# beta-team/beta-recsys

Hardware: AMD Instinct MI355X
Metric: training interactions/sec (BPR triples) (higher is better)
Workload: dtype f32; 1 GPU; BPR-MF, MovieLens-1M-shaped synthetic (BASELINE configs[1]): 6040 users x 3706 items, dim 64, batch 4096 triples/GPU, uniform users, Zipf(1.0) positives, uniform negatives; optimizer=adam, loss=bpr, batch_per_gpu=4096, global_batch=4096, parallelism=single GPU, epoch=245 steps = 1003520 triples (SURVEY 8d C2: ~1M triples / epoch)

## Files before the change

beta-recsys_amd/_lib.py:

```python
import ctypes
import os
from ctypes import POINTER, Structure, c_char_p, c_double, c_float, c_int, c_int32, c_int64
from ctypes import c_size_t, c_uint32, c_void_p

_HERE = os.path.dirname(os.path.abspath(__file__))
LIB_PATH = os.path.join(_HERE, os.environ.get("HIPREC_LIB", "libhiprec.so"))

OPT_SGD, OPT_ADAM, OPT_RMSPROP = 0, 1, 2
OPT_KINDS = {"sgd": OPT_SGD, "adam": OPT_ADAM, "rmsprop": OPT_RMSPROP}
OPT_RMSPROP_MOMENTUM = 3

STATUS_USER_OOB, STATUS_ITEM_OOB, STATUS_ROW_OOB, STATUS_ROUTE_OVERFLOW = 1, 2, 4, 8
STATUS_NEG_EXHAUSTED = 16
STATUS_LAZY_TABLE = 32
STATUS_TABLE_FULL = 64


class MfTables(Structure):

    _fields_ = [
        ("user_emb", c_void_p),
        ("item_emb", c_void_p),
        ("user_bias", c_void_p),
        ("item_bias", c_void_p),
# ... 222 lines not shown
    "hiprec_mf_sgd_rows": (
        c_int,
        [_T, _T, _P, _P, _P, _P, c_int64, c_double, _P, _P, c_int32, _P, _P, _P],
    ),
    "hiprec_ncf_plan_bytes": (c_size_t, []),
    "hiprec_gemm_f32": (
        c_int,
        [c_int, c_int, c_int, c_int, _P, c_int, _P, c_int, _P, c_int, _P, c_int, _P, c_int, _P],
    ),
    "hiprec_ncf_forward": (c_int, [POINTER(NcfPlan), _P, _P, c_int64, _P, _P]),
    "hiprec_ncf_grad": (
        c_int,
        [POINTER(NcfPlan), _P, _P, _P, c_int64, c_float, _P, _P, c_size_t, _P],
    ),
    "hiprec_ncf_step": (
        c_int,
        [POINTER(NcfPlan), _P, _P, _P, c_int64, c_float, c_int, _P, _P, _P, _P, c_int64, c_int64, c_int64, c_double,
         c_double, c_double, c_double, _P, _P, c_size_t, _P],
    ),
    "hiprec_lightgcn_plan_bytes": (c_size_t, []),
    "hiprec_spmm_csr": (c_int, [POINTER(Csr), _P, c_float, _P, _P, _P, c_int32, _P]),
    "hiprec_sliced_width": (c_int32, [c_int64, c_int32]),
    "hiprec_sliced_row_cap": (c_int32, [c_int64, c_int32]),
    "hiprec_to_sliced": (c_int, [_P, c_int64, c_int32, c_int32, _P, _P, _P]),
    "hiprec_from_sliced": (c_int, [_P, c_int64, c_int32, c_int32, _P, c_int32, _P]),
    "hiprec_sliced_drop_values": (c_int, [POINTER(SlicedCsr), _P, _P, _P]),
    "hiprec_spmm_sliced": (c_int, [POINTER(SlicedCsr), _P, c_float, _P, _P, _P, c_int32, c_int32, c_int32, _P]),
    "hiprec_edge_dropout_mask": (c_int, [_P, c_int64, c_float, ctypes.c_uint64, ctypes.c_uint64, _P]),
    "hiprec_lightgcn_step_values": (c_int, [POINTER(LightGcnPlan), _P, c_float, c_int32, ctypes.c_uint64,
                                            ctypes.c_uint64, _P]),
    "hiprec_lightgcn_opt_stage": (c_int, [POINTER(LightGcnPlan), c_int32, _P, _P, _P, c_double, c_double, c_double,
                                          c_double, _P, _P, c_float, ctypes.c_uint64, ctypes.c_uint64, _P]),
    "hiprec_lightgcn_propagate": (c_int, [POINTER(LightGcnPlan), _P, c_float, _P]),
    "hiprec_lightgcn_predict": (c_int, [POINTER(LightGcnPlan), _P, _P, c_int64, _P, _P, _P]),
    "hiprec_lightgcn_grad": (
        c_int,
        [POINTER(LightGcnPlan), _P, c_float, _P, _P, _P, c_int64, c_float, _P, _P, c_size_t, _P],
    ),
    "hiprec_random_permutation": (c_int, [_P, c_int64, ctypes.c_uint64, _P]),
    "hiprec_fused_step_bytes": (c_size_t, []),
    "hiprec_mf_bpr_fused_step": (c_int, [POINTER(FusedStep), _P, _P, _P, c_int64, c_int64, c_float, _P, _P]),
    "hiprec_dp_step_bytes": (c_size_t, []),
    "hiprec_mf_dp_step_begin": (c_int, [POINTER(DpStep), _P, _P, _P, c_int64, c_float, _P]),
    "hiprec_mf_dp_step_end": (c_int, [POINTER(DpStep), _P]),
    "hiprec_sample_negatives": (
        c_int,
        [_P, _P, c_int64, c_int64, _P, c_int64, c_int32, ctypes.c_uint64, _P, _P, _P],
    ),
    "hiprec_pgmf_workspace_bytes": (c_size_t, [c_int32]),
    "hiprec_pgmf_bpr_grad": (
        c_int,
        [POINTER(PgmfTables), POINTER(PgmfTables), _P, _P, _P, c_int64, c_float, c_float, _P, _P, c_size_t,
         _P, c_size_t, _P],
    ),
    "hiprec_pgmf_epoch": (
        c_int,
        [POINTER(PgmfTables), POINTER(PgmfTables), _P, _P, _P, c_int64, c_int64, c_float, c_float, c_int,
         c_double, c_double, c_double, c_double, _P, _P, _P, _P, c_int64, _P, _P, c_size_t, _P, c_size_t,
         _P, c_size_t, _P],
    ),
    "hiprec_cmn_tables_bytes": (c_size_t, []),
    "hiprec_cmn_workspace_bytes": (c_size_t, [c_int32, c_int64]),
    "hiprec_cmn_grad_padded": (
        c_int,
        [POINTER(CmnTables), POINTER(CmnTables), _P, _P, _P, _P, _P, c_int64, _P, _P, c_int64, c_int64, c_float,
         c_float, _P, _P, _P, _P, c_size_t, _P, c_size_t, _P],
    ),
    "hiprec_cmn_grad_csr": (
        c_int,
        [POINTER(CmnTables), POINTER(CmnTables), _P, _P, _P, _P, _P, c_int64, c_float, c_float, _P, _P, _P, _P,
         c_size_t, _P, c_size_t, _P],
    ),
    "hiprec_cmn_epoch": (
        c_int,
        [POINTER(CmnTables), POINTER(CmnTables), _P, _P, _P, _P, _P, c_int64, c_int64, c_float, c_float, c_int,
         c_double, c_double, c_double, c_double, _P, _P, _P, _P, c_int64, _P, _P, c_size_t, _P, c_size_t,
         _P, c_size_t, _P],
    ),
    "hiprec_t2v_epoch": (
        c_int,
        [POINTER(T2vTables), POINTER(T2vTables), _P, _P, _P, _P, _P, _P, c_int64, c_int64, c_int32, c_float,
         c_int, c_double, c_double, c_double, c_double, _P, _P, _P, _P, c_int64, _P, _P, c_size_t, _P],
    ),
    "hiprec_clip_workspace_bytes": (c_size_t, []),
    "hiprec_clip_grad_norm": (c_int, [_P, c_int64, c_float, _P, c_size_t, _P]),
    "hiprec_clip_opt_dense_step": (
        c_int,
        [c_int, _P, _P, _P, _P, c_int64, c_double, c_double, c_double, c_double, _P, _P, c_int64, c_float, _P, c_size_t,
         _P],
    ),
    "hiprec_t2v_grad": (
        c_int,
        [POINTER(T2vTables), POINTER(T2vTables), _P, _P, _P, _P, _P, _P, c_int64, c_int32, c_float, _P, _P,
         c_size_t, _P],
    ),
    "hiprec_t2v_predict": (c_int, [POINTER(T2vTables), _P, _P, c_int64, _P, _P, _P]),
    "hiprec_sumsq_workspace_bytes": (c_size_t, []),
    "hiprec_sumsq": (c_int, [_P, c_int64, _P, c_size_t, _P]),
    "hiprec_opt_dense_step_decay": (
        c_int,
        [c_int, _P, _P, _P, _P, c_int64, c_double, c_double, c_double, c_double, _P, _P, c_float, _P, c_size_t, _P],
    ),
    "hiprec_decay_grad": (c_int, [_P, _P, c_int64, c_float, _P]),
    "hiprec_ultragcn_grad": (
        c_int,
        [POINTER(UltraGcnTables), POINTER(UltraGcnTables), POINTER(UltraGcnParams), _P, _P, _P, c_int64, c_int32, _P,
         _P, _P, c_size_t, _P],
    ),
    "hiprec_ultragcn_predict": (c_int, [POINTER(UltraGcnTables), _P, _P, c_int64, _P, _P, _P]),
    "hiprec_ultragcn_epoch": (
        c_int,
        [POINTER(UltraGcnTables), POINTER(UltraGcnTables), POINTER(UltraGcnParams), _P, _P, _P, c_int64, c_int64,
         c_int32, c_int, c_double, c_double, c_double, c_double, _P, _P, _P, _P, c_int64, _P, c_size_t, _P, _P,
         c_size_t, _P],
    ),
    "hiprec_alias_sample": (c_int, [_P, _P, _P, c_int64, ctypes.c_uint64, _P, c_int64, _P]),
    "hiprec_ngcf_plan_bytes": (c_size_t, []),
    "hiprec_ngcf_forward": (c_int, [POINTER(NgcfPlan), c_int, _P]),
    "hiprec_ngcf_predict": (c_int, [POINTER(NgcfPlan), _P, _P, c_int64, _P, _P, _P]),
    "hiprec_ngcf_grad": (c_int, [POINTER(NgcfPlan), _P, _P, _P, c_int64, c_float, _P, _P, c_size_t, _P]),
    "hiprec_csr_n_slices": (c_int64, [c_int64]),
    "hiprec_csr_slice_rows": (c_int, [POINTER(Csr), _P, c_int64, _P]),
    "hiprec_rank_metrics_workspace_bytes": (c_size_t, [c_int64, c_int32]),
    "hiprec_rank_metrics": (
        c_int,
        [_P, c_int64, _P, _P, POINTER(c_int32), c_int32, _P, c_size_t, _P, _P],
    ),
    "hiprec_topk_workspace_bytes": (c_size_t, [c_int64, c_int64, c_int32, c_int32]),
    "hiprec_topk_recommend": (
        c_int,
        [_P, c_int64, c_int64, _P, c_int64, c_int64, c_int32, c_float, _P, _P, c_int64, _P, _P, c_int32, c_int32, _P,
         c_size_t, _P, _P, _P, _P],
    ),
    "hiprec_topk_metrics": (
        c_int,
        [_P, c_int64, c_int32, _P, _P, POINTER(c_int32), c_int32, _P, c_size_t, _P, _P],
    ),
    "hiprec_stage_epoch": (c_int, [_P, _P, _P, c_int32, _P, c_int64, c_int64, _P, _P, _P, _P]),
    "hiprec_stage_epoch_shuffled": (c_int, [_P, _P, _P, c_int32, ctypes.c_uint64, c_int64, c_int64, _P, _P, _P, _P]),
    "hiprec_mf_bce_epoch": (
        c_int,
        [_T, _T, _P, _P, _P, _P, c_int64, c_int64, c_float, c_int]
        + [c_double, c_double, c_double, c_double]
        + [_P, _P, _P, _P, c_int64, _P, _P, c_int32, _P, _P, c_size_t, _P],
    ),
    "hiprec_mf_bpr_epoch_fused": (
        c_int,
        [c_int, _P, _P, _P, _P, _P, c_int64, c_int64, c_int32, _P, _P, _P, c_int64, c_int64, c_float,
         c_double, c_double, c_double, c_double, _P, POINTER(c_int32), _P],
    ),
    "hiprec_mf_bpr_epoch_fused_range": (
        c_int,
        [c_int, _P, _P, _P, _P, _P, c_int64, c_int64, c_int32, _P, _P, _P, c_int64, c_int64, c_int64, c_int64,
         c_float, c_double, c_double, c_double, c_double, _P, POINTER(c_int32), _P],
    ),
    "hiprec_mf_bpr_dp_epoch_fused_range": (
        c_int,
        [c_int, _P, _P, c_int64, _P, _P, c_int64, c_int64, c_int64, c_int32, _P, _P, _P, c_int64, c_int64, c_int64,
         c_int64, c_int32, c_float, c_double, c_double, c_double, c_double, _P, _P, _P, POINTER(c_int32), _P],
    ),
    "hiprec_mf_bpr_epoch_owned": (
        c_int,
        [_P, c_int64, c_int64, c_int32, _P, _P, _P, _P, _P, _P, _P, c_int64, _P, _P, c_int64, _P, _P, c_int64,
         c_int64, c_int64, c_int64, c_float, c_double, _P, _P],
    ),
    "hiprec_ownership_table_bits": (c_int32, [c_int64]),
    "hiprec_ownership_ws_ints": (c_int64, [c_int64, c_int64, c_int32]),
    "hiprec_batch_row_ownership": (
        c_int, [_P, _P, _P, c_int64, c_int64, c_int64, c_int64, c_int32, _P, _P, _P, _P]),
    "hiprec_stage_grouped_ws_ints": (c_int64, [c_int64, c_int64, c_int64]),
    "hiprec_stage_epoch_grouped": (
        c_int, [_P, _P, _P, _P, c_int32, ctypes.c_uint64, c_int64, c_int64, c_int64, _P, _P, _P, _P, _P]),
    "hiprec_mf_pull_chunk": (c_int32, [c_int32]),
    "hiprec_contrib_row_cap": (c_int64, [c_int64, c_int32]),
    "hiprec_batch_row_contrib": (
        c_int, [_P, _P, _P, c_int64, c_int64, c_int64, c_int64, c_int32, c_int32, c_int32, _P, _P, _P, c_int64, _P, _P]),
    "hiprec_mf_bpr_epoch_pull": (
        c_int,
        [_P, c_int64, c_int64, c_int32, _P, _P, _P, _P, c_int64, _P, c_int64, _P, _P, _P, _P, c_int64, c_int64,
         c_int64, c_int64, c_float, c_double, _P, _P],
    ),
    "hiprec_mf_bpr_owned_remote_step": (
        c_int,
        [_P, c_int64, c_int64, c_int32, _P, _P, c_int64, _P, _P, _P, _P, _P, _P, _P, _P, _P, c_int64, c_float,
         c_float, c_double, _P, _P, _P],
    ),
    "hiprec_mf_bpr_pull_remote_step": (
        c_int,
        [_P, c_int64, c_int64, c_int32, _P, _P, c_int64, _P, _P, _P, _P, _P, _P, _P, c_int64, _P, _P, _P, _P, c_int32,
         c_int64, c_float, c_float, c_double, _P, _P, _P],
    ),
    "hiprec_batch_row_ownership_tables": (
        c_int, [_P, _P, _P, c_int64, c_int64, c_int64, c_int64, c_int32, _P, _P, _P, _P, _P, _P, _P]),
    "hiprec_plan_route_tiles": (c_int64, [c_int64, c_int64]),
    "hiprec_plan_route_triples": (
        c_int, [_P, _P, _P, _P, c_int64, c_int64, c_int32, c_int64, c_int64, _P, _P, _P, _P, _P]),
    "hiprec_plan_place_triples": (c_int, [_P, c_int64, _P, c_int32, c_int64, c_int64, _P, _P, _P, _P, _P]),
    "hiprec_plan_slot_ws_ints": (c_int64, [c_int64, c_int32, c_int32]),
    "hiprec_plan_item_slots": (
        c_int, [_P, c_int64, c_int64, c_int32, c_int64, c_int32] + [_P] * 16 + [_P, _P, c_int64, _P, _P]),
    "hiprec_plan_place_requests": (c_int, [_P, c_int64, _P, c_int32, c_int64, _P, _P, _P, _P, c_int64, _P, _P]),
    "hiprec_shard_payload_zero": (
        c_int, [_P, _P, c_int64, c_int32, _P, c_int64, c_int64, c_int64, _P, _P, _P, c_int64, _P, _P, _P]),
    "hiprec_mf_bpr_grad_remote_step": (
        c_int,
        [_P, _P, c_int64, c_int64, c_int32, _P, _P, c_int64, _P, _P, _P, _P, _P, _P, _P, c_int64, c_float, c_float,
         _P, _P, _P],
    ),
    "hiprec_shard_apply_finish": (
        c_int, [_P, _P, c_int64, c_int32, _P, _P, c_int64, c_int64, c_int64, _P, c_double, _P, c_int32, _P, c_double,
                c_int32, _P, _P, _P]),
    "hiprec_shard_planned_steps": (
        c_int, [POINTER(ShardPlan), POINTER(ShardBufs), c_int64, c_int64, c_int32, c_float, c_double, c_double,
                c_double, c_double, POINTER(NcclFns), _P, _P, _P]),
    "hiprec_shard_planned_steps_ex": (
        c_int, [POINTER(ShardPlan), POINTER(ShardBufs), c_int64, c_int64, c_int32, c_float, c_double, c_double,
                c_double, c_double, POINTER(NcclFns), _P, ctypes.c_uint32, _P, _P]),
    "hiprec_gather_epoch": (c_int, [_P, _P, _P, _P, c_int32, ctypes.c_uint64, _P, c_int64, _P, _P, _P, _P]),
    "hiprec_stage_sort_keys": (c_int, [_P, _P, c_int32, ctypes.c_uint64, c_int64, c_int64, c_int64, c_int32, _P, _P]),
    "hiprec_group_epoch_by_item": (c_int, [_P, _P, _P, c_int64, c_int64, c_int64, c_int32, _P, _P, _P, _P, _P, _P, _P, _P,
                                           _P, _P]),
    "hiprec_lazy_state_bytes": (c_size_t, []),
    "hiprec_lazy_catchup": (c_int, [POINTER(LazyState), POINTER(LazyRows), _P, _P]),
    "hiprec_lazy_update": (c_int, [POINTER(LazyState), POINTER(LazyRows), _P, _P, _P]),
    "hiprec_lazy_flush": (c_int, [POINTER(LazyState), _P, _P]),
    "hiprec_lazy_mark_current": (c_int, [POINTER(LazyState), _P, _P]),
    "hiprec_mf_epoch_lazy": (c_int, [POINTER(LazyState), _T, _T, _P, _P, _P, c_int32, c_int64, c_int64, c_int32, c_float,
                                     _P, _P, c_size_t, _P]),
    "hiprec_mf_bpr_grad_owned": (c_int, [_P, _P, c_int64, c_int64, c_int32, _P, _P, _P, _P, _P, _P, _P, c_int64, c_float,
                                         c_float, _P, _P, _P]),
    "hiprec_mf_epoch_lazy_pull": (c_int, [POINTER(LazyState), _P, _P, _P, _P, c_int64, _P, c_int64, _P, _P, _P, c_int64,
                                          c_int64, c_int32, c_float, _P, _P, _P]),
    "hiprec_mf_epoch_lazy_owned": (c_int, [POINTER(LazyState), _P, _P, _P, _P, _P, _P, _P, c_int64, c_int64, c_int64,
                                           c_int32, c_float, _P, _P, _P]),
    "hiprec_shard_plan_bytes": (c_size_t, []),
    "hiprec_shard_bufs_bytes": (c_size_t, []),
    "hiprec_shard_publish_partials": (c_int, [_P, _P, c_int32, _P, c_int32, _P]),
    "hiprec_shard_apply_rows": (c_int, [_P, _P, c_int64, c_int32, _P, _P, c_int64, c_double, _P, _P]),
    "hiprec_shard_finish_step": (c_int, [_P, c_int32, _P, c_int32, _P, c_double, c_int32, _P, _P]),
    "hiprec_mf_bpr_epoch_sgd_fused": (
        c_int,
        [_P, _P, _P, c_int64, c_int64, c_int32, _P, _P, _P, c_int64, c_int64, c_float, c_double, _P,
         POINTER(c_int32), _P],
    ),
    "hiprec_mf_bpr_epoch": (
        c_int,
        [_T, _T, _P, _P, _P, _P, c_int64, c_int64, c_float, c_int]
        + [c_double, c_double, c_double, c_double]
        + [_P, _P, _P, _P, c_int64, _P, _P, c_int32, _P, _P, c_size_t, _P],
    ),
}

_lib = None


class HiprecError(RuntimeError):
    """A libhiprec call returned a non-zero code."""


def load():
    global _lib
    if _lib is not None:
        return _lib
    if not os.path.exists(LIB_PATH):
        raise RuntimeError(
            f"libhiprec.so not found at {LIB_PATH}: the HIP extension is the only compute path of "
            "this package (there is no CPU fallback). Build it with "
            "`python -c 'import __graft_entry__ as g; g.build()'` (hipcc --offload-arch=gfx950)."
        )
    import torch

    lib = ctypes.CDLL(LIB_PATH)
    for name, (restype, argtypes) in SIGNATURES.items():
        try:
            fn = getattr(lib, name)
        except AttributeError as exc:
            raise RuntimeError(f"libhiprec.so does not export {name}; rebuild it") from exc
        fn.restype = restype
        fn.argtypes = argtypes
    if lib.hiprec_stats_bytes() != ctypes.sizeof(Stats):
        raise RuntimeError("hiprec_stats layout mismatch between _lib.py and libhiprec.so")
    if lib.hiprec_lightgcn_plan_bytes() != ctypes.sizeof(LightGcnPlan):
        raise RuntimeError("hiprec_lightgcn_plan layout mismatch between _lib.py and libhiprec.so")
    if lib.hiprec_fused_step_bytes() != ctypes.sizeof(FusedStep):
        raise RuntimeError("hiprec_fused_step layout mismatch between _lib.py and libhiprec.so")
    if lib.hiprec_dp_step_bytes() != ctypes.sizeof(DpStep):
        raise RuntimeError("hiprec_dp_step layout mismatch between _lib.py and libhiprec.so")
    if lib.hiprec_ngcf_plan_bytes() != ctypes.sizeof(NgcfPlan):
        raise RuntimeError("hiprec_ngcf_plan layout mismatch between _lib.py and libhiprec.so")
    if lib.hiprec_lazy_state_bytes() != ctypes.sizeof(LazyState):
        raise RuntimeError("hiprec_lazy_state layout mismatch between _lib.py and libhiprec.so")
    if lib.hiprec_shard_bufs_bytes() != ctypes.sizeof(ShardBufs):
        raise RuntimeError("hiprec_shard_bufs layout mismatch between _lib.py and libhiprec.so")
    if lib.hiprec_cmn_tables_bytes() != ctypes.sizeof(CmnTables):
        raise RuntimeError("hiprec_cmn_tables layout mismatch between _lib.py and libhiprec.so")
    if lib.hiprec_ncf_plan_bytes() != ctypes.sizeof(NcfPlan):
        raise RuntimeError("hiprec_ncf_plan layout mismatch between _lib.py and libhiprec.so")
    _lib = _DeviceGuardedLib(lib)
    return _lib


class _Stream(c_void_p):

    device_index = None


# ... 77 lines not shown
```

beta-recsys_amd/csrc/common.hpp:

```cpp
#pragma once
#include <hip/hip_runtime.h>

#include <atomic>
#include <initializer_list>

#include <cstdarg>
#include <cstdint>
#include <cstdio>

#include "../../include/hiprec.h"

namespace hiprec {

constexpr int kWave = 64;
constexpr int kBlock = 256;
constexpr int kWavesPerBlock = kBlock / kWave;
constexpr int kMaxBlocks = 2048;
constexpr int kAggWaves = 16;
constexpr int kAggBlock = kAggWaves * kWave;
constexpr int kAggMaxBlocks = 512;
constexpr size_t kScratchBytes = 16 + sizeof(float) * 4 * kMaxBlocks;

struct Scratch {
  uint32_t n_partials;
  uint32_t _pad[3];
  float4 partials[kMaxBlocks];
};
static_assert(sizeof(Scratch) == kScratchBytes, "scratch layout");

void set_error(const char* fmt, ...);
int hip_fail(hipError_t e, const char* what);

int allow_dynamic_lds(std::initializer_list<const void*> kernels, size_t bytes, std::atomic<uint64_t>& done,
                      const char* what);

int opt_dense_step_impl(int kind, float* w, float* g, float* m, float* v, int64_t n, double lr, double beta1,
                        double beta2, double eps, hiprec_stats* stats, const void* scratch, int64_t scalar_index,
                        double* clip_ws, int n_clip, float max_norm, void* stream);

#define HIPREC_TRY(expr)                                   \
  do {                                                     \
    hipError_t _e = (expr);                                \
    if (_e != hipSuccess) return hiprec::hip_fail(_e, #expr); \
  } while (0)

#define HIPREC_REQUIRE(cond, ...)        \
  do {                                   \
    if (!(cond)) {                       \
      hiprec::set_error(__VA_ARGS__);    \
      return HIPREC_E_BADARG;            \
    }                                    \
  } while (0)

inline int grid_for_waves(int64_t n_waves) {
  int64_t blocks = (n_waves + kWavesPerBlock - 1) / kWavesPerBlock;
  if (blocks < 1) blocks = 1;
  if (blocks > kMaxBlocks) blocks = kMaxBlocks;
  return static_cast<int>(blocks);
}

inline int grid_for_threads(int64_t n_threads) {
  int64_t blocks = (n_threads + kBlock - 1) / kBlock;
  if (blocks < 1) blocks = 1;
  if (blocks > kMaxBlocks) blocks = kMaxBlocks;
  return static_cast<int>(blocks);
}

__host__ __device__ inline int feistel_half_bits(uint64_t n) {
  int bits = 2;
  while (bits < 62 && (1ull << bits) < n) ++bits;
  return (bits + 1) / 2;
}

#if defined(__HIPCC__)

__device__ __forceinline__ uint64_t splitmix64(uint64_t x) {
  x += 0x9E3779B97F4A7C15ull;
  x = (x ^ (x >> 30)) * 0xBF58476D1CE4E5B9ull;
  x = (x ^ (x >> 27)) * 0x94D049BB133111EBull;
  return x ^ (x >> 31);
}

__device__ __forceinline__ bool keep_draw(uint64_t seed, uint64_t step, int64_t e, float keep_prob) {
  uint64_t z = seed + 0x9E3779B97F4A7C15ull * (static_cast<uint64_t>(e) + 1) + 0xD1B54A32D192ED03ull * (step + 1);
  z = (z ^ (z >> 30)) * 0xBF58476D1CE4E5B9ull;
  z = (z ^ (z >> 27)) * 0x94D049BB133111EBull;
  z ^= z >> 31;
  return static_cast<float>(z >> 40) * (1.0f / 16777216.0f) < keep_prob;
}

__device__ __forceinline__ uint32_t feistel_round(uint32_t x, uint32_t key) {
  x = (x ^ key) * 0x9E3779B1u;
  x ^= x >> 15;
  x *= 0x85EBCA77u;
  x ^= x >> 13;
  return x;
}

__device__ __forceinline__ uint64_t feistel_permute(uint64_t i, uint64_t n, int half_bits, uint64_t seed) {
  const uint64_t mask = (1ull << half_bits) - 1ull;
  uint64_t x = i;
  do {
    uint32_t l = static_cast<uint32_t>(x >> half_bits), r = static_cast<uint32_t>(x & mask);
#pragma unroll
    for (int round = 0; round < 6; ++round) {
      const uint32_t k = static_cast<uint32_t>(seed >> (8 * (round & 3))) + 0x632BE5ABu * (round + 1) +
                         static_cast<uint32_t>(seed >> 32);
      const uint32_t f = feistel_round(r, k) & static_cast<uint32_t>(mask);
      const uint32_t nl = r;
      r = l ^ f;
      l = nl;
    }
    x = (static_cast<uint64_t>(l) << half_bits) | r;
  } while (x >= n);
  return x;
}

template <int CTRL>
__device__ __forceinline__ float dpp_add(float v) {
  int moved = __builtin_amdgcn_update_dpp(0, __builtin_bit_cast(int, v), CTRL, 0xF, 0xF, false);
  return v + __builtin_bit_cast(float, moved);
}

__device__ __forceinline__ float wave_sum(float v) {
  v = dpp_add<0xB1>(v);
  v = dpp_add<0x4E>(v);
  v = dpp_add<0x141>(v);
  v = dpp_add<0x140>(v);
  int iv = __builtin_bit_cast(int, v);
  float r0 = __builtin_bit_cast(float, __builtin_amdgcn_readlane(iv, 0));
  float r1 = __builtin_bit_cast(float, __builtin_amdgcn_readlane(iv, 16));
  float r2 = __builtin_bit_cast(float, __builtin_amdgcn_readlane(iv, 32));
  float r3 = __builtin_bit_cast(float, __builtin_amdgcn_readlane(iv, 48));
  return (r0 + r1) + (r2 + r3);
}

__device__ __forceinline__ int wave_in_block() {
  return __builtin_amdgcn_readfirstlane(static_cast<int>(threadIdx.x) >> 6);
}

__device__ __forceinline__ int lane_id() { return static_cast<int>(threadIdx.x) & 63; }

__device__ __forceinline__ void lds_barrier() {
  asm volatile("s_waitcnt lgkmcnt(0)" ::: "memory");
  __builtin_amdgcn_s_barrier();
  asm volatile("" ::: "memory");
}

__device__ __forceinline__ void lds_add_f32(float* p, float v) {
  __hip_atomic_fetch_add(p, v, __ATOMIC_RELAXED, __HIP_MEMORY_SCOPE_WORKGROUP);
}

__device__ __forceinline__ void atomic_add_f32(float* p, float v) {
  __hip_atomic_fetch_add(p, v, __ATOMIC_RELAXED, __HIP_MEMORY_SCOPE_AGENT);
}

__device__ __forceinline__ int run_head(const long long* s_item, int wv, long long item) {
  int head = wv;
  while (head > 0 && s_item[head - 1] == item) --head;
  return head;
}

__device__ __forceinline__ int run_end(const long long* s_item, int wv, long long item, int n_waves) {
  int end = wv + 1;
  while (end < n_waves && s_item[end] == item) ++end;
  return end;
}

__device__ __forceinline__ float sigmoid_f32(float s) { return 1.0f / (1.0f + expf(-s)); }

__device__ __forceinline__ float neg_logsigmoid(float x, float* sig_neg_x) {
  float z = expf(-fabsf(x));
  float frac = z / (1.0f + z);
  *sig_neg_x = x < 0.0f ? 1.0f - frac : frac;
  return log1pf(z) - fminf(x, 0.0f);
}

template <int NW>
__device__ __forceinline__ void publish_partials(float loss_w, float reg_lane, float gb_w,
                                                 float inv_batch, Scratch* scratch) {
  __shared__ float s_loss[NW];
  __shared__ float s_reg[NW];
  __shared__ float s_gb[NW];
  float reg_w = wave_sum(reg_lane);
  const int w = wave_in_block();
  if (lane_id() == 0) {
    s_loss[w] = loss_w;
    s_reg[w] = reg_w;
    s_gb[w] = gb_w;
  }
  lds_barrier();
  if (threadIdx.x == 0) {
    float l = 0.f, r = 0.f, b = 0.f;
#pragma unroll
    for (int i = 0; i < NW; ++i) {
      l += s_loss[i];
      r += s_reg[i];
      b += s_gb[i];
    }
    scratch->partials[blockIdx.x] = make_float4(l * inv_batch, r * inv_batch, b, 0.f);
    if (blockIdx.x == 0) scratch->n_partials = gridDim.x;
  }
}

template <int NT = kBlock>
__device__ __forceinline__ float finalize_partials(hiprec_stats* stats, const Scratch* scratch) {
  __shared__ double s_l[NT];
  __shared__ double s_r[NT];
  __shared__ double s_b[NT];
  const uint32_t n = scratch->n_partials;
  double l = 0.0, r = 0.0, b = 0.0;
  for (uint32_t i = threadIdx.x; i < n; i += NT) {
    float4 p = scratch->partials[i];
    l += p.x;
    r += p.y;
    b += p.z;
  }
  s_l[threadIdx.x] = l;
  s_r[threadIdx.x] = r;
  s_b[threadIdx.x] = b;
  __syncthreads();
  for (int s = NT / 2; s > 0; s >>= 1) {
    if (static_cast<int>(threadIdx.x) < s) {
      s_l[threadIdx.x] += s_l[threadIdx.x + s];
// ... 108 lines not shown
```

beta-recsys_amd/csrc/mf.hip:

```cpp
#include <algorithm>
#include <type_traits>

#include "common.hpp"

namespace hiprec {



struct TripleIdx {
  int64_t u, p, n;
  bool valid;
};

__device__ __forceinline__ TripleIdx load_triple(const hiprec_mf_tables& w,
                                                 const int64_t* __restrict__ users,
                                                 const int64_t* __restrict__ pos,
                                                 const int64_t* __restrict__ neg,
                                                 const int64_t* __restrict__ perm, int64_t t,
                                                 int64_t batch, hiprec_stats* stats, int lane) {
  TripleIdx r{0, 0, 0, t < batch};
  if (r.valid) {
    const int64_t j = perm ? perm[t] : t;
    r.u = users[j];
    r.p = pos[j];
// ... 324 lines not shown
      const bool i_ok = static_cast<uint64_t>(p) < static_cast<uint64_t>(f.n_items) &&
                        static_cast<uint64_t>(n) < static_cast<uint64_t>(f.n_items);
      if (!(u_ok && i_ok)) {
        if (lane == 0)
          atomicOr(&stats->status,
                   (u_ok ? 0u : HIPREC_STATUS_USER_OOB) | (i_ok ? 0u : HIPREC_STATUS_ITEM_OOB));
        valid = false;
      }
    }
    if (lane == 0) s_item[wv] = valid ? static_cast<long long>(p) : -static_cast<long long>(wv + 1);
    lds_barrier();
    const int head = valid ? run_head(s_item, wv, p) : wv;
    const bool is_head = head == wv;
    const int tail = (valid && is_head) ? run_end(s_item, wv, p, kAggWaves) : wv + 1;

    float uu[NPL], pp[NPL];
    float dpos = 0.f, bp = 0.f;
    if (valid) {
      const int64_t ou = u * D, op = o_ie + p * D, on = o_ie + n * D;
      float nn[NPL];
      float dp = 0.f, dn = 0.f;
      const float wbu = wf[o_ub + u], gbu = f.g_prev[o_ub + u];
      const float wbn = wf[o_ib + n], gbn = f.g_prev[o_ib + n];
      const float wbp = wf[o_ib + p], gbp_ = f.g_prev[o_ib + p];
      float mbu = 0.f, mbn = 0.f, mbp = 0.f, vbu = 0.f, vbn = 0.f, vbp = 0.f;
      if constexpr (kHasM) {
        mbu = f.m_read[o_ub + u];
        mbn = f.m_read[o_ib + n];
        mbp = f.m_read[o_ib + p];
      }
      if constexpr (kHasV) {
        vbu = f.v_read[o_ub + u];
        vbn = f.v_read[o_ib + n];
        vbp = f.v_read[o_ib + p];
      }
      float wu[NPL], gu[NPL], wp[NPL], gpv[NPL], wn[NPL], gn[NPL];
      float mu[NPL], mpv[NPL], mn[NPL], vu[NPL], vpv[NPL], vn[NPL];
#pragma unroll
      for (int k = 0; k < NPL; ++k) {
        const int c = lane + kWave * k;
        const int cc = c < D ? c : D - 1;
        wu[k] = wf[ou + cc];
        gu[k] = f.g_prev[ou + cc];
        wp[k] = wf[op + cc];
        gpv[k] = f.g_prev[op + cc];
        wn[k] = wf[on + cc];
        gn[k] = f.g_prev[on + cc];
        mu[k] = mpv[k] = mn[k] = vu[k] = vpv[k] = vn[k] = 0.f;
        if constexpr (kHasM) {
          mu[k] = f.m_read[ou + cc];
          mpv[k] = f.m_read[op + cc];
          mn[k] = f.m_read[on + cc];
        }
        if constexpr (kHasV) {
          vu[k] = f.v_read[ou + cc];
          vpv[k] = f.v_read[op + cc];
          vn[k] = f.v_read[on + cc];
        }
      }
#pragma unroll
      for (int k = 0; k < NPL; ++k) {
        const bool in = lane + kWave * k < D;
        if (apply) {
          wu[k] = fused_eff<KIND>(wu[k], gu[k], mu[k], vu[k], f.s, step_size, bc2_sqrt);
          wp[k] = fused_eff<KIND>(wp[k], gpv[k], mpv[k], vpv[k], f.s, step_size, bc2_sqrt);
          wn[k] = fused_eff<KIND>(wn[k], gn[k], mn[k], vn[k], f.s, step_size, bc2_sqrt);
        }
        uu[k] = in ? wu[k] : 0.f;
        pp[k] = in ? wp[k] : 0.f;
        nn[k] = in ? wn[k] : 0.f;
      }
#pragma unroll
      for (int k = 0; k < NPL; ++k) {
        dp += uu[k] * pp[k];
        dn += uu[k] * nn[k];
        reg_acc += 2.f * uu[k] * uu[k] + pp[k] * pp[k] + nn[k] * nn[k];
      }
      dp = wave_sum(dp);
      dn = wave_sum(dn);
      if (!gb_ready) {
        float gbp = 0.f;
#pragma unroll
        for (int j = 0; j < kFusedSlots; ++j) {
          asm volatile("" : "+v"(gbz[j]));
          gbp += lane + kWave * j < f.n_prev_partials ? gbz[j] : 0.f;
        }
        gb = apply ? fused_eff<KIND>(gb_w, gb_g + wave_sum(gbp), gb_m, gb_v, f.s, step_size, bc2_sqrt)
                   : gb_w;
        gb_ready = true;
      }
      float bu = wbu, bn = wbn;
      bp = wbp;
      if (apply) {
        bu = fused_eff<KIND>(wbu, gbu, mbu, vbu, f.s, step_size, bc2_sqrt);
        bn = fused_eff<KIND>(wbn, gbn, mbn, vbn, f.s, step_size, bc2_sqrt);
        bp = fused_eff<KIND>(wbp, gbp_, mbp, vbp, f.s, step_size, bc2_sqrt);
      }
      const float yp = sigmoid_f32(((dp + bu) + bp) + gb);
      const float yn = sigmoid_f32(((dn + bu) + bn) + gb);
      float sig_neg_x;
      const float nls = neg_logsigmoid(yp - yn, &sig_neg_x);
      const float delta = -sig_neg_x * inv_batch;
      dpos = delta * ((1.f - yp) * yp);
      const float dneg = -delta * ((1.f - yn) * yn);
      float* gur = gf + ou;
      float* gnr = gf + on;
      float* slot = s_acc + wv * ld;
#pragma unroll
      for (int k = 0; k < NPL; ++k) {
        const int c = lane + kWave * k;
        if (c < D) {
          atomic_add_f32(gur + c, (dpos * pp[k] + dneg * nn[k]) + ru * uu[k]);
          atomic_add_f32(gnr + c, dneg * uu[k] + ri * nn[k]);
          slot[c] = dpos * uu[k] + ri * pp[k];
        }
      }
      if (lane == 0) {
        atomic_add_f32(gf + o_ub + u, (dpos + dneg) + ru * bu);
        atomic_add_f32(gf + o_ib + n, dneg + ri * bn);
        slot[D] = dpos + ri * bp;
        reg_acc += 2.f * bu * bu + bp * bp + bn * bn;
      }
      loss_acc += nls;
      gb_acc += dpos + dneg;
    }
    lds_barrier();
    if (valid && is_head) {
      float* gpr = gf + o_ie + p * D;
      for (int c = lane; c <= D; c += kWave) {
        float t = s_acc[wv * ld + c];
        for (int j = wv + 1; j < tail; ++j) t += s_acc[j * ld + c];
        atomic_add_f32(c < D ? gpr + c : gf + o_ib + p, t);
      }
    }
  }
  __shared__ float s_loss[kAggWaves], s_reg[kAggWaves], s_gbv[kAggWaves];
  const float reg_w = wave_sum(reg_acc);
  if (lane == 0) {
    s_loss[wv] = loss_acc;
    s_reg[wv] = reg_w;
    s_gbv[wv] = gb_acc;
  }
  lds_barrier();
  if (threadIdx.x == 0) {
    float l = 0.f, r = 0.f, b = 0.f;
#pragma unroll
    for (int i = 0; i < kAggWaves; ++i) {
      l += s_loss[i];
      r += s_reg[i];
      b += s_gbv[i];
    }
    scratch->partials[blockIdx.x] = make_float4(l * inv_batch, r * inv_batch, b, 0.f);
    if (blockIdx.x == 0) scratch->n_partials = static_cast<uint32_t>(f.n_gather_blocks);
  }
}

template <int NPL>
__global__ __launch_bounds__(kAggBlock) void mf_bce_grad_kernel(
    hiprec_mf_tables w, hiprec_mf_tables g, const int64_t* __restrict__ users,
    const int64_t* __restrict__ items, const float* __restrict__ ratings,
    const int64_t* __restrict__ perm, int64_t batch, float inv_batch, float reg_coef,
    hiprec_stats* stats, Scratch* scratch) {
  extern __shared__ __attribute__((aligned(16))) float s_acc[];
  __shared__ long long s_item[kAggWaves];
  const int lane = lane_id();
  const int wv = wave_in_block();
  const int D = w.dim;
  const int ld = D + 1;
  const float gb = load_scalar_param(w.global_bias);
  const float rr = 2.f * reg_coef * inv_batch;

  float loss_acc = 0.f, reg_acc = 0.f, gb_acc = 0.f;
  const bool stepper = blockIdx.x == 0 && threadIdx.x == 0;
  StepState step_state{};
  if (stepper) step_state = step_load(stats);

  for (int64_t base = static_cast<int64_t>(blockIdx.x) * kAggWaves; base < batch;
       base += static_cast<int64_t>(gridDim.x) * kAggWaves) {
    const int64_t t = base + wv;
    bool valid = t < batch;
    int64_t u = 0, i = 0;
    float r = 0.f;
    if (valid) {
      const int64_t j = perm ? perm[t] : t;
      u = users[j];
      i = items[j];
      r = ratings[j];
      const bool u_ok = static_cast<uint64_t>(u) < static_cast<uint64_t>(w.n_users);
      const bool i_ok = static_cast<uint64_t>(i) < static_cast<uint64_t>(w.n_items);
      if (!(u_ok && i_ok)) {
        if (lane == 0)
          atomicOr(&stats->status,
                   (u_ok ? 0u : HIPREC_STATUS_USER_OOB) | (i_ok ? 0u : HIPREC_STATUS_ITEM_OOB));
        valid = false;
      }
    }
    if (lane == 0) s_item[wv] = valid ? static_cast<long long>(i) : -static_cast<long long>(wv + 1);
    lds_barrier();
    const int head = valid ? run_head(s_item, wv, i) : wv;
    const bool is_head = head == wv;
    const int tail = (valid && is_head) ? run_end(s_item, wv, i, kAggWaves) : wv + 1;

    const float* ur = w.user_emb + u * D;
    const float* ir = w.item_emb + i * D;
    float uu[NPL > 0 ? NPL : 1], ii[NPL > 0 ? NPL : 1];
    float ds = 0.f, bi = 0.f;
    if (valid) {
      float* gur = g.user_emb + u * D;
      float dot = 0.f;
      if constexpr (NPL > 0) {
#pragma unroll
        for (int k = 0; k < NPL; ++k) {
          const int c = lane + kWave * k;
          const bool in = c < D;
          uu[k] = in ? ur[c] : 0.f;
          ii[k] = in ? ir[c] : 0.f;
          dot += uu[k] * ii[k];
          reg_acc += uu[k] * uu[k] + ii[k] * ii[k];
        }
      } else {
        for (int c = lane; c < D; c += kWave) {
          const float a = ur[c], b = ir[c];
          dot += a * b;
          reg_acc += a * a + b * b;
        }
      }
      dot = wave_sum(dot);
      const float bu = w.user_bias[u];
      bi = w.item_bias[i];
      const float y = sigmoid_f32(((dot + bu) + bi) + gb);
      const float ly = fmaxf(logf(y), -100.f);
      const float l1y = fmaxf(log1pf(-y), -100.f);
      const float loss_k = -(r * ly + (1.f - r) * l1y);
      const float gy = (y - r) / fmaxf((1.f - y) * y, 1e-12f) * inv_batch;
      ds = gy * ((1.f - y) * y);

      float* slot = s_acc + wv * ld;
      if constexpr (NPL > 0) {
#pragma unroll
        for (int k = 0; k < NPL; ++k) {
          const int c = lane + kWave * k;
          if (c < D) {
            atomic_add_f32(gur + c, ds * ii[k] + rr * uu[k]);
            slot[c] = ds * uu[k] + rr * ii[k];
          }
        }
      } else {
        for (int c = lane; c < D; c += kWave) {
          const float a = ur[c], b = ir[c];
          atomic_add_f32(gur + c, ds * b + rr * a);
          slot[c] = ds * a + rr * b;
        }
      }
      if (lane == 0) {
        atomic_add_f32(g.user_bias + u, ds + rr * bu);
        slot[D] = ds + rr * bi;
        reg_acc += bu * bu + bi * bi;
      }
      loss_acc += loss_k;
      gb_acc += ds;
    }
    lds_barrier();
    if (valid && is_head) {
      float* gir = g.item_emb + i * D;
      for (int c = lane; c <= D; c += kWave) {
        float t = s_acc[wv * ld + c];
        for (int j = wv + 1; j < tail; ++j) t += s_acc[j * ld + c];
        atomic_add_f32(c < D ? gir + c : g.item_bias + i, t);
      }
    }
  }
  publish_partials<kAggWaves>(loss_acc, reg_acc, gb_acc, inv_batch, scratch);
  if (stepper) step_store_advanced(stats, step_state);
}

__global__ __launch_bounds__(kBlock) void mf_predict_kernel(hiprec_mf_tables w,
                                                            const int64_t* __restrict__ users,
                                                            const int64_t* __restrict__ items,
                                                            int64_t n, float* __restrict__ scores,
                                                            float* __restrict__ sq, hiprec_stats* stats) {
  const int lane = lane_id();
  const int D = w.dim;
  const int64_t wave0 = static_cast<int64_t>(blockIdx.x) * kWavesPerBlock + wave_in_block();
  const int64_t n_waves = static_cast<int64_t>(gridDim.x) * kWavesPerBlock;
  const float gb = load_scalar_param(w.global_bias);
  for (int64_t t = wave0; t < n; t += n_waves) {
    const int64_t u = users[t], i = items[t];
    const bool u_ok = static_cast<uint64_t>(u) < static_cast<uint64_t>(w.n_users);
    const bool i_ok = static_cast<uint64_t>(i) < static_cast<uint64_t>(w.n_items);
    if (!(u_ok && i_ok)) {
      if (lane == 0) {
        atomicOr(&stats->status,
                 (u_ok ? 0u : HIPREC_STATUS_USER_OOB) | (i_ok ? 0u : HIPREC_STATUS_ITEM_OOB));
        scores[t] = __builtin_nanf("");
        if (sq) sq[t] = 0.f;
      }
      continue;
    }
    const float* ur = w.user_emb + u * D;
    const float* ir = w.item_emb + i * D;
    float dot = 0.f, ss = 0.f;
    for (int c = lane; c < D; c += kWave) {
      const float a = ur[c], b = ir[c];
      dot += a * b;
      ss += a * a + b * b;
    }
// ... 247 lines not shown
  return dispatch_npl(w->dim, [&](auto npl) {
    mf_sgd_rows_kernel<decltype(npl)::value><<<grid, kBlock, 0, st>>>(
        *w, *g, users, items_a, items_b, perm, batch, static_cast<float>(lr), user_stamp, item_stamp, stamp,
        stats, static_cast<const Scratch*>(scratch));
  });
}

template <int KIND>
static int launch_fused(int dim, int grid, size_t lds, hipStream_t st, const FusedOpt& f, const int64_t* uu,
                        const int64_t* pp, const int64_t* nn, int64_t b, float inv_b, float reg_coef,
                        hiprec_stats* stats, Scratch* sc) {
  if (b == 0)
    mf_bpr_fused_kernel<1, KIND, true><<<grid, kAggBlock, lds, st>>>(f, uu, pp, nn, b, inv_b, reg_coef, stats, sc);
  else if (dim <= 64)
    mf_bpr_fused_kernel<1, KIND, false><<<grid, kAggBlock, lds, st>>>(f, uu, pp, nn, b, inv_b, reg_coef, stats, sc);
  else if (dim <= 128)
    mf_bpr_fused_kernel<2, KIND, false><<<grid, kAggBlock, lds, st>>>(f, uu, pp, nn, b, inv_b, reg_coef, stats, sc);
  else
    mf_bpr_fused_kernel<4, KIND, false><<<grid, kAggBlock, lds, st>>>(f, uu, pp, nn, b, inv_b, reg_coef, stats, sc);
  HIPREC_TRY(hipGetLastError());
  return 0;
}

extern "C" int hiprec_mf_bpr_fused_step(const hiprec_fused_step* c, const int64_t* users,
                                        const int64_t* pos, const int64_t* neg, int64_t batch,
                                        int64_t prev_batch, float inv_batch, hiprec_stats* stats,
                                        void* stream) {
  HIPREC_REQUIRE(c && stats, "NULL step / stats");
  const int kind = c->kind;
  HIPREC_REQUIRE(kind == HIPREC_OPT_SGD || kind == HIPREC_OPT_ADAM || kind == HIPREC_OPT_RMSPROP,
                 "unknown optimizer kind %d", kind);
  const bool has_m = kind == HIPREC_OPT_ADAM, has_v = kind != HIPREC_OPT_SGD;
  HIPREC_REQUIRE(c->w_read && c->w_write && c->g_prev && c->g_cur && c->g_zero && c->scratch_prev &&
                     c->scratch_cur, "NULL buffer");
  HIPREC_REQUIRE(!has_m || (c->m_read && c->m_write), "Adam needs m_read / m_write");
  HIPREC_REQUIRE(!has_v || (c->v_read && c->v_write), "Adam/RMSprop need v_read / v_write");
  HIPREC_REQUIRE(c->n_users > 0 && c->n_items > 0 && c->dim > 0 && c->dim <= 256, "fused step needs dim <= 256");
  HIPREC_REQUIRE(batch >= 0 && prev_batch >= 0, "negative batch");
  HIPREC_REQUIRE(batch == 0 || (users && pos && neg), "NULL index arrays");
  hipStream_t st = static_cast<hipStream_t>(stream);
  const int64_t n_users = c->n_users, n_items = c->n_items;
  const int dim = c->dim;
  const int64_t n_flat = (n_users + n_items) * (static_cast<int64_t>(dim) + 1) + 1;
  FusedOpt f;
  f.n_users = n_users;
  f.n_items = n_items;
  f.dim = dim;
  f._pad0 = 0;
  f.g_cur = c->g_cur;
  f.w_read = c->w_read;
  f.g_prev = c->g_prev;
  f.m_read = has_m ? c->m_read : nullptr;
  f.v_read = has_v ? c->v_read : nullptr;
  f.w_write = c->w_write;
  f.m_write = has_m ? c->m_write : nullptr;
  f.v_write = has_v ? c->v_write : nullptr;
  f.g_zero = c->g_zero;
  f.g_zero2 = batch == 0 ? const_cast<float*>(c->g_prev) : nullptr;
  f.n_flat = n_flat;
  f.s = OptScalars{c->lr,
                   static_cast<float>(c->lr),
                   static_cast<float>(c->beta2),
                   static_cast<float>(1.0 - c->beta1),
                   static_cast<float>(1.0 - c->beta2),
                   static_cast<float>(c->eps)};
  f.n_gather_blocks = batch > 0 ? std::min(agg_grid(batch), kFusedMaxGather) : 0;
  f.n_prev_partials = prev_batch > 0 ? std::min(agg_grid(prev_batch), kFusedMaxGather) : 0;
  f.apply_prev = prev_batch > 0 ? 1 : 0;
  f.scratch_prev = static_cast<const Scratch*>(c->scratch_prev);
  Scratch* sc = static_cast<Scratch*>(c->scratch_cur);
  const size_t lds = agg_lds_bytes(dim);
  const int n_sweep = static_cast<int>(std::min<int64_t>(256, (n_flat / 4 + kAggBlock - 1) / kAggBlock));
  const int grid = f.n_gather_blocks + n_sweep;
  int rc;
  if (kind == HIPREC_OPT_SGD)
    rc = launch_fused<HIPREC_OPT_SGD>(dim, grid, lds, st, f, users, pos, neg, batch, inv_batch, c->reg_coef, stats, sc);
  else if (kind == HIPREC_OPT_ADAM)
    rc = launch_fused<HIPREC_OPT_ADAM>(dim, grid, lds, st, f, users, pos, neg, batch, inv_batch, c->reg_coef, stats, sc);
  else
    rc = launch_fused<HIPREC_OPT_RMSPROP>(dim, grid, lds, st, f, users, pos, neg, batch, inv_batch, c->reg_coef, stats, sc);
  return rc;
}

extern "C" size_t hiprec_fused_step_bytes(void) { return sizeof(hiprec_fused_step); }

extern "C" int hiprec_mf_bpr_epoch_fused_range(int kind, float* const* w_flat, float* const* g_flat,
                                               float* const* m_flat, float* const* v_flat,
                                               void* const* scratch2, int64_t n_users, int64_t n_items,
                                               int32_t dim, const int64_t* users, const int64_t* pos,
                                               const int64_t* neg, int64_t n_triples, int64_t batch,
                                               int64_t step_begin, int64_t step_end,
                                               float reg_coef, double lr, double beta1, double beta2,
                                               double eps, hiprec_stats* stats, int32_t* final_index,
                                               void* stream) {
  HIPREC_REQUIRE(w_flat && g_flat && scratch2 && final_index && stats, "NULL pointer");
  HIPREC_REQUIRE(w_flat[0] && w_flat[1] && g_flat[0] && g_flat[1] && g_flat[2] && scratch2[0] &&
                     scratch2[1], "NULL buffer");
  const bool has_m = kind == HIPREC_OPT_ADAM, has_v = kind != HIPREC_OPT_SGD;
  HIPREC_REQUIRE(!has_m || (m_flat && m_flat[0] && m_flat[1]), "Adam needs m_flat[2]");
  HIPREC_REQUIRE(!has_v || (v_flat && v_flat[0] && v_flat[1]), "Adam/RMSprop need v_flat[2]");
  HIPREC_REQUIRE(n_triples >= 0 && batch > 0, "bad n_triples/batch");
  HIPREC_REQUIRE(n_triples == 0 || (users && pos && neg), "NULL index arrays");
  const int64_t n_steps = (n_triples + batch - 1) / batch;
  HIPREC_REQUIRE(0 <= step_begin && step_begin <= step_end && step_end <= n_steps,
                 "bad step range [%lld, %lld) of %lld", (long long)step_begin, (long long)step_end, (long long)n_steps);
  const int64_t k_end = step_end == n_steps ? n_steps + 1 : step_end;
  hiprec_fused_step c{};
  c.kind = kind;
  c.dim = dim;
  c.n_users = n_users;
  c.n_items = n_items;
  c.lr = lr;
  c.beta1 = beta1;
  c.beta2 = beta2;
  c.eps = eps;
  c.reg_coef = reg_coef;
  for (int64_t k = step_begin; k < k_end; ++k) {
    const int64_t off = k * batch;
    const int64_t b = k < n_steps ? std::min<int64_t>(batch, n_triples - off) : 0;
    const int64_t prev_b = k > 0 ? std::min<int64_t>(batch, n_triples - (k - 1) * batch) : 0;
    const int out = k == n_steps ? 0 : static_cast<int>((k + 1) & 1);
    c.w_read = w_flat[k & 1];
    c.w_write = w_flat[out];
    c.m_read = has_m ? m_flat[k & 1] : nullptr;
    c.m_write = has_m ? m_flat[out] : nullptr;
    c.v_read = has_v ? v_flat[k & 1] : nullptr;
    c.v_write = has_v ? v_flat[out] : nullptr;
    c.g_prev = g_flat[(k + 2) % 3];
    c.g_cur = g_flat[k % 3];
    c.g_zero = g_flat[(k + 1) % 3];
    c.scratch_prev = scratch2[(k + 1) & 1];
    c.scratch_cur = scratch2[k & 1];
    const float inv_b = b > 0 ? 1.0f / static_cast<float>(b) : 0.f;
    if (int rc = hiprec_mf_bpr_fused_step(&c, users ? users + off : nullptr, pos ? pos + off : nullptr,
                                          neg ? neg + off : nullptr, b, prev_b, inv_b, stats, stream))
      return rc;
  }
  *final_index = step_end == n_steps ? 0 : -1;
  return 0;
}

extern "C" int hiprec_mf_bpr_epoch_fused(int kind, float* const* w_flat, float* const* g_flat,
                                         float* const* m_flat, float* const* v_flat,
                                         void* const* scratch2, int64_t n_users, int64_t n_items,
                                         int32_t dim, const int64_t* users, const int64_t* pos,
                                         const int64_t* neg, int64_t n_triples, int64_t batch,
                                         float reg_coef, double lr, double beta1, double beta2,
                                         double eps, hiprec_stats* stats, int32_t* final_index,
                                         void* stream) {
  const int64_t n_steps = batch > 0 && n_triples >= 0 ? (n_triples + batch - 1) / batch : 0;
  return hiprec_mf_bpr_epoch_fused_range(kind, w_flat, g_flat, m_flat, v_flat, scratch2, n_users, n_items, dim,
                                         users, pos, neg, n_triples, batch, 0, n_steps, reg_coef, lr, beta1,
                                         beta2, eps, stats, final_index, stream);
}

using nccl_all_reduce_fn = int (*)(const void*, void*, size_t, int, int, void*, hipStream_t);
constexpr int kNcclFloat32 = 7, kNcclSum = 0;

extern "C" int hiprec_mf_bpr_dp_epoch_fused_range(int kind, float* const* w_flat, float* const* bufs,
                                                  int64_t scratch_floats, float* const* m_flat,
                                                  float* const* v_flat, int64_t n_flat, int64_t n_users,
                                                  int64_t n_items, int32_t dim, const int64_t* users,
                                                  const int64_t* pos, const int64_t* neg, int64_t n_triples,
                                                  int64_t batch, int64_t step_begin, int64_t step_end,
                                                  int32_t world, float reg_coef, double lr, double beta1,
                                                  double beta2, double eps, hiprec_stats* stats,
                                                  void* all_reduce_fn, void* comm, int32_t* final_index,
                                                  void* stream) {
  HIPREC_REQUIRE(w_flat && bufs && final_index && stats && all_reduce_fn && comm, "NULL pointer");
  HIPREC_REQUIRE(w_flat[0] && w_flat[1] && bufs[0] && bufs[1] && bufs[2], "NULL buffer");
  const bool has_m = kind == HIPREC_OPT_ADAM, has_v = kind != HIPREC_OPT_SGD;
  HIPREC_REQUIRE(!has_m || (m_flat && m_flat[0] && m_flat[1]), "Adam needs m_flat[2]");
  HIPREC_REQUIRE(!has_v || (v_flat && v_flat[0] && v_flat[1]), "Adam/RMSprop need v_flat[2]");
  HIPREC_REQUIRE(n_triples >= 0 && batch > 0 && world >= 1 && scratch_floats >= 4 && n_flat > 0, "bad sizes");
  HIPREC_REQUIRE(n_triples == 0 || (users && pos && neg), "NULL index arrays");
  const int64_t n_steps = (n_triples + batch - 1) / batch;
  HIPREC_REQUIRE(0 <= step_begin && step_begin <= step_end && step_end <= n_steps,
                 "bad step range [%lld, %lld) of %lld", (long long)step_begin, (long long)step_end, (long long)n_steps);
  const auto all_reduce = reinterpret_cast<nccl_all_reduce_fn>(all_reduce_fn);
  const int64_t k_end = step_end == n_steps ? n_steps + 1 : step_end;
  hiprec_fused_step c{};
  c.kind = kind;
  c.dim = dim;
  c.n_users = n_users;
  c.n_items = n_items;
  c.lr = lr;
  c.beta1 = beta1;
  c.beta2 = beta2;
  c.eps = eps;
  c.reg_coef = reg_coef;
  for (int64_t k = step_begin; k < k_end; ++k) {
    const int64_t off = k * batch;
    const int64_t b = k < n_steps ? std::min<int64_t>(batch, n_triples - off) : 0;
    const int64_t prev_b = k > 0 ? std::min<int64_t>(batch, n_triples - (k - 1) * batch) : 0;
    const int out = k == n_steps ? 0 : static_cast<int>((k + 1) & 1);
    float* prev = bufs[(k + 2) % 3];
    float* cur = bufs[k % 3];
    float* nxt = bufs[(k + 1) % 3];
    c.w_read = w_flat[k & 1];
    c.w_write = w_flat[out];
    c.m_read = has_m ? m_flat[k & 1] : nullptr;
    c.m_write = has_m ? m_flat[out] : nullptr;
    c.v_read = has_v ? v_flat[k & 1] : nullptr;
    c.v_write = has_v ? v_flat[out] : nullptr;
    c.scratch_prev = prev;
    c.g_prev = prev + scratch_floats;
    c.scratch_cur = cur;
    c.g_cur = cur + scratch_floats;
    c.g_zero = nxt + scratch_floats;
    const float inv_b = b > 0 ? 1.0f / (static_cast<float>(b) * static_cast<float>(world)) : 0.f;
    if (int rc = hiprec_mf_bpr_fused_step(&c, b ? users + off : nullptr, b ? pos + off : nullptr,
                                          b ? neg + off : nullptr, b, prev_b, inv_b, stats, stream))
      return rc;
    if (k < n_steps) {
      const int rc = all_reduce(cur + 4, cur + 4, static_cast<size_t>(scratch_floats - 4 + n_flat), kNcclFloat32,
                                kNcclSum, comm, static_cast<hipStream_t>(stream));
      if (rc != 0) {
        set_error("the caller's all-reduce returned %d at step %lld", rc, (long long)k);
        return HIPREC_E_UNSUPPORTED;
      }
    }
  }
  *final_index = step_end == n_steps ? 0 : -1;
  return 0;
}

extern "C" int hiprec_mf_bpr_epoch_sgd_fused(float* const* w_flat, float* const* g_flat,
                                             void* const* scratch2, int64_t n_users,
                                             int64_t n_items, int32_t dim, const int64_t* users,
                                             const int64_t* pos, const int64_t* neg,
                                             int64_t n_triples, int64_t batch, float reg_coef,
                                             double lr, hiprec_stats* stats, int32_t* final_index,
                                             void* stream) {
  return hiprec_mf_bpr_epoch_fused(HIPREC_OPT_SGD, w_flat, g_flat, nullptr, nullptr, scratch2, n_users,
                                   n_items, dim, users, pos, neg, n_triples, batch, reg_coef, lr, 0.0,
                                   0.0, 0.0, stats, final_index, stream);
}
```

beta-recsys_amd/csrc/util.hip:

```cpp
#include <cstring>

#include <cmath>

#include "common.hpp"

namespace hiprec {

static thread_local char g_err[512] = "";

void set_error(const char* fmt, ...) {
  va_list ap;
  va_start(ap, fmt);
  vsnprintf(g_err, sizeof(g_err), fmt, ap);
  va_end(ap);
}

int hip_fail(hipError_t e, const char* what) {
  set_error("HIP error %d (%s) in %s", static_cast<int>(e), hipGetErrorString(e), what);
  return static_cast<int>(e);
}

int allow_dynamic_lds(std::initializer_list<const void*> kernels, size_t bytes, std::atomic<uint64_t>& done,
                      const char* what) {
  int dev = 0, lds_max = 0;
// ... 116 lines not shown
__global__ __launch_bounds__(kBlock) void scatter_add_rows_kernel(float* __restrict__ table,
                                                                  int64_t n_rows, int dim,
                                                                  const int64_t* __restrict__ idx,
                                                                  const float* __restrict__ src,
                                                                  int64_t src_stride, int64_t n,
                                                                  hiprec_stats* stats) {
  const int lane = lane_id();
  const int64_t wave0 = static_cast<int64_t>(blockIdx.x) * kWavesPerBlock + wave_in_block();
  const int64_t n_waves = static_cast<int64_t>(gridDim.x) * kWavesPerBlock;
  for (int64_t k = wave0; k < n; k += n_waves) {
    const int64_t r = idx[k];
    if (r == -1) continue;
    if (static_cast<uint64_t>(r) >= static_cast<uint64_t>(n_rows)) {
      if (lane == 0) atomicOr(&stats->status, HIPREC_STATUS_ROW_OOB);
      continue;
    }
    const float* s = src + k * src_stride;
    float* d = table + r * dim;
    for (int c = lane; c < dim; c += kWave) atomic_add_f32(d + c, s[c]);
  }
}

__global__ __launch_bounds__(kBlock) void random_permutation_kernel(int64_t* __restrict__ out,
                                                                    int64_t n, int half_bits,
                                                                    uint64_t seed) {
  const int64_t stride = static_cast<int64_t>(gridDim.x) * kBlock;
  for (int64_t i = static_cast<int64_t>(blockIdx.x) * kBlock + threadIdx.x; i < n; i += stride) {
    const uint64_t x = feistel_permute(static_cast<uint64_t>(i), static_cast<uint64_t>(n), half_bits, seed);
    out[i] = static_cast<int64_t>(x);
  }
}

template <typename K, int NPAD, int NT>
__device__ __forceinline__ void bitonic_sort_lds(K* s_kv, bool dirty) {
  constexpr int kWaves = NT / kWave;
  constexpr int C = NPAD / kWaves;
  static_assert(C >= kWave && (C & (C - 1)) == 0, "chunk must be a power of two >= the wave size");
  const int lane = lane_id();
  const int chunk0 = wave_in_block() * C;
  for (int k = 2; k <= NPAD; k <<= 1) {
    for (int j = k >> 1; j > 0; j >>= 1) {
      if (j >= C) {
        __syncthreads();
        for (int p = threadIdx.x; p < NPAD / 2; p += NT) {
          const int i = ((p & ~(j - 1)) << 1) | (p & (j - 1)), l = i | j;
          const K a = s_kv[i], b = s_kv[l];
          if ((a > b) == ((i & k) == 0)) {
            s_kv[i] = b;
            s_kv[l] = a;
          }
        }
        dirty = true;
      } else {
        if (dirty) {
          __syncthreads();
          dirty = false;
        }
#pragma unroll
        for (int p = lane; p < C / 2; p += kWave) {
          const int i = chunk0 + (((p & ~(j - 1)) << 1) | (p & (j - 1))), l = i | j;
          const K a = s_kv[i], b = s_kv[l];
          if ((a > b) == ((i & k) == 0)) {
            s_kv[i] = b;
            s_kv[l] = a;
          }
        }
        __builtin_amdgcn_fence(__ATOMIC_ACQ_REL, "wavefront");
        __builtin_amdgcn_wave_barrier();
      }
    }
  }
  __syncthreads();
}

constexpr int kStagePosBits = 13;

template <int NPAD, int NT>
__global__ __launch_bounds__(NT) void stage_epoch_kernel(const int64_t* __restrict__ users,
                                                         const int64_t* __restrict__ items,
                                                         const void* __restrict__ third,
                                                         int third_bytes,
                                                         const int64_t* __restrict__ perm,
                                                         uint64_t seed, int half_bits,
                                                         int64_t n, int64_t batch,
                                                         int64_t* __restrict__ out_u,
                                                         int64_t* __restrict__ out_i,
                                                         void* __restrict__ out_third) {
  static_assert(NPAD <= (1 << kStagePosBits), "position bits");
  __shared__ unsigned long long s_kv[NPAD];
  uint32_t* s_k32 = reinterpret_cast<uint32_t*>(s_kv);
  const int64_t off = static_cast<int64_t>(blockIdx.x) * batch;
  const int cnt = static_cast<int>(min<int64_t>(batch, n - off));
  auto source = [&](int i) -> int64_t {
    const int64_t j = off + i;
    if (perm) return perm[j];
    if (half_bits)
      return static_cast<int64_t>(feistel_permute(static_cast<uint64_t>(j), static_cast<uint64_t>(n), half_bits, seed));
    return j;
  };
  constexpr int kPer = (NPAD + NT - 1) / NT;
  uint32_t mine[kPer];
  bool fits = true;
#pragma unroll
  for (int t = 0; t < kPer; ++t) {
    const int i = threadIdx.x + t * NT;
    mine[t] = 0xFFFFFFFFu;
    if (i < cnt) {
      mine[t] = static_cast<uint32_t>(items[source(i)]);
      fits = fits && (mine[t] >> (32 - kStagePosBits)) == 0;
    }
  }
  const bool small = __syncthreads_and(fits) != 0;
  int src_of[kPer];
  if (small) {
#pragma unroll
    for (int t = 0; t < kPer; ++t) {
      const int i = threadIdx.x + t * NT;
      if (i < NPAD) s_k32[i] = i < cnt ? (mine[t] << kStagePosBits) | static_cast<uint32_t>(i) : 0xFFFFFFFFu;
    }
    bitonic_sort_lds<uint32_t, NPAD, NT>(s_k32, true);
#pragma unroll
    for (int t = 0; t < kPer; ++t) {
      const int i = threadIdx.x + t * NT;
      src_of[t] = i < cnt ? static_cast<int>(s_k32[i] & ((1u << kStagePosBits) - 1u)) : 0;
    }
  } else {
#pragma unroll
    for (int t = 0; t < kPer; ++t) {
      const int i = threadIdx.x + t * NT;
      if (i < NPAD)
        s_kv[i] = i < cnt ? (static_cast<unsigned long long>(mine[t]) << 32) | static_cast<uint32_t>(i) : ~0ull;
    }
    bitonic_sort_lds<unsigned long long, NPAD, NT>(s_kv, true);
#pragma unroll
    for (int t = 0; t < kPer; ++t) {
      const int i = threadIdx.x + t * NT;
      src_of[t] = i < cnt ? static_cast<int>(s_kv[i] & 0xFFFFFFFFull) : 0;
    }
  }
#pragma unroll
  for (int t = 0; t < kPer; ++t) {
    const int i = threadIdx.x + t * NT;
    if (i >= cnt) continue;
    const int64_t j = source(src_of[t]);
    out_u[off + i] = users[j];
    out_i[off + i] = items[j];
    if (third_bytes == 8)
      static_cast<int64_t*>(out_third)[off + i] = static_cast<const int64_t*>(third)[j];
    else
      static_cast<float*>(out_third)[off + i] = static_cast<const float*>(third)[j];
  }
}

}

using namespace hiprec;

extern "C" int hiprec_random_permutation(int64_t* out, int64_t n, uint64_t seed, void* stream) {
  HIPREC_REQUIRE(n >= 0 && n < (1ll << 62) && (n == 0 || out), "bad permutation request");
  if (n == 0) return 0;
  const int half_bits = feistel_half_bits(static_cast<uint64_t>(n));
  HIPREC_REQUIRE(half_bits <= 31, "n too large for the 32-bit Feistel halves");
  random_permutation_kernel<<<grid_for_threads(n), kBlock, 0, static_cast<hipStream_t>(stream)>>>(
      out, n, half_bits, seed);
  HIPREC_TRY(hipGetLastError());
  return 0;
}

static int stage_epoch_impl(const int64_t* users, const int64_t* items, const void* third, int32_t third_bytes,
                            const int64_t* perm, uint64_t seed, bool shuffle, int64_t n, int64_t batch,
                            int64_t* out_users, int64_t* out_items, void* out_third, void* stream) {
  HIPREC_REQUIRE(n >= 0 && batch > 0, "bad n / batch");
  HIPREC_REQUIRE(third_bytes == 4 || third_bytes == 8, "third array must be fp32 or int64");
  if (n == 0) return 0;
  HIPREC_REQUIRE(users && items && third && out_users && out_items && out_third, "NULL pointer");
  if (batch > 8192) {
    set_error("hiprec_stage_epoch sorts a batch in LDS: batch %lld > 8192 is not supported",
              (long long)batch);
    return HIPREC_E_UNSUPPORTED;
  }
  const int64_t n_batches = (n + batch - 1) / batch;
  HIPREC_REQUIRE(n_batches < (1ll << 31), "too many batches");
  int half_bits = 0;
  if (shuffle) {
    half_bits = feistel_half_bits(static_cast<uint64_t>(n));
    HIPREC_REQUIRE(half_bits <= 31, "n too large for the 32-bit Feistel halves");
  }
  hipStream_t st = static_cast<hipStream_t>(stream);
  const int grid = static_cast<int>(n_batches);
#define HIPREC_STAGE(NP, T)                                                                              \
  stage_epoch_kernel<NP, T><<<grid, T, 0, st>>>(users, items, third, third_bytes, perm, seed, half_bits, \
                                                n, batch, out_users, out_items, out_third)
  if (batch <= 64) HIPREC_STAGE(64, 64);
  else if (batch <= 256) HIPREC_STAGE(256, 256);
  else if (batch <= 1024) HIPREC_STAGE(1024, 512);
  else if (batch <= 2048) HIPREC_STAGE(2048, 1024);
  else if (batch <= 4096) HIPREC_STAGE(4096, 1024);
  else HIPREC_STAGE(8192, 1024);
#undef HIPREC_STAGE
  HIPREC_TRY(hipGetLastError());
  return 0;
}

extern "C" int hiprec_stage_epoch(const int64_t* users, const int64_t* items, const void* third,
                                  int32_t third_bytes, const int64_t* perm, int64_t n, int64_t batch,
                                  int64_t* out_users, int64_t* out_items, void* out_third,
                                  void* stream) {
  return stage_epoch_impl(users, items, third, third_bytes, perm, 0, false, n, batch, out_users, out_items,
                          out_third, stream);
}

extern "C" int hiprec_stage_epoch_shuffled(const int64_t* users, const int64_t* items, const void* third,
                                           int32_t third_bytes, uint64_t seed, int64_t n, int64_t batch,
                                           int64_t* out_users, int64_t* out_items, void* out_third,
                                           void* stream) {
  return stage_epoch_impl(users, items, third, third_bytes, nullptr, seed, true, n, batch, out_users,
                          out_items, out_third, stream);
}

extern "C" int hiprec_scatter_add_rows(float* table, int64_t n_rows, int32_t dim,
                                       const int64_t* idx, const float* src, int64_t src_stride,
                                       int64_t n, hiprec_stats* stats, void* stream) {
  HIPREC_REQUIRE(n >= 0 && n_rows > 0 && dim > 0 && src_stride >= dim, "bad sizes");
  if (n == 0) return 0;
  HIPREC_REQUIRE(table && idx && src && stats, "NULL pointer");
  scatter_add_rows_kernel<<<grid_for_waves(n), kBlock, 0, static_cast<hipStream_t>(stream)>>>(
      table, n_rows, dim, idx, src, src_stride, n, stats);
  HIPREC_TRY(hipGetLastError());
  return 0;
}

extern "C" int hiprec_version(void) { return HIPREC_VERSION; }

#ifndef HIPREC_SOURCE_HASH
#define HIPREC_SOURCE_HASH "unknown"
#endif
extern "C" const char* hiprec_source_hash(void) { return HIPREC_SOURCE_HASH; }
extern "C" const char* hiprec_last_error(void) { return g_err; }
extern "C" size_t hiprec_stats_bytes(void) { return sizeof(hiprec_stats); }
extern "C" size_t hiprec_scratch_bytes(int64_t) { return kScratchBytes; }

extern "C" int hiprec_stats_reset(hiprec_stats* stats, double beta1, double beta2, void* stream) {
  HIPREC_REQUIRE(stats, "NULL stats");
  stats_reset_kernel<<<1, 1, 0, static_cast<hipStream_t>(stream)>>>(stats, beta1, beta2);
  HIPREC_TRY(hipGetLastError());
  return 0;
}

extern "C" int hiprec_stats_set_step(hiprec_stats* stats, int64_t step, double beta1, double beta2, void* stream) {
  HIPREC_REQUIRE(stats && step >= 0, "NULL stats / negative step");
  stats_set_step_kernel<<<1, 1, 0, static_cast<hipStream_t>(stream)>>>(
      stats, static_cast<long long>(step), beta1, beta2, pow(beta1, static_cast<double>(step)),
      pow(beta2, static_cast<double>(step)));
  HIPREC_TRY(hipGetLastError());
  return 0;
}

extern "C" int hiprec_stats_begin_epoch(hiprec_stats* stats, void* stream) {
  HIPREC_REQUIRE(stats, "NULL stats");
  stats_begin_epoch_kernel<<<1, 1, 0, static_cast<hipStream_t>(stream)>>>(stats);
  HIPREC_TRY(hipGetLastError());
  return 0;
}

extern "C" int hiprec_stats_advance_step(hiprec_stats* stats, void* stream) {
  HIPREC_REQUIRE(stats, "NULL stats");
  stats_advance_kernel<<<1, 1, 0, static_cast<hipStream_t>(stream)>>>(stats);
  HIPREC_TRY(hipGetLastError());
  return 0;
}

extern "C" int hiprec_finalize_stats(hiprec_stats* stats, const void* scratch, float* g_scalar,
                                     float* loss_reg_out, void* stream) {
  HIPREC_REQUIRE(stats && scratch, "NULL stats/scratch");
  finalize_kernel<<<1, kBlock, 0, static_cast<hipStream_t>(stream)>>>(
      stats, static_cast<const Scratch*>(scratch), g_scalar, loss_reg_out);
  HIPREC_TRY(hipGetLastError());
  return 0;
}

extern "C" int hiprec_gather_rows(const float* table, int64_t n_rows, int32_t dim,
                                  const int64_t* idx, int64_t n, float* out, hiprec_stats* stats,
                                  void* stream) {
  HIPREC_REQUIRE(n >= 0 && n_rows > 0 && dim > 0, "bad sizes");
  if (n == 0) return 0;
  HIPREC_REQUIRE(table && idx && out && stats, "NULL pointer");
  hipStream_t st = static_cast<hipStream_t>(stream);
  const bool vec4 = (dim % 4 == 0) && ((reinterpret_cast<uintptr_t>(table) & 15) == 0) &&
                    ((reinterpret_cast<uintptr_t>(out) & 15) == 0);
  if (vec4) {
    gather_rows_kernel<4><<<grid_for_threads(n * (dim / 4)), kBlock, 0, st>>>(table, n_rows, dim,
                                                                             idx, n, out, stats);
  } else {
    gather_rows_kernel<1><<<grid_for_threads(n * dim), kBlock, 0, st>>>(table, n_rows, dim, idx,
                                                                       n, out, stats);
  }
  HIPREC_TRY(hipGetLastError());
  return 0;
}

extern "C" int hiprec_route_bucket(const int64_t* keys, int64_t n, int32_t n_dest, int64_t cap,
                                   int32_t* counts, int64_t* slot_out, hiprec_stats* stats,
                                   void* stream) {
  HIPREC_REQUIRE(n >= 0 && n_dest > 0 && n_dest <= 64 && cap > 0, "bad routing sizes");
  HIPREC_REQUIRE(counts && stats && (n == 0 || (keys && slot_out)), "NULL pointer");
  hipStream_t st = static_cast<hipStream_t>(stream);
  HIPREC_TRY(hipMemsetAsync(counts, 0, sizeof(int32_t) * n_dest, st));
  if (n == 0) return 0;
  route_bucket_kernel<<<grid_for_threads(n), kBlock, 0, st>>>(keys, n, n_dest, cap, counts, slot_out,
                                                              stats);
  HIPREC_TRY(hipGetLastError());
  return 0;
}

extern "C" int hiprec_mf_bpr_epoch(const hiprec_mf_tables* w, const hiprec_mf_tables* g,
                                   const int64_t* users, const int64_t* pos, const int64_t* neg,
                                   const int64_t* perm, int64_t n_triples, int64_t batch,
                                   float reg_coef, int kind,
                                   double lr, double beta1, double beta2, double eps,
                                   float* flat_w, float* flat_g, float* flat_m, float* flat_v,
                                   int64_t n_flat, int32_t* user_stamp, int32_t* item_stamp,
                                   int32_t first_stamp, hiprec_stats* stats, void* scratch,
                                   size_t scratch_bytes, void* stream) {
  HIPREC_REQUIRE(n_triples >= 0 && batch > 0, "bad n_triples/batch");
  const bool rows_sgd = (kind == HIPREC_OPT_SGD) && user_stamp && item_stamp;
  if (!rows_sgd) HIPREC_REQUIRE(flat_w && flat_g && n_flat > 0, "dense optimizer needs flat buffers");
  if (int rc = hiprec_stats_begin_epoch(stats, stream)) return rc;
  int32_t stamp = first_stamp;
  for (int64_t off = 0; off < n_triples; off += batch, ++stamp) {
    const int64_t b = (n_triples - off < batch) ? (n_triples - off) : batch;
    const float inv_b = 1.0f / static_cast<float>(b);
    const int64_t* pm = perm ? perm + off : nullptr;
    const int64_t* uu = perm ? users : users + off;
    const int64_t* pp = perm ? pos : pos + off;
    const int64_t* nn = perm ? neg : neg + off;
    if (int rc = hiprec_mf_bpr_grad(w, g, uu, pp, nn, pm, b, inv_b, reg_coef, stats, scratch,
                                    scratch_bytes, stream))
      return rc;
    int rc;
    if (rows_sgd)
      rc = hiprec_mf_sgd_rows(w, g, uu, pp, nn, pm, b, lr, user_stamp, item_stamp, stamp, stats,
                              scratch, stream);
    else
      rc = hiprec_opt_dense_step(kind, flat_w, flat_g, flat_m, flat_v, n_flat, lr, beta1, beta2,
                                 eps, stats, scratch, w->global_bias - flat_w, stream);
    if (rc) return rc;
  }
  return 0;
}

extern "C" int hiprec_mf_bce_epoch(const hiprec_mf_tables* w, const hiprec_mf_tables* g,
                                   const int64_t* users, const int64_t* items, const float* ratings,
                                   const int64_t* perm, int64_t n_samples, int64_t batch,
                                   float reg_coef, int kind, double lr, double beta1, double beta2,
                                   double eps, float* flat_w, float* flat_g, float* flat_m,
                                   float* flat_v, int64_t n_flat, int32_t* user_stamp,
                                   int32_t* item_stamp, int32_t first_stamp, hiprec_stats* stats,
                                   void* scratch, size_t scratch_bytes, void* stream) {
  HIPREC_REQUIRE(n_samples >= 0 && batch > 0, "bad n_samples/batch");
  const bool rows_sgd = (kind == HIPREC_OPT_SGD) && user_stamp && item_stamp;
  if (!rows_sgd) HIPREC_REQUIRE(flat_w && flat_g && n_flat > 0, "dense optimizer needs flat buffers");
  if (int rc = hiprec_stats_begin_epoch(stats, stream)) return rc;
  int32_t stamp = first_stamp;
  for (int64_t off = 0; off < n_samples; off += batch, ++stamp) {
    const int64_t b = (n_samples - off < batch) ? (n_samples - off) : batch;
    const float inv_b = 1.0f / static_cast<float>(b);
    const int64_t* pm = perm ? perm + off : nullptr;
    const int64_t* uu = perm ? users : users + off;
    const int64_t* ii = perm ? items : items + off;
    const float* rr = perm ? ratings : ratings + off;
// ... 38 lines not shown
```

beta-recsys_amd/mf.py:

```python
import ctypes
import time
from functools import wraps

import numpy as np
import torch
import torch.nn as nn
from torch.nn import Parameter

from . import _lib
from .torch_engine import ModelEngine


def timeit(method):

    @wraps(method)
    def wrapper(*args, **kw):
        ts = time.time()
        result = method(*args, **kw)
        te = time.time()
        if "log_time" in kw:
            name = kw.get("log_name", method.__name__.upper())
            kw["log_time"][name] = int((te - ts) * 1000)
        else:
            print("Execute [{}] method costing {:2.2f} ms".format(method.__name__, (te - ts) * 1000))
# ... 95 lines not shown
    return out.reshape(*idx.shape, table.shape[1])


class MF(nn.Module):

    def __init__(self, config):
        super().__init__()
        self.config = config
        self.device = self.config["device_str"]
        self.stddev = self.config["stddev"] if "stddev" in self.config else 0.1
        self.n_users = int(self.config["n_users"])
        self.n_items = int(self.config["n_items"])
        self.emb_dim = int(self.config["emb_dim"])
        U, I, D = self.n_users, self.n_items, self.emb_dim
        self._sizes = (U * D, I * D, U, I, 1)
        flat = torch.empty(sum(self._sizes), dtype=torch.float32)
        ue, ie, ub, ib, gb = self._views(flat)
        ue.normal_(0, 1)
        ie.normal_(0, 1)
        ub.normal_(0, 1)
        ib.normal_(0, 1)
        ub.fill_(0.0)
        ib.fill_(0.0)
        gb.fill_(0.0)
        ue.normal_(0, self.stddev)
        ie.normal_(0, self.stddev)
        self._flat = flat
        self._table_cache = {}
        self.user_emb = _Table(ue)
        self.item_emb = _Table(ie)
        self.user_bias = _Table(ub)
        self.item_bias = _Table(ib)
        self.global_bias = Parameter(gb, requires_grad=False)
        self._stats = None

    def _views(self, flat):
        U, I, D = self.n_users, self.n_items, self.emb_dim
        o = np.cumsum((0,) + self._sizes)
        return (
            flat[o[0]:o[1]].view(U, D),
            flat[o[1]:o[2]].view(I, D),
            flat[o[2]:o[3]].view(U, 1),
            flat[o[3]:o[4]].view(I, 1),
            flat[o[4]:o[5]],
        )

    def _rebind(self, flat):
        ue, ie, ub, ib, gb = self._views(flat)
        self._flat = flat
        self.user_emb.weight.data = ue
        self.item_emb.weight.data = ie
        self.user_bias.weight.data = ub
        self.item_bias.weight.data = ib
        self.global_bias.data = gb

    def _apply(self, fn, recurse=True):
        new_flat = fn(self._flat)
        if new_flat.dtype != torch.float32:
            raise TypeError("hiprec MF keeps fp32 parameters (the reference trains in fp32)")
        if new_flat is not self._flat:
            self._rebind(new_flat.contiguous())
            self._stats = None
        return self

    @property
    def flat(self):
        return self._flat

    def tables(self, flat=None):
        flat = self._flat if flat is None else flat
        base = flat.data_ptr()
        cached = self._table_cache.get(base)
        if cached is None:
            o = np.cumsum((0,) + self._sizes) * 4
            cached = _lib.MfTables(
                base + int(o[0]), base + int(o[1]), base + int(o[2]), base + int(o[3]),
                base + int(o[4]), self.n_users, self.n_items, self.emb_dim, 0)
            if len(self._table_cache) > 8:
                self._table_cache.clear()
            self._table_cache[base] = cached
        return cached

    def _require_hip(self):
        if self._flat.device.type != "cuda":
            raise RuntimeError(
                "hiprec MF computes on an MI355X through libhiprec.so only; parameters are on "
                f"{self._flat.device} and there is deliberately no CPU fallback"
            )
        if self._stats is None:
            self._stats = _new_stats(self._flat.device)
        return _lib.load()

    def forward(self, batch_data):
        users, items = batch_data
        dev = self._flat.device
        users = torch.as_tensor(users, dtype=torch.int64, device=dev).contiguous()
        items = torch.as_tensor(items, dtype=torch.int64, device=dev).contiguous()
        lib, n = self._require_hip(), users.numel()
        if items.numel() != n:
            raise ValueError("users and items must have the same length")
        scores, sq = torch.empty(n, dtype=torch.float32, device=dev), torch.empty(n, dtype=torch.float32, device=dev)
        tabs = self.tables()
        _lib.check(lib.hiprec_mf_forward(ctypes.byref(tabs), _lib.ptr(users), _lib.ptr(items), n, _lib.ptr(scores),
                                         _lib.ptr(sq), _lib.ptr(self._stats), _lib.stream_ptr(dev)))
        st = read_stats(self._stats)
        if st.status:
            clear_status(self._stats)
            raise_on_status(st.status)
        return scores, sq.sum() / max(n, 1)

    def _scores(self, users, items):
        lib = self._require_hip()
        dev = self._flat.device
        n = users.numel()
        if items.numel() != n:
            raise ValueError("users and items must have the same length")
        scores = torch.empty(n, dtype=torch.float32, device=dev)
        tabs = self.tables()
        _lib.check(
            lib.hiprec_mf_predict(
                ctypes.byref(tabs), _lib.ptr(users), _lib.ptr(items), n, _lib.ptr(scores),
                _lib.ptr(self._stats), _lib.stream_ptr(dev),
            )
        )
        return scores

    def ranking_factors(self):
        self._require_hip()
        return self.user_emb.weight.data, self.item_emb.weight.data, 1.0, self.item_bias.weight.data.reshape(-1)

    def predict(self, users, items):
        dev = self._flat.device
        users_t = torch.as_tensor(np.asarray(users), dtype=torch.int64).to(dev).contiguous()
        items_t = torch.as_tensor(np.asarray(items), dtype=torch.int64).to(dev).contiguous()
        scores = self._scores(users_t.reshape(-1), items_t.reshape(-1))
        st = read_stats(self._stats)
        if st.status:
            _lib.check(_lib.load().hiprec_stats_reset(_lib.ptr(self._stats), 0.9, 0.999,
                                                      _lib.stream_ptr(dev)))
            raise_on_status(st.status)
        return scores


def sort_within_batches(perm, items, batch_size, n_items):
    n = items.numel()
    idx = torch.arange(n, device=items.device) if perm is None else perm
    key = torch.div(torch.arange(n, device=items.device), batch_size, rounding_mode="floor")
    key = key * int(n_items) + items[idx]
    if (n + batch_size - 1) // batch_size * int(n_items) < 2**31:
        key = key.to(torch.int32)
    return idx[torch.argsort(key)].contiguous()


class PreparedEpoch(tuple):

    own = None


def batch_row_ownership(users, pos, neg, batch_size, n_users, n_items):
    if users.device.type != "cuda" or n_users + n_items >= 2**31:
        return batch_row_ownership_torch(users, pos, neg, batch_size, n_users, n_items)
    lib = _lib.load()
    n, dev = users.numel(), users.device
    n_batches = max((n + batch_size - 1) // batch_size, 1)
    bits = lib.hiprec_ownership_table_bits(batch_size)
    stride = 1 << bits
    keys = torch.empty(max(lib.hiprec_ownership_ws_ints(n, batch_size, bits), 1), dtype=torch.int32, device=dev)
    total = torch.empty((n_batches, stride), dtype=torch.int32, device=dev)
    own = torch.empty((3, n), dtype=torch.int32, device=dev)
    _lib.check(lib.hiprec_batch_row_ownership(
        _lib.ptr(users), _lib.ptr(pos), _lib.ptr(neg), n, batch_size, n_users, n_items, bits, _lib.ptr(keys),
        _lib.ptr(total), _lib.ptr(own), _lib.stream_ptr(dev)))
    return own, total, stride


class RowContributions(tuple):
    """(cidx int32 [3, n], rows int32 [n_batches, row_cap, 4], counts int32 [n_batches, 4], row_cap) of a staged
    epoch: hiprec_batch_row_contrib's arrays for the owner-pulls step (hiprec_mf_bpr_epoch_pull)."""


def batch_row_contributions(users, pos, neg, batch_size, n_users, n_items, dim, every_row=False):
    lib = _lib.load()
    n, dev = users.numel(), users.device
    n_batches = max((n + batch_size - 1) // batch_size, 1)
    bits = lib.hiprec_ownership_table_bits(batch_size)
    min_contrib = 1 if every_row else 2
    row_cap = lib.hiprec_contrib_row_cap(batch_size, min_contrib)
    i32 = dict(dtype=torch.int32, device=dev)
    ws = torch.empty(max(lib.hiprec_ownership_ws_ints(n, batch_size, bits), 1), **i32)
    cidx = torch.empty((3, n), **i32)
    rows = torch.empty((n_batches, row_cap, 4), **i32)
    counts = torch.empty((n_batches, 4), **i32)
    _lib.check(lib.hiprec_batch_row_contrib(
        _lib.ptr(users), _lib.ptr(pos), _lib.ptr(neg), n, batch_size, n_users, n_items, bits,
        lib.hiprec_mf_pull_chunk(dim), min_contrib, _lib.ptr(ws), _lib.ptr(cidx), _lib.ptr(rows), row_cap, _lib.ptr(counts),
        _lib.stream_ptr(dev)))
    return RowContributions((cidx, rows, counts, row_cap))


def group_epoch_by_item(users, pos, neg, batch_size, n_users, n_items):
    lib = _lib.load()
    n, dev = users.numel(), users.device
    n_batches = max((n + batch_size - 1) // batch_size, 1)
    bits = lib.hiprec_ownership_table_bits(batch_size)
    stride = 1 << bits
    i32 = dict(dtype=torch.int32, device=dev)
    keys, occ = torch.empty(max(lib.hiprec_ownership_ws_ints(n, batch_size, bits), 1), **i32), torch.empty(3 * n, **i32)
    own, own2 = torch.empty((3, n), **i32), torch.empty((3, n), **i32)
    total, tab_keys, pos_cnt = (torch.empty((n_batches, stride), **i32) for _ in range(3))
    invalid = torch.empty(n_batches, **i32)
    st = _lib.stream_ptr(dev)
    _lib.check(lib.hiprec_batch_row_ownership_tables(
        _lib.ptr(users), _lib.ptr(pos), _lib.ptr(neg), n, batch_size, n_users, n_items, bits, _lib.ptr(keys),
        _lib.ptr(total), _lib.ptr(own), _lib.ptr(tab_keys), _lib.ptr(pos_cnt), _lib.ptr(occ), st))
    ou, op, on = torch.empty_like(users), torch.empty_like(pos), torch.empty_like(neg)
    _lib.check(lib.hiprec_group_epoch_by_item(
        _lib.ptr(users), _lib.ptr(pos), _lib.ptr(neg), n, batch_size, n_users, bits, _lib.ptr(own), _lib.ptr(occ),
        _lib.ptr(tab_keys), _lib.ptr(pos_cnt), _lib.ptr(invalid), _lib.ptr(ou), _lib.ptr(op), _lib.ptr(on),
        _lib.ptr(own2), st))
    return ou, op, on, (own2, total, stride)


def batch_row_ownership_torch(users, pos, neg, batch_size, n_users, n_items):
    n, dev = users.numel(), users.device
    n_batches = (n + batch_size - 1) // batch_size
    stride = batch_size + batch_size // 2
    total = torch.zeros(n_batches * stride + 1, dtype=torch.int32, device=dev)
    if n == 0:
        return torch.zeros((3, 0), dtype=torch.int32, device=dev), total[:-1].view(n_batches, stride), stride
    idx = torch.arange(n, device=dev)
    bid = torch.div(idx, batch_size, rounding_mode="floor")
    ok = ((users >= 0) & (users < n_users) & (pos >= 0) & (pos < n_items) & (neg >= 0) & (neg < n_items))

    def slots(keys, n_rows, first_slot):
        skeys, order = torch.sort(keys)
        new_run = torch.ones_like(skeys, dtype=torch.bool)
        new_run[1:] = skeys[1:] != skeys[:-1]
        run = torch.cumsum(new_run, 0) - 1
        cnt = torch.zeros_like(skeys).index_add_(0, run, torch.ones_like(skeys))[run]
        shared = (cnt > 1) & (skeys >= 0)
        head = (shared & new_run).to(torch.int64)
        sb = torch.div(skeys, n_rows, rounding_mode="floor").clamp_(min=0)
        n_shared = torch.zeros(n_batches, dtype=torch.int64, device=dev).index_add_(0, sb, head)
        batch_start = torch.cumsum(n_shared, 0) - n_shared
        slot = torch.cumsum(head, 0) - 1 - batch_start[sb] + first_slot[sb]
        dump = torch.full_like(slot, n_batches * stride)
        total.index_put_((torch.where(head.bool(), sb * stride + slot, dump),), cnt.to(torch.int32))
        out = torch.empty_like(slot)
        out[order] = torch.where(shared, slot, torch.full_like(slot, -1))
        return out, n_shared

    ku = torch.where(ok, bid * n_users + users, -1 - idx)
    su, n_su = slots(ku, n_users, torch.zeros(n_batches, dtype=torch.int64, device=dev))
    ki = torch.cat([torch.where(ok, bid * n_items + pos, -1 - idx), torch.where(ok, bid * n_items + neg, -1 - n - idx)])
    si, _ = slots(ki, n_items, n_su)
    own = torch.stack([su, si[:n], si[n:]]).to(torch.int32).contiguous()
    return own, total[:-1].view(n_batches, stride), stride


class DeviceTripleBatcher:

    def __init__(self, users, pos_items, neg_items, batch_size, shuffle=True, generator=None):
        self.user_tensor = torch.as_tensor(users, dtype=torch.int64).contiguous()
        dev = self.user_tensor.device
        self.pos_item_tensor = torch.as_tensor(pos_items, dtype=torch.int64, device=dev).contiguous()
        self.neg_item_tensor = torch.as_tensor(neg_items, dtype=torch.int64, device=dev).contiguous()
        if not (len(self.user_tensor) == len(self.pos_item_tensor) == len(self.neg_item_tensor)):
            raise ValueError("users / pos_items / neg_items differ in length")
        self.batch_size = int(batch_size)
        self.shuffle = shuffle
        self.generator = generator

    def __len__(self):
        n = len(self.user_tensor)
        return (n + self.batch_size - 1) // self.batch_size

    def draw_seed(self):
        return int(torch.randint(0, 2**62, (1,)).item())

    def native_shuffle(self):
        return self.shuffle and self.generator is None and self.user_tensor.device.type == "cuda"

    def permutation(self):
        if not self.shuffle:
            return None
        n = len(self.user_tensor)
        dev = self.user_tensor.device
        if self.generator is not None:
            return torch.randperm(n, generator=self.generator).to(dev)
        if dev.type != "cuda":
            return torch.randperm(n)
        seed = self.draw_seed()
        perm = torch.empty(n, dtype=torch.int64, device=dev)
        _lib.check(_lib.load().hiprec_random_permutation(_lib.ptr(perm), n, seed, _lib.stream_ptr(dev)))
        return perm

    def __iter__(self):
        perm = self.permutation()
        n = len(self.user_tensor)
        for off in range(0, n, self.batch_size):
            if perm is None:
                sl = slice(off, min(off + self.batch_size, n))
                yield self.user_tensor[sl], self.pos_item_tensor[sl], self.neg_item_tensor[sl]
            else:
                idx = perm[off:off + self.batch_size]
                yield self.user_tensor[idx], self.pos_item_tensor[idx], self.neg_item_tensor[idx]


def _print_config_table(config, tag):
    print("-" * 80)
    print(tag)
    for k, v in config.items():
        print(f"  {k:<16} {v}")
    print("-" * 80)


class MFEngine(ModelEngine):

    ROWS_SGD_MIN_BYTES = 64 << 20
    SORT_MIN_BATCH = 256
    presorted = False
    fused_step = True

    def __init__(self, config):
        self.config = config
        _print_config_table(config["model"], tag="MF model config")
        self.model = MF(config["model"])
        self.reg = config["model"]["reg"] if "reg" in config else 0.0
        self.batch_size = config["model"]["batch_size"]
        super(MFEngine, self).__init__(config)
        self.model.to(self.device)
        self.loss = self.config["model"]["loss"] if "loss" in self.config["model"] else "bpr"
        print(f"using {self.loss} loss...")
        self._buffers_ready = False
        self._stamp = 1

    def _setup(self):
        lib = self.require_hip()
        if self._buffers_ready and self._g_flat.device == self.model.flat.device:
            return lib
        flat = self.model.flat
        dev = flat.device
        self._g_flat = torch.zeros_like(flat)
        self.optimizer.allocate_state(flat)
        self._scratch = torch.zeros(lib.hiprec_scratch_bytes(0), dtype=torch.uint8, device=dev)
        self._stats = _new_stats(dev, self.optimizer.beta1 or 0.9, self.optimizer.beta2 or 0.999)
        rows, self._owned_sgd = self._sgd_modes()
        self._rows_sgd = rows
        if rows:
            self._user_stamp = torch.zeros(self.model.n_users, dtype=torch.int32, device=dev)
            self._item_stamp = torch.zeros(self.model.n_items, dtype=torch.int32, device=dev)
        else:
            self._user_stamp = self._item_stamp = None
        mode = self.config["model"].get("dense_opt", "auto")
        if mode not in ("sweep", "lazy", "auto"):
            raise ValueError(f"dense_opt must be 'sweep', 'lazy' or 'auto', not {mode!r}")
        self._lazy = None
        if (self.optimizer.name != "sgd" and self.model.emb_dim <= 256 and self._lazy_capable
                and (mode == "lazy" or (mode == "auto" and flat.numel() * 4 >= self.ROWS_SGD_MIN_BYTES
                                        and _lib.lazy_betas_converge(self.optimizer)))):
            opt, m = self.optimizer, self.model
            lz = {"stamp_u": torch.full((m.n_users,), -1, dtype=torch.int32, device=dev),
                  "stamp_i": torch.full((m.n_items,), -1, dtype=torch.int32, device=dev),
                  "scalars": _lib.lazy_scalars_table(opt, dev), "dirty": False}
            lz["c"] = _lib.LazyState(
                flat.data_ptr(), self._g_flat.data_ptr(), opt.exp_avg.data_ptr() if opt.exp_avg is not None else None,
                opt.exp_avg_sq.data_ptr(), m.n_users, m.n_items, m.emb_dim, opt.kind, lz["stamp_u"].data_ptr(),
                lz["stamp_i"].data_ptr(), lz["scalars"].data_ptr(), _lib.LAZY_SCALARS_CAP, 0, opt.lr, opt.beta1,
                opt.beta2, opt.eps)
            self._lazy = lz
        self._buffers_ready = True
        return lib

    _lazy_capable = True

    def _epoch_flush(self):
        return bool(self.config["model"].get("lazy_epoch_flush", True))

    def flush_lazy(self):
        lz = getattr(self, "_lazy", None)
        if lz is not None and lz["dirty"]:
            _lib.check(_lib.load().hiprec_lazy_flush(ctypes.byref(lz["c"]), _lib.ptr(self._stats),
                                                     _lib.stream_ptr(self.model.flat.device)))
            lz["dirty"] = False

    def _lazy_mark_current(self):
        lz = getattr(self, "_lazy", None)
        if lz is not None:
            _lib.check(_lib.load().hiprec_lazy_mark_current(ctypes.byref(lz["c"]), _lib.ptr(self._stats),
                                                            _lib.stream_ptr(self.model.flat.device)))

    def _take_stamps(self, n):
        if self._stamp + n >= 2**31 - 1:
            self._user_stamp.zero_()
            self._item_stamp.zero_()
            self._stamp = 1
        first = self._stamp
        self._stamp += n
        return first

    def _as_index(self, t):
        return torch.as_tensor(t, device=self.device).to(torch.int64).contiguous()

    def _prepare_batch(self, batch_data):
        if self.loss == "bpr":
            users, a_items, third = (self._as_index(x) for x in batch_data)
        elif self.loss == "bce":
            users, a_items = (self._as_index(x) for x in batch_data[:2])
            third = torch.as_tensor(batch_data[2], device=self.device).to(torch.float32).contiguous()
        else:
            raise RuntimeError(
                f"Unsupported loss type {self.loss}, try other options: 'bpr' or 'bce'"
            )
        B = users.numel()
        if (B >= self.SORT_MIN_BATCH and not self.presorted and a_items.numel() == B
                and third.numel() == B):
            order = torch.argsort(a_items)
            users, a_items, third = users[order], a_items[order], third[order]
        if not (a_items.numel() == B and third.numel() == B):
            raise ValueError("batch tensors differ in length")
        if B == 0:
            raise ValueError("empty batch")
        if B == 1:
            raise IndexError("Dimension out of range (expected to be in range of [-1, 0], but got 1)")
        return users, a_items, third

    def _enqueue_grad(self, lib, users, a_items, third):
        m = self.model
        st = _lib.stream_ptr(m.flat.device)
        w, g = m.tables(), m.tables(self._g_flat)
        B = users.numel()
        fn = lib.hiprec_mf_bpr_grad if self.loss == "bpr" else lib.hiprec_mf_bce_grad
        _lib.check(fn(
            ctypes.byref(w), ctypes.byref(g), _lib.ptr(users), _lib.ptr(a_items), _lib.ptr(third),
            None, B, 1.0 / B, float(self.reg), _lib.ptr(self._stats), _lib.ptr(self._scratch),
            self._scratch.numel(), st))

    def _enqueue_step(self, batch_data):
        users, a_items, third = self._prepare_batch(batch_data)
        lib = self._setup()
        m = self.model
        st = _lib.stream_ptr(m.flat.device)
        self._enqueue_grad(lib, users, a_items, third)
        opt = self.optimizer
        if self._rows_sgd:
            w, g = m.tables(), m.tables(self._g_flat)
            b_items = third if self.loss == "bpr" else None
            _lib.check(lib.hiprec_mf_sgd_rows(
                ctypes.byref(w), ctypes.byref(g), _lib.ptr(users), _lib.ptr(a_items),
                _lib.ptr(b_items), None, users.numel(), opt.lr, _lib.ptr(self._user_stamp),
                _lib.ptr(self._item_stamp), self._take_stamps(1), _lib.ptr(self._stats),
                _lib.ptr(self._scratch), st))
        else:
            self.flush_lazy()
            _lib.check(lib.hiprec_opt_dense_step(
                opt.kind, _lib.ptr(m.flat), _lib.ptr(self._g_flat), _lib.ptr(opt.exp_avg),
                _lib.ptr(opt.exp_avg_sq), m.flat.numel(), opt.lr, opt.beta1, opt.beta2, opt.eps,
                _lib.ptr(self._stats), _lib.ptr(self._scratch), m.flat.numel() - 1, st))
            self._lazy_mark_current()

    def backward_only(self, batch_data):
        users, a_items, third = self._prepare_batch(batch_data)
        lib = self._setup()
        self._enqueue_grad(lib, users, a_items, third)
        g_global = self.model._views(self._g_flat)[4]
        _lib.check(lib.hiprec_finalize_stats(
            _lib.ptr(self._stats), _lib.ptr(self._scratch), _lib.ptr(g_global), None,
            _lib.stream_ptr(self.model.flat.device)))
        st = self._sync_stats()
        ue, ie, ub, ib, gb = (v.clone() for v in self.model._views(self._g_flat))
        self._g_flat.zero_()
        grads = {"global_bias": gb, "user_emb.weight": ue, "item_emb.weight": ie,
                 "user_bias.weight": ub, "item_bias.weight": ib}
        return st.loss, st.reg, grads

    def load_optimizer_state(self, step, exp_avg=None, exp_avg_sq=None):
        lib = self._setup()
        opt, m = self.optimizer, self.model
        dev = m.flat.device
        _lib.check(lib.hiprec_stats_reset(
            _lib.ptr(self._stats), opt.beta1 or 0.9, opt.beta2 or 0.999, _lib.stream_ptr(dev)))
        _lib.check(lib.hiprec_stats_set_step(_lib.ptr(self._stats), int(step), opt.beta1 or 0.9,
                                             opt.beta2 or 0.999, _lib.stream_ptr(dev)))
        for buf, src in ((opt.exp_avg, exp_avg), (opt.exp_avg_sq, exp_avg_sq)):
            if buf is None:
                continue
            if src is None:
                buf.zero_()
                continue
            ue, ie, ub, ib, gb = m._views(buf)
            for view, key in ((gb, "global_bias"), (ue, "user_emb.weight"), (ie, "item_emb.weight"),
                              (ub, "user_bias.weight"), (ib, "item_bias.weight")):
                view.copy_(torch.as_tensor(src[key], dtype=torch.float32).reshape(view.shape))
        if getattr(self, "_lazy", None) is not None:
            self._lazy["dirty"] = False
            self._lazy_mark_current()

    def optimizer_state(self):
        self._setup()
        self.flush_lazy()
        st = read_stats(self._stats)
        out = []
        for buf in (self.optimizer.exp_avg, self.optimizer.exp_avg_sq):
            if buf is None:
                out.append(None)
                continue
            ue, ie, ub, ib, gb = self.model._views(buf)
            out.append({"global_bias": gb.clone(), "user_emb.weight": ue.clone(),
                        "item_emb.weight": ie.clone(), "user_bias.weight": ub.clone(),
                        "item_bias.weight": ib.clone()})
        return st.step, out[0], out[1]

    def _sync_stats(self):
        st = read_stats(self._stats)
        if st.status:
            clear_status(self._stats)
            ob = getattr(self, "_owned_bufs", None)
            if ob is not None:
                ob["arrived"].zero_()
                ob["acc"].zero_()
            raise_on_status(st.status)
        return st

    def train_single_batch(self, batch_data):
        assert hasattr(self, "model"), "Please specify the exact model !"
        self._enqueue_step(batch_data)
        st = self._sync_stats()
        return st.loss, st.reg

    def _resident_triples(self, train_loader):
        seed = None
        if isinstance(train_loader, DeviceTripleBatcher):
            if (train_loader.native_shuffle() and train_loader.user_tensor.device == self.model.flat.device
                    and (train_loader.batch_size <= 8192 or self.loss == "bpr")):
                ds, perm, seed = train_loader, None, train_loader.draw_seed()
            else:
                ds, perm = train_loader, train_loader.permutation()
        elif (self.loss == "bce" and len(getattr(train_loader, "tensors", ())) == 3
              and train_loader.tensors[2].is_floating_point() and hasattr(train_loader, "permutation")):
            class _Rating:
                user_tensor, item_tensor, target_tensor = train_loader.tensors

            ds, perm = _Rating, train_loader.permutation()
        else:
            ds = getattr(train_loader, "dataset", None)
            names = (("user_tensor", "pos_item_tensor", "neg_item_tensor") if self.loss == "bpr"
                     else ("user_tensor", "item_tensor", "target_tensor"))
            if ds is None or not all(hasattr(ds, a) for a in names):
                return None
            if getattr(train_loader, "drop_last", False) or train_loader.batch_sampler is None:
                return None
            torch.empty((), dtype=torch.int64).random_()
            order = list(iter(train_loader.sampler))
            perm = torch.as_tensor(order, dtype=torch.int64)
        dev = self.device
        users = ds.user_tensor.to(dev, torch.int64).contiguous()
        if self.loss == "bpr":
            pos = ds.pos_item_tensor.to(dev, torch.int64).contiguous()
            neg = ds.neg_item_tensor.to(dev, torch.int64).contiguous()
        else:
            pos = ds.item_tensor.to(dev, torch.int64).contiguous()
            neg = ds.target_tensor.to(dev, torch.float32).contiguous()
        perm = None if perm is None else perm.to(dev).contiguous()
        bs = int(train_loader.batch_size)
        if bs <= 8192 and dev.type == "cuda":
            ou, op, on = torch.empty_like(users), torch.empty_like(pos), torch.empty_like(neg)
            self._stage_into(users, pos, neg, perm, seed, bs, ou, op, on)
            return ou, op, on, None, bs
        if dev.type == "cuda" and self.loss == "bpr" and users.numel() > 0 and bs >= self.SORT_MIN_BATCH:
            lib, n = _lib.load(), users.numel()
            n_batches = (n + bs - 1) // bs
            shuffle = 1 if seed is not None else 0
            ws_ints = lib.hiprec_stage_grouped_ws_ints(n, bs, self.model.n_items)
            if ws_ints > 0 and self.config["model"].get("stage_big_batches", "grouped") == "grouped":
                ws = self._stage_ws = _lib.grow(getattr(self, "_stage_ws", None), ws_ints, torch.int32, dev)
                ou, op, on = torch.empty_like(users), torch.empty_like(pos), torch.empty_like(neg)
                _lib.check(lib.hiprec_stage_epoch_grouped(
                    _lib.ptr(users), _lib.ptr(pos), _lib.ptr(neg), _lib.ptr(perm), shuffle, seed or 0, n, bs,
                    self.model.n_items, _lib.ptr(ws), _lib.ptr(ou), _lib.ptr(op), _lib.ptr(on), _lib.stream_ptr(dev)))
                return ou, op, on, None, bs
            small = n_batches * self.model.n_items < 2**31
            keys = torch.empty(n, dtype=torch.int32 if small else torch.int64, device=dev)
            _lib.check(lib.hiprec_stage_sort_keys(_lib.ptr(pos), _lib.ptr(perm), shuffle, seed or 0, n, bs,
                                                  self.model.n_items, 4 if small else 8, _lib.ptr(keys),
                                                  _lib.stream_ptr(dev)))
            order = torch.sort(keys, stable=False).indices
            ou, op, on = torch.empty_like(users), torch.empty_like(pos), torch.empty_like(neg)
            _lib.check(lib.hiprec_gather_epoch(
                _lib.ptr(users), _lib.ptr(pos), _lib.ptr(neg), _lib.ptr(perm), shuffle, seed or 0, _lib.ptr(order), n,
                _lib.ptr(ou), _lib.ptr(op), _lib.ptr(on), _lib.stream_ptr(dev)))
            return ou, op, on, None, bs
        if seed is not None and perm is None:
            perm = torch.empty(users.numel(), dtype=torch.int64, device=dev)
            _lib.check(_lib.load().hiprec_random_permutation(_lib.ptr(perm), perm.numel(), seed, _lib.stream_ptr(dev)))
        if bs >= self.SORT_MIN_BATCH:
            perm = sort_within_batches(perm, pos, bs, self.model.n_items)
        if perm is not None:
            users, pos, neg, perm = users[perm], pos[perm], neg[perm], None
        return users, pos, neg, perm, bs

    def _stage_into(self, users, pos, neg, perm, seed, bs, ou, op, on):
        lib, dev = _lib.load(), users.device
        if seed is not None:
            _lib.check(lib.hiprec_stage_epoch_shuffled(
                _lib.ptr(users), _lib.ptr(pos), _lib.ptr(neg), neg.element_size(), seed, users.numel(), bs,
                _lib.ptr(ou), _lib.ptr(op), _lib.ptr(on), _lib.stream_ptr(dev)))
        else:
            _lib.check(lib.hiprec_stage_epoch(
                _lib.ptr(users), _lib.ptr(pos), _lib.ptr(neg), neg.element_size(), _lib.ptr(perm),
                users.numel(), bs, _lib.ptr(ou), _lib.ptr(op), _lib.ptr(on), _lib.stream_ptr(dev)))

    def _can_prefetch(self, train_loader):
        return (isinstance(train_loader, DeviceTripleBatcher) and self.loss == "bpr"
                and train_loader.native_shuffle()
                and train_loader.user_tensor.device == self.model.flat.device
                and len(train_loader.user_tensor) > 0)

    def prefetch_epoch(self, train_loader):
        if not self._can_prefetch(train_loader):
            return False
        self._drop_prefetch()
        dev = self.model.flat.device
        main = torch.cuda.current_stream(dev)
        pf = getattr(self, "_pf", None)
        if pf is None or pf["dev"] != dev:
            pf = self._pf = {"dev": dev, "side": torch.cuda.Stream(dev), "slots": [None, None], "next": 0}
        begin = getattr(self, "_ev_epoch_begin", None)
        if begin is not None:
            pf["side"].wait_event(begin)
        else:
            pf["side"].wait_stream(main)
        bs = train_loader.batch_size
        if bs <= 8192:
            users, pos, neg = train_loader.user_tensor, train_loader.pos_item_tensor, train_loader.neg_item_tensor
            k = pf["next"]
            pf["next"] = 1 - k
            slot = pf["slots"][k]
            if slot is None or slot[0].numel() != users.numel():
                with torch.cuda.stream(pf["side"]):
                    slot = pf["slots"][k] = tuple(torch.empty_like(t) for t in (users, pos, neg))
            seed = train_loader.draw_seed()
            with torch.cuda.stream(pf["side"]):
                self._stage_into(users, pos, neg, None, seed, bs, *slot)
                prepared = self._finish_staging(slot + (None, bs))
        else:
            with torch.cuda.stream(pf["side"]):
                prepared = self._finish_staging(self._resident_triples(train_loader))
            for t in prepared[:3]:
                t.record_stream(main)
        with torch.cuda.stream(pf["side"]):
            done = torch.cuda.Event()
            done.record(pf["side"])
        if prepared.own is not None:
            for t in prepared.own:
                if torch.is_tensor(t):
                    t.record_stream(main)
        self._prefetched = (train_loader, done, prepared, self._loader_fingerprint(train_loader))
        return True

    @staticmethod
    def _loader_fingerprint(train_loader):
        ts = (train_loader.user_tensor, train_loader.pos_item_tensor, train_loader.neg_item_tensor)
        return tuple((t.data_ptr(), t.numel(), t._version) for t in ts) + (int(train_loader.batch_size),)

    def _drop_prefetch(self):
        pending = getattr(self, "_prefetched", None)
        if pending is not None:
            torch.cuda.current_stream(self.model.flat.device).wait_event(pending[1])
            self._prefetched = None

    def prepare_epoch(self, train_loader):
        pending = getattr(self, "_prefetched", None)
        if pending is not None:
            self._prefetched = None
            torch.cuda.current_stream(self.model.flat.device).wait_event(pending[1])
            if pending[0] is train_loader and pending[3] == self._loader_fingerprint(train_loader):
                return pending[2]
        if self.loss not in ("bpr", "bce") or isinstance(train_loader, (list, tuple)):
            return None
        if self.loss == "bce" and isinstance(train_loader, DeviceTripleBatcher):
            return None
        return self._finish_staging(self._resident_triples(train_loader))

    def _sgd_modes(self):
        mode = self.config["model"].get("sgd_mode", "auto")
        big = self.model.flat.numel() * 4 >= self.ROWS_SGD_MIN_BYTES
        rows = self.optimizer.name == "sgd" and (mode in ("rows", "owned", "owned_atomic") or (mode == "auto" and big))
        return rows, rows and mode in ("owned", "owned_atomic", "auto") and self.model.emb_dim <= 256

    def _finish_staging(self, staged):
        if staged is None:
            return None
        owned = (self._sgd_modes()[1] or self._lazy_owned()) and self.loss == "bpr"
        if getattr(staged, "own", None) is not None:
            if not owned:
                staged.own = None
            return staged
        prepared = PreparedEpoch(staged)
        users, pos, neg, perm, bs = prepared
        if owned and perm is None and users.device.type == "cuda":
            small_keys = self.model.n_users + self.model.n_items < 2**31
            if self._sgd_modes()[1] and self._owned_form() == "pull" and small_keys:
                prepared.own = batch_row_contributions(users, pos, neg, bs, self.model.n_users, self.model.n_items,
                                                       self.model.emb_dim)
            elif self._lazy_owned() == "pull" and small_keys:
                prepared.own = batch_row_contributions(users, pos, neg, bs, self.model.n_users, self.model.n_items,
                                                       self.model.emb_dim, every_row=True)
            else:
                prepared.own = batch_row_ownership(users, pos, neg, bs, self.model.n_users, self.model.n_items)
        return prepared

    def _owned_form(self):
        return "atomic" if self.config["model"].get("sgd_mode", "auto") == "owned_atomic" else "pull"

    def _lazy_owned(self):
        if self.model.flat.device.type != "cuda" or self.optimizer.name == "sgd":
            return False
        self._setup()
        mode = self.config["model"].get("lazy_grad", "pull")
        if mode not in ("pull", "owned", "atomic"):
            raise ValueError(f"lazy_grad must be 'pull', 'owned' or 'atomic', not {mode!r}")
        if self._lazy is None or mode == "atomic" or self.loss != "bpr":
            return False
        if mode == "pull" and self.model.emb_dim % 4 == 0:
            return "pull"
        return "owned"

    def _fused_ok(self, perm):
        return (self.fused_step and not self._rows_sgd and self.loss == "bpr" and perm is None
                and self.model.emb_dim <= 256)

    def _run_fused_epoch(self, lib, users, pos, neg, n_run, bs, steps=None):
        m, opt = self.model, self.optimizer
        dev = m.flat.device
        if getattr(self, "_fused_bufs", None) is None or self._fused_bufs["dev"] != dev:
            self._fused_bufs = {
                "dev": dev, "w_alt": torch.empty_like(m.flat),
                "m_alt": torch.empty_like(m.flat) if opt.exp_avg is not None else None,
                "v_alt": torch.empty_like(m.flat) if opt.exp_avg_sq is not None else None,
                "g": [self._g_flat, torch.zeros_like(m.flat), torch.zeros_like(m.flat)],
                "scratch": [torch.zeros_like(self._scratch), torch.zeros_like(self._scratch)],
            }
        fb = self._fused_bufs
        fb["g"][0] = self._g_flat

        def pair(primary, alt):
            return None if primary is None else (ctypes.c_void_p * 2)(primary.data_ptr(), alt.data_ptr())

        w_arr = pair(m.flat, fb["w_alt"])
        m_arr = pair(opt.exp_avg, fb["m_alt"])
        v_arr = pair(opt.exp_avg_sq, fb["v_alt"])
        g_arr = (ctypes.c_void_p * 3)(*(t.data_ptr() for t in fb["g"]))
        s_arr = (ctypes.c_void_p * 2)(*(t.data_ptr() for t in fb["scratch"]))
        final = ctypes.c_int32(-1)
        n_steps = (n_run + bs - 1) // bs
        a, b = (0, n_steps) if steps is None else steps
        _lib.check(lib.hiprec_mf_bpr_epoch_fused_range(
            opt.kind, w_arr, g_arr, m_arr, v_arr, s_arr, m.n_users, m.n_items, m.emb_dim,
            _lib.ptr(users), _lib.ptr(pos), _lib.ptr(neg), n_run, bs, a, b, float(self.reg), opt.lr,
            opt.beta1, opt.beta2, opt.eps, _lib.ptr(self._stats), ctypes.byref(final),
            _lib.stream_ptr(dev)))
        if final.value == 1:
            m.flat.copy_(fb["w_alt"])
            if opt.exp_avg is not None:
                opt.exp_avg.copy_(fb["m_alt"])
            if opt.exp_avg_sq is not None:
                opt.exp_avg_sq.copy_(fb["v_alt"])

    def run_prepared_epoch(self, prepared, sync=True, prefetch=None, steps=None):
        lib = self._setup()
        users, pos, neg, perm, bs = prepared
        n = users.numel()
        n_run = n - 1 if n % bs == 1 else n
        if steps is not None:
            n_steps = (n_run + bs - 1) // bs
            if not (0 <= steps[0] <= steps[1] <= n_steps):
                raise ValueError(f"steps {steps} outside the epoch's {n_steps} steps")
            if sync:
                raise ValueError("a partial epoch cannot be read back: pass sync=False")
        if steps is None or steps[0] == 0:
            self._begin_epoch_marker(prepared, prefetch)
        if self._owned_sgd and self.loss == "bpr" and getattr(prepared, "own", None) is not None:
            self._run_owned_epoch(lib, prepared, n_run, steps)
            if not sync:
                return None
            st = self._sync_stats()
            if n_run != n:
                raise IndexError(
                    "Dimension out of range (expected to be in range of [-1, 0], but got 1)")
            return st
        if self._lazy is not None and perm is None and self.loss in ("bpr", "bce"):
            self._run_lazy_epoch(lib, users, pos, neg, n_run, bs, steps, getattr(prepared, "own", None))
            if not sync:
                return None
            st = self._sync_stats()
            if n_run != n:
                raise IndexError(
                    "Dimension out of range (expected to be in range of [-1, 0], but got 1)")
            return st
        if self._fused_ok(perm):
            self._run_fused_epoch(lib, users, pos, neg, n_run, bs, steps)
            if not sync:
                return None
            st = self._sync_stats()
            if n_run != n:
                raise IndexError(
                    "Dimension out of range (expected to be in range of [-1, 0], but got 1)")
            return st
        if steps is not None:
            a, b = steps[0] * bs, min(steps[1] * bs, n_run)
            users, pos, neg, n_run = users[a:b], pos[a:b], neg[a:b], b - a
            perm = None if perm is None else perm[a:b]
        return self._run_unfused_epoch(lib, users, pos, neg, perm, bs, n, n_run, sync)

    def _run_lazy_epoch(self, lib, users, items_a, third, n_run, bs, steps, own=None):
        m, lz = self.model, self._lazy
        n_steps = (n_run + bs - 1) // bs
        a, b = (0, n_steps) if steps is None else steps
        lo, hi = a * bs, min(b * bs, n_run)
        w, g = m.tables(), m.tables(self._g_flat)
        el = third.element_size()
        lz["dirty"] = True
        if isinstance(own, RowContributions) and self.loss == "bpr" and self._lazy_owned() == "pull":
            cidx, rows, counts, row_cap = own
            n_all = cidx.shape[1]
            cap = 3 * min(bs, max(n_all, 1))
            pb = getattr(self, "_pull_bufs", None)
            if pb is None or pb["dev"] != m.flat.device or pb["cap"] < cap:
                pb = self._pull_bufs = {
                    "dev": m.flat.device, "cap": cap,
                    "cbuf": torch.empty(cap * m.emb_dim, dtype=torch.float32, device=m.flat.device),
                    "cbias": torch.empty(cap, dtype=torch.float32, device=m.flat.device),
                    "scratch": torch.zeros_like(self._scratch)}
            _lib.check(lib.hiprec_mf_epoch_lazy_pull(
                ctypes.byref(lz["c"]), ctypes.c_void_p(users.data_ptr() + 8 * lo),
                ctypes.c_void_p(items_a.data_ptr() + 8 * lo), ctypes.c_void_p(third.data_ptr() + 8 * lo),
                ctypes.c_void_p(cidx.data_ptr() + 4 * lo), n_all, ctypes.c_void_p(rows.data_ptr() + 16 * a * row_cap),
                row_cap, ctypes.c_void_p(counts.data_ptr() + 16 * a), _lib.ptr(pb["cbuf"]), _lib.ptr(pb["cbias"]),
                hi - lo, bs, 1 if a == 0 else 0, float(self.reg), _lib.ptr(self._stats), _lib.ptr(self._scratch),
                _lib.stream_ptr(m.flat.device)))
            if b == n_steps and self._epoch_flush():
                self.flush_lazy()
            return
        if own is not None and not isinstance(own, RowContributions) and self.loss == "bpr" and self._lazy_owned():
            o, total, stride = own
            _lib.check(lib.hiprec_mf_epoch_lazy_owned(
                ctypes.byref(lz["c"]), ctypes.c_void_p(users.data_ptr() + 8 * lo),
                ctypes.c_void_p(items_a.data_ptr() + 8 * lo), ctypes.c_void_p(third.data_ptr() + 8 * lo),
                ctypes.c_void_p(o[0].data_ptr() + 4 * lo), ctypes.c_void_p(o[1].data_ptr() + 4 * lo),
                ctypes.c_void_p(o[2].data_ptr() + 4 * lo), ctypes.c_void_p(total.data_ptr() + 4 * a * stride), stride,
                hi - lo, bs, 1 if a == 0 else 0, float(self.reg), _lib.ptr(self._stats), _lib.ptr(self._scratch),
                _lib.stream_ptr(m.flat.device)))
            if b == n_steps and self._epoch_flush():
                self.flush_lazy()
            return
        _lib.check(lib.hiprec_mf_epoch_lazy(
            ctypes.byref(lz["c"]), ctypes.byref(w), ctypes.byref(g), ctypes.c_void_p(users.data_ptr() + 8 * lo),
            ctypes.c_void_p(items_a.data_ptr() + 8 * lo), ctypes.c_void_p(third.data_ptr() + el * lo),
            0 if self.loss == "bpr" else 1, hi - lo, bs, 1 if a == 0 else 0, float(self.reg), _lib.ptr(self._stats),
            _lib.ptr(self._scratch), self._scratch.numel(), _lib.stream_ptr(m.flat.device)))
        if b == n_steps and self._epoch_flush():
            self.flush_lazy()

    def _run_owned_epoch(self, lib, prepared, n_run, steps):
        users, pos, neg, _, bs = prepared
        if isinstance(prepared.own, RowContributions):
            return self._run_pull_epoch(lib, prepared, n_run, steps)
        own, total, stride = prepared.own
        m = self.model
        dev = m.flat.device
        ob = getattr(self, "_owned_bufs", None)
        if ob is None or ob["dev"] != dev or ob["stride"] < stride:
            ob = self._owned_bufs = {
                "dev": dev, "stride": stride,
                "arrived": torch.zeros(stride, dtype=torch.int32, device=dev),
                "acc": torch.zeros(stride * (m.emb_dim + 1), dtype=torch.float32, device=dev),
                "gb": torch.zeros(2, dtype=torch.float32, device=dev),
                "scratch": [torch.zeros_like(self._scratch), torch.zeros_like(self._scratch)]}
        s_arr = (ctypes.c_void_p * 2)(*(t.data_ptr() for t in ob["scratch"]))
        n_steps = (n_run + bs - 1) // bs
        a, b = (0, n_steps) if steps is None else steps
        _lib.check(lib.hiprec_mf_bpr_epoch_owned(
            _lib.ptr(m.flat), m.n_users, m.n_items, m.emb_dim, _lib.ptr(users), _lib.ptr(pos), _lib.ptr(neg),
            _lib.ptr(own[0]), _lib.ptr(own[1]), _lib.ptr(own[2]), _lib.ptr(total), stride,
            _lib.ptr(ob["arrived"]), _lib.ptr(ob["acc"]), ob["stride"], _lib.ptr(ob["gb"]), s_arr, n_run, bs,
            a, b, float(self.reg), self.optimizer.lr, _lib.ptr(self._stats), _lib.stream_ptr(dev)))

    def _run_pull_epoch(self, lib, prepared, n_run, steps):
        users, pos, neg, _, bs = prepared
        cidx, rows, counts, row_cap = prepared.own
        m = self.model
        dev = m.flat.device
        n = users.numel()
        cap = 3 * min(bs, max(n, 1))
        pb = getattr(self, "_pull_bufs", None)
        if pb is None or pb["dev"] != dev or pb["cap"] < cap:
            pb = self._pull_bufs = {
                "dev": dev, "cap": cap,
                "cbuf": torch.empty(cap * m.emb_dim, dtype=torch.float32, device=dev),
                "cbias": torch.empty(cap, dtype=torch.float32, device=dev),
                "scratch": torch.zeros_like(self._scratch)}
        n_steps = (n_run + bs - 1) // bs
        a, b = (0, n_steps) if steps is None else steps
        _lib.check(lib.hiprec_mf_bpr_epoch_pull(
            _lib.ptr(m.flat), m.n_users, m.n_items, m.emb_dim, _lib.ptr(users), _lib.ptr(pos), _lib.ptr(neg),
            _lib.ptr(cidx), n, _lib.ptr(rows), row_cap, _lib.ptr(counts), _lib.ptr(pb["cbuf"]), _lib.ptr(pb["cbias"]),
            _lib.ptr(pb["scratch"]), n_run, bs, a, b, float(self.reg), self.optimizer.lr, _lib.ptr(self._stats),
            _lib.stream_ptr(dev)))

    def _begin_epoch_marker(self, prepared, prefetch):
        self._ev_epoch_begin = torch.cuda.Event()
        self._ev_epoch_begin.record(torch.cuda.current_stream(self.model.flat.device))
        self._epoch_inputs = prepared
        if prefetch is not None:
            self.prefetch_epoch(prefetch)

    def _run_unfused_epoch(self, lib, users, pos, neg, perm, bs, n, n_run, sync):
        m, opt = self.model, self.optimizer
        w, g = m.tables(), m.tables(self._g_flat)
        n_batches = (n_run + bs - 1) // bs
        first = self._take_stamps(n_batches) if self._rows_sgd else 0
        epoch_fn = lib.hiprec_mf_bpr_epoch if self.loss == "bpr" else lib.hiprec_mf_bce_epoch
        _lib.check(epoch_fn(
            ctypes.byref(w), ctypes.byref(g), _lib.ptr(users), _lib.ptr(pos), _lib.ptr(neg),
            _lib.ptr(perm), n_run, bs, float(self.reg), opt.kind, opt.lr, opt.beta1, opt.beta2,
            opt.eps, _lib.ptr(m.flat), _lib.ptr(self._g_flat), _lib.ptr(opt.exp_avg),
            _lib.ptr(opt.exp_avg_sq), m.flat.numel(), _lib.ptr(self._user_stamp),
            _lib.ptr(self._item_stamp), first, _lib.ptr(self._stats),
            _lib.ptr(self._scratch), self._scratch.numel(), _lib.stream_ptr(m.flat.device)))
        if not sync:
            return None
        st = self._sync_stats()
        if n_run != n:
            raise IndexError(
                "Dimension out of range (expected to be in range of [-1, 0], but got 1)")
        return st

    def epoch_stats(self):
        return self._sync_stats()

    @timeit
    def train_an_epoch(self, train_loader, epoch_id):
        assert hasattr(self, "model"), "Please specify the exact model !"
        self.model.train()
        lib = self._setup()
        prepared = self.prepare_epoch(train_loader)
        if prepared is not None:
            ahead = train_loader if self.config["model"].get("prefetch_epoch", True) else None
            self.run_prepared_epoch(prepared, sync=False, prefetch=ahead)
            n, bs = prepared[0].numel(), prepared[4]
            st = self._sync_stats()
            if n % bs == 1:
                raise IndexError("Dimension out of range (expected to be in range of [-1, 0], but got 1)")
        else:
            _lib.check(lib.hiprec_stats_begin_epoch(
                _lib.ptr(self._stats), _lib.stream_ptr(self.model.flat.device)))
            for batch_data in train_loader:
                self._enqueue_step(batch_data)
            st = self._sync_stats()
        loss, total_loss, regularizer = st.loss, st.loss_sum, st.reg_sum
        print(f"[Training Epoch {epoch_id}], Loss {loss}, Regularizer {regularizer}")
        self.writer.add_scalar("model/loss", total_loss, epoch_id)
        self.writer.add_scalar("model/regularizer", regularizer, epoch_id)
```

include/hiprec.h:

```cpp
#ifndef HIPREC_H
#define HIPREC_H

#include <stddef.h>
#include <stdint.h>

#ifdef __cplusplus
extern "C" {
#endif

#define HIPREC_VERSION 100

#define HIPREC_E_BADARG (-1)
#define HIPREC_E_SCRATCH (-2)
#define HIPREC_E_UNSUPPORTED (-3)

#define HIPREC_STATUS_USER_OOB 1u
#define HIPREC_STATUS_ITEM_OOB 2u
#define HIPREC_STATUS_ROW_OOB 4u
#define HIPREC_STATUS_ROUTE_OVERFLOW 8u
#define HIPREC_STATUS_NEG_EXHAUSTED 16u
#define HIPREC_STATUS_LAZY_TABLE 32u
#define HIPREC_STATUS_TABLE_FULL 64u

#define HIPREC_OPT_SGD 0
#define HIPREC_OPT_ADAM 1
#define HIPREC_OPT_RMSPROP 2
#define HIPREC_OPT_RMSPROP_MOMENTUM 3

typedef struct hiprec_mf_tables {
  float* user_emb;
  float* item_emb;
  float* user_bias;
  float* item_bias;
  float* global_bias;
  int64_t n_users;
  int64_t n_items;
  int32_t dim;
  int32_t _pad;
} hiprec_mf_tables;

typedef struct hiprec_stats {
  float loss;
  float reg;
  double loss_sum;
  double reg_sum;
  int64_t step;
  double beta1;
  double beta2;
  double beta1_pow;
  double beta2_pow;
  uint32_t status;
  uint32_t _pad;
} hiprec_stats;

int hiprec_version(void);
const char* hiprec_source_hash(void);
const char* hiprec_last_error(void);
size_t hiprec_stats_bytes(void);
size_t hiprec_scratch_bytes(int64_t batch);
int hiprec_stats_reset(hiprec_stats* stats, double beta1, double beta2, void* stream);
int hiprec_stats_advance_step(hiprec_stats* stats, void* stream);
int hiprec_stats_set_step(hiprec_stats* stats, int64_t step, double beta1, double beta2, void* stream);
int hiprec_stats_begin_epoch(hiprec_stats* stats, void* stream);

int hiprec_gather_rows(const float* table, int64_t n_rows, int32_t dim, const int64_t* idx,
                       int64_t n, float* out, hiprec_stats* stats, void* stream);

int hiprec_route_bucket(const int64_t* keys, int64_t n, int32_t n_dest, int64_t cap, int32_t* counts,
                        int64_t* slot_out, hiprec_stats* stats, void* stream);

int hiprec_shard_route_triples(const int64_t* users, const int64_t* pos, const int64_t* neg, int64_t n,
                               int32_t n_dest, int64_t cap, int32_t* counts, int64_t* send,
                               hiprec_stats* stats, void* stream);
int hiprec_shard_route_items(const int64_t* recv, int64_t n_slots, int32_t n_dest, int64_t cap,
                             int32_t* counts, int64_t* req, int64_t* slot_pos, int64_t* slot_neg,
                             int64_t* u_loc, hiprec_stats* stats, void* stream);
int hiprec_shard_gather_payload(const float* item_emb, const float* item_bias, int64_t n_rows,
                                int32_t dim, const int64_t* incoming, int64_t n, int32_t n_dest,
                                float* payload, int64_t* local_idx, hiprec_stats* stats, void* stream);
int hiprec_shard_split_rows(const float* src, int64_t n, int32_t dim, float* emb, float* bias,
                            void* stream);
int hiprec_shard_join_rows(const float* emb, const float* bias, int64_t n, int32_t dim, float* dst,
                           void* stream);

int hiprec_scatter_add_rows(float* table, int64_t n_rows, int32_t dim, const int64_t* idx,
                            const float* src, int64_t src_stride, int64_t n, hiprec_stats* stats,
                            void* stream);

int hiprec_mf_predict(const hiprec_mf_tables* w, const int64_t* users, const int64_t* items,
                      int64_t n, float* scores, hiprec_stats* stats, void* stream);
int hiprec_mf_forward(const hiprec_mf_tables* w, const int64_t* users, const int64_t* items, int64_t n, float* scores,
                      float* sq, hiprec_stats* stats, void* stream);

int hiprec_mf_bpr_grad(const hiprec_mf_tables* w, const hiprec_mf_tables* g, const int64_t* users,
                       const int64_t* pos, const int64_t* neg, const int64_t* perm, int64_t batch,
                       float inv_batch, float reg_coef, hiprec_stats* stats, void* scratch,
                       size_t scratch_bytes, void* stream);

int hiprec_mf_bce_grad(const hiprec_mf_tables* w, const hiprec_mf_tables* g, const int64_t* users,
                       const int64_t* items, const float* ratings, const int64_t* perm,
                       int64_t batch, float inv_batch, float reg_coef, hiprec_stats* stats,
                       void* scratch, size_t scratch_bytes, void* stream);

int hiprec_finalize_stats(hiprec_stats* stats, const void* scratch, float* g_scalar,
                          float* loss_reg_out, void* stream);

int hiprec_opt_dense_step(int kind, float* w, float* g, float* m, float* v, int64_t n, double lr,
                          double beta1, double beta2, double eps, hiprec_stats* stats,
                          const void* scratch, int64_t scalar_index, void* stream);

int hiprec_mf_sgd_rows(const hiprec_mf_tables* w, const hiprec_mf_tables* g, const int64_t* users,
                       const int64_t* items_a, const int64_t* items_b, const int64_t* perm,
                       int64_t batch, double lr, int32_t* user_stamp, int32_t* item_stamp,
                       int32_t stamp, hiprec_stats* stats, const void* scratch, void* stream);

int hiprec_random_permutation(int64_t* out, int64_t n, uint64_t seed, void* stream);

int hiprec_stage_epoch(const int64_t* users, const int64_t* items, const void* third,
                       int32_t third_bytes, const int64_t* perm, int64_t n, int64_t batch,
                       int64_t* out_users, int64_t* out_items, void* out_third, void* stream);
int hiprec_stage_epoch_shuffled(const int64_t* users, const int64_t* items, const void* third,
                                int32_t third_bytes, uint64_t seed, int64_t n, int64_t batch,
                                int64_t* out_users, int64_t* out_items, void* out_third, void* stream);

int hiprec_mf_bpr_epoch(const hiprec_mf_tables* w, const hiprec_mf_tables* g, const int64_t* users,
                        const int64_t* pos, const int64_t* neg, const int64_t* perm,
                        int64_t n_triples, int64_t batch, float reg_coef, int kind, double lr,
                        double beta1,
                        double beta2, double eps, float* flat_w, float* flat_g, float* flat_m,
                        float* flat_v, int64_t n_flat, int32_t* user_stamp, int32_t* item_stamp,
                        int32_t first_stamp, hiprec_stats* stats, void* scratch,
                        size_t scratch_bytes, void* stream);

int hiprec_mf_bce_epoch(const hiprec_mf_tables* w, const hiprec_mf_tables* g, const int64_t* users,
                        const int64_t* items, const float* ratings, const int64_t* perm,
                        int64_t n_samples, int64_t batch, float reg_coef, int kind, double lr,
                        double beta1, double beta2, double eps, float* flat_w, float* flat_g,
                        float* flat_m, float* flat_v, int64_t n_flat, int32_t* user_stamp,
                        int32_t* item_stamp, int32_t first_stamp, hiprec_stats* stats,
                        void* scratch, size_t scratch_bytes, void* stream);

int hiprec_mf_bpr_epoch_fused(int kind, float* const* w_flat, float* const* g_flat,
                              float* const* m_flat, float* const* v_flat, void* const* scratch2,
                              int64_t n_users, int64_t n_items, int32_t dim, const int64_t* users,
                              const int64_t* pos, const int64_t* neg, int64_t n_triples,
                              int64_t batch, float reg_coef, double lr, double beta1, double beta2,
                              double eps, hiprec_stats* stats, int32_t* final_index, void* stream);
int hiprec_mf_bpr_epoch_fused_range(int kind, float* const* w_flat, float* const* g_flat,
                                    float* const* m_flat, float* const* v_flat, void* const* scratch2,
                                    int64_t n_users, int64_t n_items, int32_t dim, const int64_t* users,
                                    const int64_t* pos, const int64_t* neg, int64_t n_triples,
                                    int64_t batch, int64_t step_begin, int64_t step_end, float reg_coef,
                                    double lr, double beta1, double beta2, double eps, hiprec_stats* stats,
                                    int32_t* final_index, void* stream);
int hiprec_mf_bpr_dp_epoch_fused_range(int kind, float* const* w_flat, float* const* bufs, int64_t scratch_floats,
                                       float* const* m_flat, float* const* v_flat, int64_t n_flat, int64_t n_users,
                                       int64_t n_items, int32_t dim, const int64_t* users, const int64_t* pos,
                                       const int64_t* neg, int64_t n_triples, int64_t batch, int64_t step_begin,
                                       int64_t step_end, int32_t world, float reg_coef, double lr, double beta1,
                                       double beta2, double eps, hiprec_stats* stats, void* all_reduce_fn,
                                       void* comm, int32_t* final_index, void* stream);

int hiprec_mf_bpr_epoch_owned(float* w_flat, int64_t n_users, int64_t n_items, int32_t dim,
                              const int64_t* users, const int64_t* pos, const int64_t* neg,
                              const int32_t* own_u, const int32_t* own_p, const int32_t* own_n,
                              const int32_t* total, int64_t total_stride,
                              int32_t* arrived, float* acc, int64_t n_slots, float* gb_pingpong,
                              void* const* scratch2, int64_t n_triples, int64_t batch,
                              int64_t step_begin, int64_t step_end, float reg_coef, double lr,
                              hiprec_stats* stats, void* stream);

int32_t hiprec_ownership_table_bits(int64_t batch);
int64_t hiprec_ownership_ws_ints(int64_t n, int64_t batch, int32_t table_bits);
int hiprec_batch_row_ownership(const int64_t* users, const int64_t* pos, const int64_t* neg, int64_t n,
                               int64_t batch, int64_t n_users, int64_t n_items, int32_t table_bits,
                               int32_t* ws, int32_t* total, int32_t* own, void* stream);

int64_t hiprec_stage_grouped_ws_ints(int64_t n, int64_t batch, int64_t n_items);
int hiprec_stage_epoch_grouped(const int64_t* users, const int64_t* pos, const int64_t* neg, const int64_t* perm,
                               int32_t shuffle, uint64_t seed, int64_t n, int64_t batch, int64_t n_items, int32_t* ws,
                               int64_t* users_out, int64_t* pos_out, int64_t* neg_out, void* stream);

int32_t hiprec_mf_pull_chunk(int32_t dim);
int64_t hiprec_contrib_row_cap(int64_t batch, int32_t min_contrib);
int hiprec_batch_row_contrib(const int64_t* users, const int64_t* pos, const int64_t* neg, int64_t n, int64_t batch,
                             int64_t n_users, int64_t n_items, int32_t table_bits, int32_t chunk, int32_t min_contrib,
                             int32_t* ws, int32_t* cidx, int32_t* rows, int64_t row_cap, int32_t* counts, void* stream);
int hiprec_mf_bpr_epoch_pull(float* w_flat, int64_t n_users, int64_t n_items, int32_t dim, const int64_t* users,
                             const int64_t* pos, const int64_t* neg, const int32_t* cidx, int64_t cidx_stride,
                             const int32_t* rows, int64_t row_cap, const int32_t* counts, float* cbuf, float* cbias,
                             void* scratch,
                             int64_t n_triples, int64_t batch, int64_t step_begin, int64_t step_end, float reg_coef,
                             double lr, hiprec_stats* stats, void* stream);

int hiprec_mf_bpr_owned_remote_step(float* w_flat, int64_t n_users, int64_t n_items_local, int32_t dim,
                                    const float* fetched, float* g_send, int64_t n_slots, const int64_t* users,
                                    const int64_t* pos_slot, const int64_t* neg_slot, const int32_t* own_u,
                                    const int32_t* own_p, const int32_t* own_n, const int32_t* total,
                                    int32_t* arrived, float* acc, int64_t batch, float inv_batch, float reg_coef,
                                    double lr, hiprec_stats* stats, void* scratch, void* stream);
int hiprec_shard_publish_partials(const void* scratch, float* g_send, int32_t dim, const int64_t* extra_rows,
                                  int32_t n_dest, void* stream);
int hiprec_shard_apply_rows(float* item_emb, float* item_bias, int64_t n_rows, int32_t dim, const int64_t* idx,
                            const float* g_recv, int64_t n, double lr, hiprec_stats* stats, void* stream);
int hiprec_shard_finish_step(const float* g_recv, int32_t dim, const int64_t* extra_rows, int32_t n_src,
                             float* global_bias, double lr, int32_t first_of_epoch, hiprec_stats* stats,
                             void* stream);

int hiprec_batch_row_ownership_tables(const int64_t* users, const int64_t* pos, const int64_t* neg, int64_t n,
                                      int64_t batch, int64_t n_users, int64_t n_items, int32_t table_bits,
                                      int32_t* ws, int32_t* total, int32_t* own, int32_t* tab_keys, int32_t* pos_cnt,
                                      int32_t* occ, void* stream);
int hiprec_stage_sort_keys(const int64_t* items, const int64_t* perm, int32_t shuffle, uint64_t seed, int64_t n,
                           int64_t batch, int64_t n_items, int32_t key_bytes, void* keys, void* stream);
int hiprec_gather_epoch(const int64_t* users, const int64_t* pos, const int64_t* neg, const int64_t* perm,
                        int32_t shuffle, uint64_t seed, const int64_t* order, int64_t n, int64_t* users_out,
                        int64_t* pos_out, int64_t* neg_out, void* stream);
int hiprec_group_epoch_by_item(const int64_t* users, const int64_t* pos, const int64_t* neg, int64_t n, int64_t batch,
                               int64_t n_users, int32_t table_bits, const int32_t* own, const int32_t* occ,
                               const int32_t* tab_keys, int32_t* pos_cnt, int32_t* invalid_cnt, int64_t* users_out,
                               int64_t* pos_out, int64_t* neg_out, int32_t* own_out, void* stream);
int64_t hiprec_plan_route_tiles(int64_t n, int64_t batch);
int hiprec_plan_route_triples(const int64_t* users, const int64_t* pos, const int64_t* neg, const int64_t* perm,
                              int64_t n, int64_t batch, int32_t world, int64_t n_users, int64_t n_items,
                              int32_t* tile_ws, int32_t* cnt_ds, int32_t* send, hiprec_stats* stats, void* stream);
int hiprec_plan_place_triples(const int32_t* recv, int64_t n_recv, const int32_t* recv_cnt, int32_t world,
                              int64_t n_steps, int64_t cap, int32_t* group_ws, int64_t* users, int64_t* pos,
                              int64_t* neg, void* stream);
int64_t hiprec_plan_slot_ws_ints(int64_t n_steps, int32_t table_bits, int32_t world);
int hiprec_plan_item_slots(const int64_t* users, int64_t n_steps, int64_t cap, int32_t world, int64_t n_users_local,
                           int32_t table_bits, const int32_t* own, const int32_t* occ, const int32_t* tab_keys,
                           int32_t* pos_cnt, int32_t* ws, int32_t* slot_of, int32_t* req_cnt, int32_t* req_ds,
                           int32_t* ex_req, int32_t* n_slots, int32_t* send_base, int32_t* req_send,
                           int64_t* users_out, int64_t* pos_slot, int64_t* neg_slot, int32_t* own_out,
                           const int32_t* total, uint8_t* slot_shared, int64_t slot_stride, const int32_t* step_fill,
                           void* stream);
int hiprec_plan_place_requests(const int32_t* incoming, int64_t n_in, const int32_t* in_cnt, int32_t world,
                               int64_t n_steps, int32_t* group_ws, int32_t* in_idx, int32_t* step_off,
                               int32_t* extra_pos, int64_t n_rows_local, uint32_t* dup_ws, void* stream);

int hiprec_mf_bpr_pull_remote_step(float* w_flat, int64_t n_users, int64_t n_items_local, int32_t dim,
                                   const float* fetched, float* g_send, int64_t n_slots, const int64_t* users,
                                   const int64_t* pos_slot, const int64_t* neg_slot, const int32_t* cidx_u,
                                   const int32_t* cidx_p, const int32_t* cidx_n, const int32_t* rows, int64_t row_cap,
                                   const int32_t* counts, float* cbuf, float* cbias, const int32_t* extra_rows,
                                   int32_t n_dest, int64_t batch, float inv_batch, float reg_coef, double lr,
                                   hiprec_stats* stats, void* scratch, void* stream);
int hiprec_shard_payload_zero(const float* item_emb, const float* item_bias, int64_t n_rows, int32_t dim,
                              const int32_t* idx, int64_t n, int64_t self_lo, int64_t self_hi, float* payload,
                              float* self_dst, float* zero, int64_t zero_floats, const uint8_t* shared,
                              hiprec_stats* stats, void* stream);
int hiprec_mf_bpr_grad_remote_step(const float* w_flat, float* g_flat, int64_t n_users, int64_t n_items_local,
                                   int32_t dim, const float* fetched, float* g_send, int64_t n_slots,
                                   const int64_t* users, const int64_t* pos_slot, const int64_t* neg_slot,
                                   const int32_t* own_u, const int32_t* own_p, const int32_t* own_n,
                                   const int32_t* total, int64_t batch, float inv_batch, float reg_coef,
                                   hiprec_stats* stats, void* scratch, void* stream);
int hiprec_shard_apply_finish(float* t_emb, float* t_bias, int64_t n_rows, int32_t dim, const int32_t* idx,
                              const float* g_recv, int64_t n, int64_t self_lo, int64_t self_hi, const float* g_self,
                              double coef, const int32_t* extra_pos, int32_t n_src, float* scalar_target,
                              double scalar_coef, int32_t first_of_epoch, const uint32_t* dup_bits, hiprec_stats* stats,
                              void* stream);

typedef struct hiprec_shard_plan {
  int32_t world, rank;
  int64_t n_steps, cap;
  int64_t local_batch, n_local;
  const int64_t* users;
  const int64_t* pos_slot;
  const int64_t* neg_slot;
  const int32_t* own;
  const int32_t* total;
  int64_t total_stride;
  const int32_t* in_idx;
  const int32_t* ex_req;
  const int32_t* ex_in;
  const int64_t* in_off_host;
  const int64_t* n_slots_host;
  const int64_t* req_cnt_host;
  const int64_t* in_cnt_host;
  const uint8_t* slot_shared;
  int64_t slot_stride;
  const uint32_t* dup_bits;
  int64_t dup_words;
  const int32_t* cidx;
  const int32_t* rows;
  int64_t row_cap;
  const int32_t* counts;
} hiprec_shard_plan;

typedef struct hiprec_shard_bufs {
  float* w_flat;
  int64_t n_users_local, n_items_local;
  int32_t dim, _pad;
  float* payload;
  float* g_recv;
  float* fetched;
  float* g_send;
  int32_t* arrived;
  float* acc;
  void* scratch;
  float* g_flat;
  float* m_flat;
  float* v_flat;
  int32_t* stamp_u;
  int32_t* stamp_i;
  float* lazy_scalars;
// ... 484 lines not shown
```

Before: 373.2 million triples/s.

## Add row-owner BPR step with per-row staged interaction records

Adds a staging pass that groups each batch's triples by embedding row (user/item) into per-row records with inline entries, hot-row headers, and tail lists. A new rows kernel then has one wave own each row, recompute that row's triple scores, accumulate its gradient locally and apply the optimizer in place. This removes scatter/atomic gradient accumulation and the separate dense optimizer pass. In exchange it needs a large per-epoch staging buffer, recomputes dot products from both sides, and adds dispatch logic for an 'auto' mode.

Result: no change. 374.2 million triples/s (median of 3 runs) (+0.3%).

```diff
diff --git a/beta-recsys_amd/_lib.py b/beta-recsys_amd/_lib.py
--- a/beta-recsys_amd/_lib.py
+++ b/beta-recsys_amd/_lib.py
@@ -398,6 +398,13 @@
     "hiprec_mf_bpr_epoch_fused_range": (
         c_int,
         [c_int, _P, _P, _P, _P, _P, c_int64, c_int64, c_int32, _P, _P, _P, c_int64, c_int64, c_int64, c_int64,
+         c_float, c_double, c_double, c_double, c_double, _P, POINTER(c_int32), _P],
+    ),
+    "hiprec_mf_rows_layout": (c_int, [c_int64, c_int64, c_int64, c_int64, POINTER(c_int64)]),
+    "hiprec_stage_rows": (c_int, [_P, _P, _P, c_int64, c_int64, c_int64, c_int64, _P, c_int64, _P]),
+    "hiprec_mf_bpr_epoch_rows_range": (
+        c_int,
+        [c_int, _P, _P, _P, _P, c_int64, c_int64, c_int32, _P, c_int64, c_int64, c_int64, c_int64, c_int64, c_int64,
          c_float, c_double, c_double, c_double, c_double, _P, POINTER(c_int32), _P],
     ),
     "hiprec_mf_bpr_dp_epoch_fused_range": (
diff --git a/beta-recsys_amd/csrc/common.hpp b/beta-recsys_amd/csrc/common.hpp
--- a/beta-recsys_amd/csrc/common.hpp
+++ b/beta-recsys_amd/csrc/common.hpp
@@ -70,6 +70,31 @@
   int bits = 2;
   while (bits < 62 && (1ull << bits) < n) ++bits;
   return (bits + 1) / 2;
+}
+
+constexpr int kRowRecInts = 32;
+constexpr int kRowInline = 15;
+constexpr int kRowHdrInts = 8;
+constexpr int kRowHotInts = 8;
+constexpr int kRowKeyPosBits = 13;
+constexpr int64_t kRowMaxTable = (1ll << 19) - 1;
+
+struct RowRecLayout {
+  int64_t n_batches, rows, max_hot, hdr_stride, tail_stride, rec_off, hdr_off, tail_off, total;
+};
+
+inline RowRecLayout row_rec_layout(int64_t n_users, int64_t n_items, int64_t n_triples, int64_t batch) {
+  RowRecLayout l{};
+  l.n_batches = batch > 0 ? (n_triples + batch - 1) / batch : 0;
+  l.rows = n_users + n_items;
+  l.max_hot = 3 * batch / (kRowInline + 1) + 1;
+  l.hdr_stride = (kRowHdrInts + kRowHotInts * l.max_hot + 31) / 32 * 32;
+  l.tail_stride = 3 * batch * 2;
+  l.rec_off = 0;
+  l.hdr_off = l.rec_off + l.n_batches * l.rows * kRowRecInts;
+  l.tail_off = l.hdr_off + l.n_batches * l.hdr_stride;
+  l.total = l.tail_off + l.n_batches * l.tail_stride;
+  return l;
 }
 
 #if defined(__HIPCC__)
diff --git a/beta-recsys_amd/csrc/mf.hip b/beta-recsys_amd/csrc/mf.hip
--- a/beta-recsys_amd/csrc/mf.hip
+++ b/beta-recsys_amd/csrc/mf.hip
@@ -500,6 +500,376 @@
     }
     scratch->partials[blockIdx.x] = make_float4(l * inv_batch, r * inv_batch, b, 0.f);
     if (blockIdx.x == 0) scratch->n_partials = static_cast<uint32_t>(f.n_gather_blocks);
+  }
+}
+
+constexpr int kRowsHotBlocks = 32;
+constexpr int kRowsSlots = 7;
+constexpr int kRowsMaxUserBlocks = kRowsSlots * kWave - kRowsHotBlocks;
+constexpr int kRowsMaxItemBlocks = 4096;
+constexpr int kRowsHotTrip = 4;
+constexpr int kRowsState = kMaxBlocks - 2;
+
+struct RowsOpt {
+  int64_t n_users, n_items;
+  int32_t dim, max_hot;
+  int64_t batch_cap;
+  const float* w_read;
+  float* w_write;
+  float* m;
+  float* v;
+  const int32_t* rec;
+  const int32_t* hdr;
+  const int32_t* tail;
+  OptScalars s;
+  int n_user_blocks, n_item_blocks;
+  int n_prev_partials;
+  int apply_prev;
+  const Scratch* scratch_prev;
+};
+
+__device__ __forceinline__ float4 load_f4_vector(const float4* p) {
+  int vzero = 0;
+  asm volatile("" : "+v"(vzero));
+  return p[vzero];
+}
+
+__device__ __forceinline__ float readlane_f32(float v, int l) {
+  return __builtin_bit_cast(float, __builtin_amdgcn_readlane(__builtin_bit_cast(int, v), l));
+}
+
+template <int KIND>
+__device__ __forceinline__ void next_step_scalars(const OptScalars& s, const hiprec_stats* stats, float* step_size,
+                                                  float* bc2_sqrt) {
+  *step_size = s.lr;
+  *bc2_sqrt = 1.f;
+  if constexpr (KIND == HIPREC_OPT_ADAM) {
+    const double bc1 = 1.0 - stats->beta1_pow * stats->beta1;
+    const double bc2 = 1.0 - stats->beta2_pow * stats->beta2;
+    *step_size = static_cast<float>(s.lr_d / bc1);
+    *bc2_sqrt = static_cast<float>(sqrt(bc2));
+  }
+}
+
+struct RowsAcc {
+  float g, gbias;
+  float loss, reg, gb;
+};
+
+template <int T, bool USER>
+__device__ __forceinline__ void rows_chunk(const float* __restrict__ wf, int D, int lane, int n_users, int n_items,
+                                           uint32_t o_ie, uint32_t o_ub, uint32_t o_ib, int ea, int eb,
+                                           int n, int n0, float own, float b_own, float gb, float inv_batch, float ru,
+                                           float ri, RowsAcc& acc) {
+  const int cc = lane < D ? lane : D - 1;
+  const bool in = lane < D;
+  const int a_max = (USER ? n_items : n_users) - 1, b_max = n_items - 1;
+  ea = min(max(ea, 0), a_max);
+  eb = min(max(eb, 0), b_max);
+  const bool act = lane < n;
+  const bool first = lane < n0;
+  float bx = 0.f, by = 0.f;
+  if (act) {
+    bx = wf[(USER ? o_ib : o_ub) + ea];
+    by = wf[o_ib + eb];
+  }
+  for (int base = 0; base < n; base += T) {
+    float X[T], Y[T];
+#pragma unroll
+    for (int j = 0; j < T; ++j) {
+      const int e = base + j;
+      X[j] = Y[j] = 0.f;
+      if (e < n) {
+        const uint32_t ra = __builtin_amdgcn_readlane(ea, e), rb = __builtin_amdgcn_readlane(eb, e);
+        X[j] = wf[(USER ? o_ie : 0u) + ra * D + cc];
+        Y[j] = wf[o_ie + rb * D + cc];
+      }
+    }
+    float vdp = 0.f, vdn = 0.f;
+#pragma unroll
+    for (int j = 0; j < T; ++j) {
+      const int e = base + j;
+      if (e < n) {
+        const float x = in ? X[j] : 0.f, y = in ? Y[j] : 0.f;
+        X[j] = x;
+        Y[j] = y;
+        float dp, dn;
+        if (USER) {
+          dp = own * x;
+          dn = own * y;
+        } else if (e < n0) {
+          dp = x * own;
+          dn = x * y;
+        } else {
+          dp = x * y;
+          dn = x * own;
+        }
+        dp = wave_sum(dp);
+        dn = wave_sum(dn);
+        if (lane == e) {
+          vdp = dp;
+          vdn = dn;
+        }
+      }
+    }
+    const bool mine = act && lane >= base && lane < base + T;
+    const float bu = USER ? b_own : bx;
+    const float bp = USER ? bx : (first ? b_own : by);
+    const float bn = USER ? by : (first ? by : b_own);
+    const float yp = sigmoid_f32(((vdp + bu) + bp) + gb);
+    const float yn = sigmoid_f32(((vdn + bu) + bn) + gb);
+    float sig_neg_x;
+    const float nls = neg_logsigmoid(yp - yn, &sig_neg_x);
+    const float delta = -sig_neg_x * inv_batch;
+    const float dpos = mine ? delta * ((1.f - yp) * yp) : 0.f;
+    const float dneg = mine ? -delta * ((1.f - yn) * yn) : 0.f;
+    if (USER) {
+      acc.loss += mine ? nls : 0.f;
+      acc.gb += dpos + dneg;
+      acc.reg += mine ? 2.f * bu * bu + bp * bp + bn * bn : 0.f;
+    }
+#pragma unroll
+    for (int j = 0; j < T; ++j) {
+      const int e = base + j;
+      if (e < n) {
+        const float dpe = readlane_f32(dpos, e), dne = readlane_f32(dneg, e);
+        if (USER) {
+          acc.g += (dpe * X[j] + dne * Y[j]) + ru * own;
+          acc.gbias += (dpe + dne) + ru * b_own;
+          acc.reg += 2.f * own * own + X[j] * X[j] + Y[j] * Y[j];
+        } else {
+          const float d = e < n0 ? dpe : dne;
+          acc.g += d * X[j] + ri * own;
+          acc.gbias += d + ri * b_own;
+        }
+      }
+    }
+  }
+}
+
+template <int KIND>
+__global__ __launch_bounds__(kAggBlock) __attribute__((amdgpu_waves_per_eu(8, 8))) void mf_bpr_rows_kernel(RowsOpt f, float inv_batch, float reg_coef,
+                                                                hiprec_stats* stats, Scratch* scratch) {
+  __shared__ float s_part[kAggWaves][kWave + 1];
+  __shared__ float s_loss[kAggWaves], s_reg[kAggWaves], s_gbv[kAggWaves];
+  constexpr bool kHasM = KIND == HIPREC_OPT_ADAM;
+  constexpr bool kHasV = KIND != HIPREC_OPT_SGD;
+  const int lane = lane_id();
+  const int wv = wave_in_block();
+  const int D = f.dim;
+  const int b = static_cast<int>(blockIdx.x);
+  const int U = static_cast<int>(f.n_users), I = static_cast<int>(f.n_items);
+  const uint32_t o_ie = static_cast<uint32_t>(U) * D, o_ub = o_ie + static_cast<uint32_t>(I) * D, o_ib = o_ub + U;
+  const float* const wf = f.w_read;
+  const bool apply = f.apply_prev != 0;
+  const float4* const pv = f.scratch_prev->partials;
+
+  if (b == kRowsHotBlocks + f.n_user_blocks + f.n_item_blocks) {
+    const float gb_part = finalize_partials<kAggBlock>(stats, f.scratch_prev);
+    if (threadIdx.x == 0) {
+      const float4 st0 = pv[kRowsState], st1 = pv[kRowsState + 1];
+      float gw = st0.x, gg = gb_part, gm = st0.y, gv = st0.z;
+      if (apply) opt_update<KIND>(gw, gg, gm, gv, f.s, st1.x, st1.y);
+      const int bad = f.hdr[1];
+      if (bad) atomicOr(&stats->status, static_cast<uint32_t>(bad) & (HIPREC_STATUS_USER_OOB | HIPREC_STATUS_ITEM_OOB));
+      advance_step(stats);
+      float ss, bq;
+      next_step_scalars<KIND>(f.s, stats, &ss, &bq);
+      scratch->partials[kRowsState] = make_float4(gw, gm, gv, 0.f);
+      scratch->partials[kRowsState + 1] = make_float4(st1.z, st1.w, ss, bq);
+      scratch->n_partials = static_cast<uint32_t>(f.n_user_blocks + kRowsHotBlocks);
+    }
+    return;
+  }
+
+  float gbz[kRowsSlots];
+#pragma unroll
+  for (int j = 0; j < kRowsSlots; ++j) gbz[j] = pv[lane + kWave * j].z;
+  const float4 st0 = load_f4_vector(pv + kRowsState), st1 = load_f4_vector(pv + kRowsState + 1);
+  const float step_size = KIND == HIPREC_OPT_ADAM ? st1.z : f.s.lr;
+  const float bc2_sqrt = KIND == HIPREC_OPT_ADAM ? st1.w : 1.f;
+  float gb = st0.x;
+  {
+    float gbp = 0.f;
+#pragma unroll
+    for (int j = 0; j < kRowsSlots; ++j) gbp += lane + kWave * j < f.n_prev_partials ? gbz[j] : 0.f;
+    if (apply) {
+      float gg = wave_sum(gbp), gm = st0.y, gv = st0.z;
+      opt_update<KIND>(gb, gg, gm, gv, f.s, st1.x, st1.y);
+    }
+  }
+  const float ru = 4.f * reg_coef * inv_batch, ri = 2.f * reg_coef * inv_batch;
+  const int cc = lane < D ? lane : D - 1;
+  RowsAcc acc{0.f, 0.f, 0.f, 0.f, 0.f};
+  int slot = -1;
+
+  if (b < kRowsHotBlocks) {
+    slot = f.n_user_blocks + b;
+    const int n_hot = min(max(f.hdr[0], 0), f.max_hot);
+    const int cap = static_cast<int>(f.batch_cap);
+    for (int h = b; h < n_hot; h += kRowsHotBlocks) {
+      const int32_t* q = f.hdr + kRowHdrInts + kRowHotInts * h;
+      const int row = min(max(q[0], 0), U + I - 1);
+      const int c0 = min(max(q[1], 0), cap), c1 = min(max(q[2], 0), cap);
+      const int lo0 = min(max(q[3], 0), cap - c0), lo1 = min(max(q[4], 0), cap - c1);
+      const bool user = row < U;
+      const uint32_t r = user ? row : row - U;
+      const uint32_t orow = (user ? 0u : o_ie) + r * D, obias = (user ? o_ub : o_ib) + r;
+      const int32_t* tail_a = f.tail + (user ? 0 : 2 * f.batch_cap);
+      const int32_t* tail_b = f.tail + 4 * f.batch_cap;
+      const int cnt = c0 + c1, per = (cnt + kAggWaves - 1) / kAggWaves;
+      const int e0 = min(wv * per, cnt), e1 = min(e0 + per, cnt);
+      const float w_own = wf[orow + cc], b_own = wf[obias];
+      const float own = lane < D ? w_own : 0.f;
+      acc.g = acc.gbias = 0.f;
+      for (int cb = e0; cb < e1; cb += kWave) {
+        const int n = min(kWave, e1 - cb);
+        const int e = cb + lane;
+        int ea = 0, eb = 0;
+        if (lane < n) {
+          const int2 ent = *reinterpret_cast<const int2*>(e < c0 ? tail_a + 2 * (lo0 + e) : tail_b + 2 * (lo1 + e - c0));
+          ea = ent.x;
+          eb = ent.y;
+        }
+        const int n0 = min(max(c0 - cb, 0), n);
+        if (user)
+          rows_chunk<kRowsHotTrip, true>(wf, D, lane, U, I, o_ie, o_ub, o_ib, ea, eb, n, n0, own, b_own, gb,
+                              inv_batch, ru, ri, acc);
+        else
+          rows_chunk<kRowsHotTrip, false>(wf, D, lane, U, I, o_ie, o_ub, o_ib, ea, eb, n, n0, own, b_own, gb,
+                               inv_batch, ru, ri, acc);
+      }
+      s_part[wv][lane] = acc.g;
+      if (lane == 0) s_part[wv][kWave] = acc.gbias;
+      lds_barrier();
+      if (wv == 0) {
+        float g = 0.f, gbias = 0.f;
+#pragma unroll
+        for (int w = 0; w < kAggWaves; ++w) {
+          g += s_part[w][lane];
+          gbias += s_part[w][kWave];
+        }
+        float wn = w_own, m = 0.f, v = 0.f, bw = b_own, bm = 0.f, bv = 0.f;
+        if constexpr (kHasM) {
+          m = f.m[orow + cc];
+          bm = f.m[obias];
+        }
+        if constexpr (kHasV) {
+          v = f.v[orow + cc];
+          bv = f.v[obias];
+        }
+        opt_update<KIND>(wn, g, m, v, f.s, step_size, bc2_sqrt);
+        opt_update<KIND>(bw, gbias, bm, bv, f.s, step_size, bc2_sqrt);
+        if (lane < D) {
+          f.w_write[orow + lane] = wn;
+          if constexpr (kHasM) f.m[orow + lane] = m;
+          if constexpr (kHasV) f.v[orow + lane] = v;
+        }
+        if (lane == 0) {
+          f.w_write[obias] = bw;
+          if constexpr (kHasM) f.m[obias] = bm;
+          if constexpr (kHasV) f.v[obias] = bv;
+        }
+      }
+      lds_barrier();
+    }
+  } else {
+    const int rb = b - kRowsHotBlocks;
+    const bool user = rb < f.n_user_blocks;
+    if (user) slot = rb;
+    const int n_role = user ? U : I;
+    const int first = (user ? rb : rb - f.n_user_blocks) * kAggWaves + wv;
+    const int stride = (user ? f.n_user_blocks : f.n_item_blocks) * kAggWaves;
+    for (int r = first; r < n_role; r += stride) {
+      const uint32_t orow = (user ? 0u : o_ie) + static_cast<uint32_t>(r) * D, obias = (user ? o_ub : o_ib) + r;
+      const int rw = f.rec[static_cast<uint32_t>((user ? 0 : U) + r) * kRowRecInts + (lane & (kRowRecInts - 1))];
+      float w = wf[orow + cc], bw = wf[obias], m = 0.f, v = 0.f, bm = 0.f, bv = 0.f;
+      if constexpr (kHasM) {
+        m = f.m[orow + cc];
+        bm = f.m[obias];
+      }
+      if constexpr (kHasV) {
+        v = f.v[orow + cc];
+        bv = f.v[obias];
+      }
+      const int c0 = __builtin_amdgcn_readlane(rw, 0), c1 = __builtin_amdgcn_readlane(rw, 1);
+      const int cnt = c0 + c1;
+      if (cnt > kRowInline || c0 < 0 || c1 < 0) continue;
+      acc.g = acc.gbias = 0.f;
+      if (cnt > 0) {
+        const int ea = __shfl(rw, 2 + 2 * lane), eb = __shfl(rw, 3 + 2 * lane);
+        const float own = lane < D ? w : 0.f;
+        if (user)
+          rows_chunk<4, true>(wf, D, lane, U, I, o_ie, o_ub, o_ib, ea, eb, cnt, c0, own, bw, gb,
+                              inv_batch, ru, ri, acc);
+        else
+          rows_chunk<4, false>(wf, D, lane, U, I, o_ie, o_ub, o_ib, ea, eb, cnt, c0, own, bw, gb,
+                               inv_batch, ru, ri, acc);
+      }
+      float g = acc.g, gbias = acc.gbias;
+      opt_update<KIND>(w, g, m, v, f.s, step_size, bc2_sqrt);
+      opt_update<KIND>(bw, gbias, bm, bv, f.s, step_size, bc2_sqrt);
+      if (lane < D) {
+        f.w_write[orow + lane] = w;
+        if constexpr (kHasM) f.m[orow + lane] = m;
+        if constexpr (kHasV) f.v[orow + lane] = v;
+      }
+      if (lane == 0) {
+        f.w_write[obias] = bw;
+        if constexpr (kHasM) f.m[obias] = bm;
+        if constexpr (kHasV) f.v[obias] = bv;
+      }
+    }
+  }
+  if (slot < 0) return;
+  const float l_w = wave_sum(acc.loss), r_w = wave_sum(acc.reg), g_w = wave_sum(acc.gb);
+  if (lane == 0) {
+    s_loss[wv] = l_w;
+    s_reg[wv] = r_w;
+    s_gbv[wv] = g_w;
+  }
+  lds_barrier();
+  if (threadIdx.x == 0) {
+    float l = 0.f, r = 0.f, g = 0.f;
+#pragma unroll
+    for (int i = 0; i < kAggWaves; ++i) {
+      l += s_loss[i];
+      r += s_reg[i];
+      g += s_gbv[i];
+    }
+    scratch->partials[slot] = make_float4(l * inv_batch, r * inv_batch, g, 0.f);
+  }
+}
+
+template <int KIND, bool FLUSH>
+__global__ __launch_bounds__(kAggBlock) void mf_bpr_rows_edge_kernel(RowsOpt f, float* w_final, hiprec_stats* stats,
+                                                                     Scratch* sc, Scratch* sc_other) {
+  const int64_t o_gb = (f.n_users + f.n_items) * (static_cast<int64_t>(f.dim) + 1);
+  if constexpr (FLUSH) {
+    const float gb_part = finalize_partials<kAggBlock>(stats, sc);
+    if (threadIdx.x == 0) {
+      const float4 st0 = sc->partials[kRowsState], st1 = sc->partials[kRowsState + 1];
+      float gw = st0.x, gg = gb_part, gm = st0.y, gv = st0.z;
+      if (sc->n_partials > 0) opt_update<KIND>(gw, gg, gm, gv, f.s, st1.x, st1.y);
+      w_final[o_gb] = gw;
+      if constexpr (KIND == HIPREC_OPT_ADAM) f.m[o_gb] = gm;
+      if constexpr (KIND != HIPREC_OPT_SGD) f.v[o_gb] = gv;
+      sc->n_partials = 0;
+      sc_other->n_partials = 0;
+    }
+  } else {
+    if (threadIdx.x == 0) {
+      stats->loss_sum = 0.0;
+      stats->reg_sum = 0.0;
+      float ss, bq;
+      next_step_scalars<KIND>(f.s, stats, &ss, &bq);
+      float gm = 0.f, gv = 0.f;
+      if constexpr (KIND == HIPREC_OPT_ADAM) gm = f.m[o_gb];
+      if constexpr (KIND != HIPREC_OPT_SGD) gv = f.v[o_gb];
+      sc->partials[kRowsState] = make_float4(f.w_read[o_gb], gm, gv, 0.f);
+      sc->partials[kRowsState + 1] = make_float4(0.f, 0.f, ss, bq);
+      sc->n_partials = 0;
+    }
   }
 }
 
@@ -1053,6 +1423,96 @@
   return hiprec_mf_bpr_epoch_fused_range(kind, w_flat, g_flat, m_flat, v_flat, scratch2, n_users, n_items, dim,
                                          users, pos, neg, n_triples, batch, 0, n_steps, reg_coef, lr, beta1,
                                          beta2, eps, stats, final_index, stream);
+}
+
+template <int KIND>
+static int rows_range(const RowsOpt& base, float* const* w_flat, void* const* scratch2, const int32_t* records,
+                      const RowRecLayout& L, int64_t n_triples, int64_t batch, int64_t step_begin, int64_t step_end,
+                      int64_t n_steps, float reg_coef, hiprec_stats* stats, hipStream_t st) {
+  RowsOpt f = base;
+  if (step_begin == 0) {
+    f.w_read = w_flat[0];
+    mf_bpr_rows_edge_kernel<KIND, false><<<1, kAggBlock, 0, st>>>(f, nullptr, stats, static_cast<Scratch*>(scratch2[1]),
+                                                                  nullptr);
+    HIPREC_TRY(hipGetLastError());
+  }
+  const int grid = kRowsHotBlocks + f.n_user_blocks + f.n_item_blocks + 1;
+  for (int64_t k = step_begin; k < step_end; ++k) {
+    const int64_t b = std::min<int64_t>(batch, n_triples - k * batch);
+    f.w_read = w_flat[k & 1];
+    f.w_write = w_flat[(k + 1) & 1];
+    f.rec = records + L.rec_off + k * L.rows * kRowRecInts;
+    f.hdr = records + L.hdr_off + k * L.hdr_stride;
+    f.tail = records + L.tail_off + k * L.tail_stride;
+    f.n_prev_partials = k > 0 ? f.n_user_blocks + kRowsHotBlocks : 0;
+    f.apply_prev = k > 0 ? 1 : 0;
+    f.scratch_prev = static_cast<const Scratch*>(scratch2[(k + 1) & 1]);
+    mf_bpr_rows_kernel<KIND><<<grid, kAggBlock, 0, st>>>(f, 1.0f / static_cast<float>(b), reg_coef, stats,
+                                                        static_cast<Scratch*>(scratch2[k & 1]));
+    HIPREC_TRY(hipGetLastError());
+  }
+  if (step_end == n_steps && n_steps > 0) {
+    mf_bpr_rows_edge_kernel<KIND, true><<<1, kAggBlock, 0, st>>>(f, w_flat[n_steps & 1], stats,
+                                                                 static_cast<Scratch*>(scratch2[(n_steps + 1) & 1]),
+                                                                 static_cast<Scratch*>(scratch2[n_steps & 1]));
+    HIPREC_TRY(hipGetLastError());
+  }
+  return 0;
+}
+
+extern "C" int hiprec_mf_bpr_epoch_rows_range(int kind, float* const* w_flat, float* m_flat, float* v_flat,
+                                              void* const* scratch2, int64_t n_users, int64_t n_items, int32_t dim,
+                                              const int32_t* records, int64_t records_ints, int64_t records_triples,
+                                              int64_t n_triples, int64_t batch, int64_t step_begin, int64_t step_end,
+                                              float reg_coef, double lr, double beta1, double beta2, double eps,
+                                              hiprec_stats* stats, int32_t* final_index, void* stream) {
+  HIPREC_REQUIRE(w_flat && scratch2 && final_index && stats, "NULL pointer");
+  HIPREC_REQUIRE(w_flat[0] && w_flat[1] && scratch2[0] && scratch2[1], "NULL buffer");
+  HIPREC_REQUIRE(kind == HIPREC_OPT_SGD || kind == HIPREC_OPT_ADAM || kind == HIPREC_OPT_RMSPROP,
+                 "unknown optimizer kind %d", kind);
+  const bool has_m = kind == HIPREC_OPT_ADAM, has_v = kind != HIPREC_OPT_SGD;
+  HIPREC_REQUIRE(!has_m || m_flat, "Adam needs m_flat");
+  HIPREC_REQUIRE(!has_v || v_flat, "Adam/RMSprop need v_flat");
+  HIPREC_REQUIRE(n_users > 0 && n_items > 0 && dim > 0, "bad table sizes");
+  HIPREC_REQUIRE(dim <= kWave && n_users <= kRowMaxTable && n_items <= kRowMaxTable && batch <= 8192,
+                 "the owner-recomputes step needs dim <= 64, tables of at most %lld rows and batches up to 8192",
+                 (long long)kRowMaxTable);
+  HIPREC_REQUIRE(n_triples >= 0 && batch > 0 && records_triples >= n_triples, "bad n_triples/batch");
+  const int64_t n_steps = (n_triples + batch - 1) / batch;
+  HIPREC_REQUIRE(0 <= step_begin && step_begin <= step_end && step_end <= n_steps,
+                 "bad step range [%lld, %lld) of %lld", (long long)step_begin, (long long)step_end, (long long)n_steps);
+  const RowRecLayout L = row_rec_layout(n_users, n_items, records_triples, batch);
+  HIPREC_REQUIRE(n_triples == 0 || (records && records_ints >= L.total), "records missing or too small");
+  RowsOpt f{};
+  f.n_users = n_users;
+  f.n_items = n_items;
+  f.dim = dim;
+  f.max_hot = static_cast<int32_t>(L.max_hot);
+  f.batch_cap = batch;
+  f.m = has_m ? m_flat : nullptr;
+  f.v = has_v ? v_flat : nullptr;
+  f.s = OptScalars{lr,
+                   static_cast<float>(lr),
+                   static_cast<float>(beta2),
+                   static_cast<float>(1.0 - beta1),
+                   static_cast<float>(1.0 - beta2),
+                   static_cast<float>(eps)};
+  f.n_user_blocks = static_cast<int>(std::min<int64_t>((n_users + kAggWaves - 1) / kAggWaves, kRowsMaxUserBlocks));
+  f.n_item_blocks = static_cast<int>(std::min<int64_t>((n_items + kAggWaves - 1) / kAggWaves, kRowsMaxItemBlocks));
+  hipStream_t st = static_cast<hipStream_t>(stream);
+  int rc;
+  if (kind == HIPREC_OPT_SGD)
+    rc = rows_range<HIPREC_OPT_SGD>(f, w_flat, scratch2, records, L, n_triples, batch, step_begin, step_end, n_steps,
+                                    reg_coef, stats, st);
+  else if (kind == HIPREC_OPT_ADAM)
+    rc = rows_range<HIPREC_OPT_ADAM>(f, w_flat, scratch2, records, L, n_triples, batch, step_begin, step_end, n_steps,
+                                     reg_coef, stats, st);
+  else
+    rc = rows_range<HIPREC_OPT_RMSPROP>(f, w_flat, scratch2, records, L, n_triples, batch, step_begin, step_end,
+                                        n_steps, reg_coef, stats, st);
+  if (rc) return rc;
+  *final_index = static_cast<int32_t>(step_end & 1);
+  return 0;
 }
 
 using nccl_all_reduce_fn = int (*)(const void*, void*, size_t, int, int, void*, hipStream_t);
diff --git a/beta-recsys_amd/csrc/util.hip b/beta-recsys_amd/csrc/util.hip
--- a/beta-recsys_amd/csrc/util.hip
+++ b/beta-recsys_amd/csrc/util.hip
@@ -292,6 +292,177 @@
   }
 }
 
+__device__ __forceinline__ int lower_bound_u32(const uint32_t* s, int n, uint32_t key) {
+  int lo = 0, len = n;
+  while (len > 0) {
+    const int half = len >> 1;
+    if (s[lo + half] < key) {
+      lo += half + 1;
+      len -= half + 1;
+    } else {
+      len = half;
+    }
+  }
+  return lo;
+}
+
+template <int NT>
+__device__ __forceinline__ int block_rank(bool flag, uint32_t* s_w, int& running) {
+  const unsigned long long m = __ballot(flag);
+  const int lane = lane_id(), wv = wave_in_block();
+  if (lane == 0) s_w[wv] = static_cast<uint32_t>(__popcll(m));
+  __syncthreads();
+  int before = 0, total = 0;
+  for (int w = 0; w < NT / kWave; ++w) {
+    const int c = static_cast<int>(s_w[w]);
+    before += w < wv ? c : 0;
+    total += c;
+  }
+  __syncthreads();
+  const int r = running + before + __popcll(m & ((1ull << lane) - 1ull));
+  running += total;
+  return r;
+}
+
+template <int NPAD, int NT>
+__global__ __launch_bounds__(NT) void stage_rows_kernel(const int64_t* __restrict__ su,
+                                                        const int64_t* __restrict__ sp,
+                                                        const int64_t* __restrict__ sn, int64_t n, int64_t batch,
+                                                        int64_t n_users, int64_t n_items,
+                                                        int32_t* __restrict__ out, RowRecLayout L) {
+  static_assert(NPAD <= (1 << kRowKeyPosBits), "position bits");
+  extern __shared__ __attribute__((aligned(16))) uint32_t s_dyn[];
+  uint32_t* s_a = s_dyn;
+  uint32_t* s_b = s_dyn + NPAD;
+  uint32_t* s_w = s_dyn + 2 * NPAD;
+  constexpr int kPer = (NPAD + NT - 1) / NT;
+  constexpr uint32_t kPosMask = (1u << kRowKeyPosBits) - 1u;
+  const int tid = static_cast<int>(threadIdx.x);
+  const int64_t off = static_cast<int64_t>(blockIdx.x) * batch;
+  const int cnt = static_cast<int>(min<int64_t>(batch, n - off));
+  const int U = static_cast<int>(n_users), I = static_cast<int>(n_items);
+  int32_t* rec = out + L.rec_off + static_cast<int64_t>(blockIdx.x) * L.rows * kRowRecInts;
+  int32_t* hdr = out + L.hdr_off + static_cast<int64_t>(blockIdx.x) * L.hdr_stride;
+  int32_t* tail_u = out + L.tail_off + static_cast<int64_t>(blockIdx.x) * L.tail_stride;
+  int32_t* tail_p = tail_u + 2 * batch;
+  int32_t* tail_n = tail_u + 4 * batch;
+  if (tid == 0) s_w[16] = 0u;
+  __syncthreads();
+
+  auto key_of = [&](int i, int which, uint32_t& bad) -> uint32_t {
+    if (i >= cnt) return ~0u;
+    const int64_t u = su[off + i], p = sp[off + i], q = sn[off + i];
+    const bool u_ok = static_cast<uint64_t>(u) < static_cast<uint64_t>(n_users);
+    const bool i_ok = static_cast<uint64_t>(p) < static_cast<uint64_t>(n_items) &&
+                      static_cast<uint64_t>(q) < static_cast<uint64_t>(n_items);
+    if (!(u_ok && i_ok)) {
+      bad |= (u_ok ? 0u : HIPREC_STATUS_USER_OOB) | (i_ok ? 0u : HIPREC_STATUS_ITEM_OOB);
+      return ~0u;
+    }
+    const uint32_t row = static_cast<uint32_t>(which == 0 ? u : which == 1 ? p : q);
+    return (row << kRowKeyPosBits) | static_cast<uint32_t>(i);
+  };
+  auto fill_sorted = [&](uint32_t* s_k, int which) {
+    uint32_t bad = 0u;
+#pragma unroll
+    for (int t = 0; t < kPer; ++t) {
+      const int i = tid + t * NT;
+      if (i < NPAD) s_k[i] = key_of(i, which, bad);
+    }
+    if (bad) atomicOr(&s_w[16], bad);
+    bitonic_sort_lds<uint32_t, NPAD, NT>(s_k, true);
+  };
+  auto run_of = [&](const uint32_t* s_k, uint32_t row, int& lo, int& c) {
+    lo = lower_bound_u32(s_k, NPAD, row << kRowKeyPosBits);
+    c = lower_bound_u32(s_k, NPAD, (row + 1u) << kRowKeyPosBits) - lo;
+  };
+  auto put = [&](int32_t* dst, int64_t a, int64_t b) {
+    *reinterpret_cast<int2*>(dst) = make_int2(static_cast<int>(a), static_cast<int>(b));
+  };
+
+  fill_sorted(s_a, 0);
+#pragma unroll
+  for (int t = 0; t < kPer; ++t) {
+    const int s = tid + t * NT;
+    if (s >= NPAD) continue;
+    const uint32_t key = s_a[s];
+    if (key == ~0u) continue;
+    const uint32_t row = key >> kRowKeyPosBits;
+    const int i = static_cast<int>(key & kPosMask);
+    int lo, c;
+    run_of(s_a, row, lo, c);
+    int32_t* dst = c <= kRowInline ? rec + static_cast<int64_t>(row) * kRowRecInts + 2 + 2 * (s - lo) : tail_u + 2 * s;
+    put(dst, sp[off + i], sn[off + i]);
+  }
+  int n_hot = 0;
+  for (int base = 0; base < U; base += NT) {
+    const int r = base + tid;
+    int lo = 0, c = 0;
+    if (r < U) {
+      run_of(s_a, static_cast<uint32_t>(r), lo, c);
+      put(rec + static_cast<int64_t>(r) * kRowRecInts, c, 0);
+    }
+    const bool hot = c > kRowInline;
+    const int slot = block_rank<NT>(hot, s_w, n_hot);
+    if (hot && slot < L.max_hot) {
+      int32_t* q = hdr + kRowHdrInts + kRowHotInts * slot;
+      put(q, r, c);
+      put(q + 2, 0, lo);
+      put(q + 4, 0, 0);
+    }
+  }
+  __syncthreads();
+
+  fill_sorted(s_b, 1);
+  fill_sorted(s_a, 2);
+#pragma unroll
+  for (int t = 0; t < kPer; ++t) {
+    const int s = tid + t * NT;
+    if (s >= NPAD) continue;
+    const uint32_t kp = s_b[s], kn = s_a[s];
+    if (kp != ~0u) {
+      const uint32_t row = kp >> kRowKeyPosBits;
+      const int i = static_cast<int>(kp & kPosMask);
+      int lo0, c0, lo1, c1;
+      run_of(s_b, row, lo0, c0);
+      run_of(s_a, row, lo1, c1);
+      int32_t* dst = c0 + c1 <= kRowInline
+                         ? rec + (static_cast<int64_t>(U) + row) * kRowRecInts + 2 + 2 * (s - lo0)
+                         : tail_p + 2 * s;
+      put(dst, su[off + i], sn[off + i]);
+    }
+    if (kn != ~0u) {
+      const uint32_t row = kn >> kRowKeyPosBits;
+      const int i = static_cast<int>(kn & kPosMask);
+      int lo0, c0, lo1, c1;
+      run_of(s_b, row, lo0, c0);
+      run_of(s_a, row, lo1, c1);
+      int32_t* dst = c0 + c1 <= kRowInline
+                         ? rec + (static_cast<int64_t>(U) + row) * kRowRecInts + 2 + 2 * (c0 + s - lo1)
+                         : tail_n + 2 * s;
+      put(dst, su[off + i], sp[off + i]);
+    }
+  }
+  for (int base = 0; base < I; base += NT) {
+    const int r = base + tid;
+    int lo0 = 0, c0 = 0, lo1 = 0, c1 = 0;
+    if (r < I) {
+      run_of(s_b, static_cast<uint32_t>(r), lo0, c0);
+      run_of(s_a, static_cast<uint32_t>(r), lo1, c1);
+      put(rec + (static_cast<int64_t>(U) + r) * kRowRecInts, c0, c1);
+    }
+    const bool hot = c0 + c1 > kRowInline;
+    const int slot = block_rank<NT>(hot, s_w, n_hot);
+    if (hot && slot < L.max_hot) {
+      int32_t* q = hdr + kRowHdrInts + kRowHotInts * slot;
+      put(q, U + r, c0);
+      put(q + 2, c1, lo0);
+      put(q + 4, lo1, 0);
+    }
+  }
+  if (tid == 0) put(hdr, n_hot < L.max_hot ? n_hot : static_cast<int>(L.max_hot), static_cast<int>(s_w[16]));
+}
+
 }
 
 using namespace hiprec;
@@ -356,6 +527,55 @@
                                            void* stream) {
   return stage_epoch_impl(users, items, third, third_bytes, nullptr, seed, true, n, batch, out_users,
                           out_items, out_third, stream);
+}
+
+extern "C" int hiprec_mf_rows_layout(int64_t n_users, int64_t n_items, int64_t n_triples, int64_t batch,
+                                     int64_t* out9) {
+  HIPREC_REQUIRE(out9 != nullptr, "NULL output");
+  HIPREC_REQUIRE(n_users > 0 && n_items > 0 && n_triples >= 0 && batch > 0, "bad sizes");
+  const RowRecLayout l = row_rec_layout(n_users, n_items, n_triples, batch);
+  const int64_t v[9] = {l.n_batches, l.rows, l.max_hot, l.hdr_stride, l.tail_stride, l.rec_off, l.hdr_off, l.tail_off,
+                        l.total};
+  for (int i = 0; i < 9; ++i) out9[i] = v[i];
+  return 0;
+}
+
+extern "C" int hiprec_stage_rows(const int64_t* users, const int64_t* pos, const int64_t* neg, int64_t n,
+                                 int64_t batch, int64_t n_users, int64_t n_items, int32_t* records,
+                                 int64_t records_ints, void* stream) {
+  HIPREC_REQUIRE(n >= 0 && batch > 0, "bad n / batch");
+  HIPREC_REQUIRE(n_users > 0 && n_items > 0, "bad table sizes");
+  if (batch > 8192 || n_users > kRowMaxTable || n_items > kRowMaxTable) {
+    set_error("hiprec_stage_rows sorts (row, position) keys of 32 bits in LDS: batch %lld > 8192 or a table beyond "
+              "%lld rows is not supported", (long long)batch, (long long)kRowMaxTable);
+    return HIPREC_E_UNSUPPORTED;
+  }
+  if (n == 0) return 0;
+  HIPREC_REQUIRE(users && pos && neg && records, "NULL pointer");
+  const RowRecLayout L = row_rec_layout(n_users, n_items, n, batch);
+  HIPREC_REQUIRE(records_ints >= L.total, "records buffer too small: %lld < %lld ints", (long long)records_ints,
+                 (long long)L.total);
+  HIPREC_REQUIRE(L.n_batches < (1ll << 31), "too many batches");
+  hipStream_t st = static_cast<hipStream_t>(stream);
+  const int grid = static_cast<int>(L.n_batches);
+#define HIPREC_STAGE_ROWS(NP, T)                                                                       \
+  stage_rows_kernel<NP, T><<<grid, T, sizeof(uint32_t) * (2 * NP + 32), st>>>(users, pos, neg, n, batch, n_users, \
+                                                                             n_items, records, L)
+  if (batch <= 64) HIPREC_STAGE_ROWS(64, 64);
+  else if (batch <= 256) HIPREC_STAGE_ROWS(256, 256);
+  else if (batch <= 1024) HIPREC_STAGE_ROWS(1024, 512);
+  else if (batch <= 2048) HIPREC_STAGE_ROWS(2048, 1024);
+  else if (batch <= 4096) HIPREC_STAGE_ROWS(4096, 1024);
+  else {
+    static std::atomic<uint64_t> lds_ok{0};
+    if (int rc = allow_dynamic_lds({reinterpret_cast<const void*>(&stage_rows_kernel<8192, 1024>)},
+                                   sizeof(uint32_t) * (2 * 8192 + 32), lds_ok, "the row records of batches beyond 4096"))
+      return rc;
+    HIPREC_STAGE_ROWS(8192, 1024);
+  }
+#undef HIPREC_STAGE_ROWS
+  HIPREC_TRY(hipGetLastError());
+  return 0;
 }
 
 extern "C" int hiprec_scatter_add_rows(float* table, int64_t n_rows, int32_t dim,
diff --git a/beta-recsys_amd/mf.py b/beta-recsys_amd/mf.py
--- a/beta-recsys_amd/mf.py
+++ b/beta-recsys_amd/mf.py
@@ -271,9 +271,21 @@
     return idx[torch.argsort(key)].contiguous()
 
 
+def owner_step_applies(mode, *, plain_engine, loss, emb_dim, batch, n_triples, staged_on_device, n_users, n_items,
+                       fused_path, optimizer, auto_optimizers):
+    if mode not in ("auto", "owner", "fused"):
+        raise ValueError(f"mf_step must be 'auto', 'owner' or 'fused', not {mode!r}")
+    if mode == "fused":
+        return False
+    return bool(plain_engine and loss == "bpr" and emb_dim <= 64 and 0 < batch <= 8192 and n_triples > 0
+                and staged_on_device and max(n_users, n_items) < 2**19 and fused_path
+                and (mode == "owner" or optimizer in auto_optimizers))
+
+
 class PreparedEpoch(tuple):
 
     own = None
+    rows = None
 
 
 def batch_row_ownership(users, pos, neg, batch_size, n_users, n_items):
@@ -440,6 +452,9 @@
     SORT_MIN_BATCH = 256
     presorted = False
     fused_step = True
+    OWNER_AUTO_OPTIMIZERS = ()
+    RECORDS_BYTES = 1 << 30
+    last_step_form = None
 
     def __init__(self, config):
         self.config = config
@@ -743,7 +758,8 @@
         main = torch.cuda.current_stream(dev)
         pf = getattr(self, "_pf", None)
         if pf is None or pf["dev"] != dev:
-            pf = self._pf = {"dev": dev, "side": torch.cuda.Stream(dev), "slots": [None, None], "next": 0}
+            pf = self._pf = {"dev": dev, "side": torch.cuda.Stream(dev), "slots": [None, None], "rows": [None, None],
+                             "next": 0}
         begin = getattr(self, "_ev_epoch_begin", None)
         if begin is not None:
             pf["side"].wait_event(begin)
@@ -761,7 +777,8 @@
             seed = train_loader.draw_seed()
             with torch.cuda.stream(pf["side"]):
                 self._stage_into(users, pos, neg, None, seed, bs, *slot)
-                prepared = self._finish_staging(slot + (None, bs))
+                prepared = self._finish_staging(slot + (None, bs), rows_buf=pf["rows"][k])
+                pf["rows"][k] = prepared.rows
         else:
             with torch.cuda.stream(pf["side"]):
                 prepared = self._finish_staging(self._resident_triples(train_loader))
@@ -807,7 +824,45 @@
         rows = self.optimizer.name == "sgd" and (mode in ("rows", "owned", "owned_atomic") or (mode == "auto" and big))
         return rows, rows and mode in ("owned", "owned_atomic", "auto") and self.model.emb_dim <= 256
 
-    def _finish_staging(self, staged):
+    def _mf_step(self):
+        mode = self.config["model"].get("mf_step", "auto")
+        if mode not in ("auto", "owner", "fused"):
+            raise ValueError(f"mf_step must be 'auto', 'owner' or 'fused', not {mode!r}")
+        return mode
+
+    def _records_budget(self):
+        return int(self.config["model"].get("mf_records_bytes", self.RECORDS_BYTES))
+
+    def _owner_eligible(self, n, bs, perm):
+        mode = self._mf_step()
+        m = self.model
+        if mode == "fused" or m.flat.device.type != "cuda":
+            return False
+        self._setup()
+        return owner_step_applies(
+            mode, plain_engine=type(self) is MFEngine, loss=self.loss, emb_dim=m.emb_dim, batch=bs, n_triples=n,
+            staged_on_device=perm is None, n_users=m.n_users, n_items=m.n_items,
+            fused_path=self._lazy is None and self._fused_ok(perm), optimizer=self.optimizer.name,
+            auto_optimizers=self.OWNER_AUTO_OPTIMIZERS)
+
+    def _rows_layout(self, n, bs):
+        out = (ctypes.c_int64 * 9)()
+        _lib.check(_lib.load().hiprec_mf_rows_layout(self.model.n_users, self.model.n_items, n, bs, out))
+        return tuple(out)
+
+    def _stage_rows(self, users, pos, neg, bs, buf=None):
+        n, dev = users.numel(), users.device
+        ints = self._rows_layout(n, bs)[8]
+        if ints * 4 > self._records_budget():
+            return None
+        if buf is None or buf.numel() < ints or buf.device != dev:
+            buf = torch.empty(ints, dtype=torch.int32, device=dev)
+        _lib.check(_lib.load().hiprec_stage_rows(
+            _lib.ptr(users), _lib.ptr(pos), _lib.ptr(neg), n, bs, self.model.n_users, self.model.n_items,
+            _lib.ptr(buf), buf.numel(), _lib.stream_ptr(dev)))
+        return buf
+
+    def _finish_staging(self, staged, rows_buf=None):
         if staged is None:
             return None
         owned = (self._sgd_modes()[1] or self._lazy_owned()) and self.loss == "bpr"
@@ -817,6 +872,8 @@
             return staged
         prepared = PreparedEpoch(staged)
         users, pos, neg, perm, bs = prepared
+        if self._owner_eligible(users.numel(), bs, perm):
+            prepared.rows = self._stage_rows(users, pos, neg, bs, rows_buf)
         if owned and perm is None and users.device.type == "cuda":
             small_keys = self.model.n_users + self.model.n_items < 2**31
             if self._sgd_modes()[1] and self._owned_form() == "pull" and small_keys:
@@ -852,9 +909,10 @@
     def _run_fused_epoch(self, lib, users, pos, neg, n_run, bs, steps=None):
         m, opt = self.model, self.optimizer
         dev = m.flat.device
-        if getattr(self, "_fused_bufs", None) is None or self._fused_bufs["dev"] != dev:
+        fb = getattr(self, "_fused_bufs", None)
+        if fb is None or fb["dev"] != dev or fb.get("form") != "fused":
             self._fused_bufs = {
-                "dev": dev, "w_alt": torch.empty_like(m.flat),
+                "dev": dev, "form": "fused", "w_alt": torch.empty_like(m.flat),
                 "m_alt": torch.empty_like(m.flat) if opt.exp_avg is not None else None,
                 "v_alt": torch.empty_like(m.flat) if opt.exp_avg_sq is not None else None,
                 "g": [self._g_flat, torch.zeros_like(m.flat), torch.zeros_like(m.flat)],
@@ -886,6 +944,28 @@
             if opt.exp_avg_sq is not None:
                 opt.exp_avg_sq.copy_(fb["v_alt"])
 
+    def _run_owner_epoch(self, lib, prepared, n_run, bs, steps=None):
+        m, opt = self.model, self.optimizer
+        dev = m.flat.device
+        fb = getattr(self, "_fused_bufs", None)
+        if fb is None or fb["dev"] != dev or fb.get("form") != "owner":
+            fb = self._fused_bufs = {
+                "dev": dev, "form": "owner", "w_alt": torch.empty_like(m.flat), "g": [self._g_flat],
+                "scratch": [torch.zeros_like(self._scratch), torch.zeros_like(self._scratch)]}
+        fb["g"][0] = self._g_flat
+        w_arr = (ctypes.c_void_p * 2)(m.flat.data_ptr(), fb["w_alt"].data_ptr())
+        s_arr = (ctypes.c_void_p * 2)(*(t.data_ptr() for t in fb["scratch"]))
+        final = ctypes.c_int32(-1)
+        n_steps = (n_run + bs - 1) // bs
+        a, b = (0, n_steps) if steps is None else steps
+        rows = prepared.rows
+        _lib.check(lib.hiprec_mf_bpr_epoch_rows_range(
+            opt.kind, w_arr, _lib.ptr(opt.exp_avg), _lib.ptr(opt.exp_avg_sq), s_arr, m.n_users, m.n_items, m.emb_dim,
+            _lib.ptr(rows), rows.numel(), prepared[0].numel(), n_run, bs, a, b, float(self.reg), opt.lr, opt.beta1,
+            opt.beta2, opt.eps, _lib.ptr(self._stats), ctypes.byref(final), _lib.stream_ptr(dev)))
+        if b == n_steps and final.value == 1:
+            m.flat.copy_(fb["w_alt"])
+
     def run_prepared_epoch(self, prepared, sync=True, prefetch=None, steps=None):
         lib = self._setup()
         users, pos, neg, perm, bs = prepared
@@ -900,6 +980,7 @@
         if steps is None or steps[0] == 0:
             self._begin_epoch_marker(prepared, prefetch)
         if self._owned_sgd and self.loss == "bpr" and getattr(prepared, "own", None) is not None:
+            self.last_step_form = "owned"
             self._run_owned_epoch(lib, prepared, n_run, steps)
             if not sync:
                 return None
@@ -909,6 +990,7 @@
                     "Dimension out of range (expected to be in range of [-1, 0], but got 1)")
             return st
         if self._lazy is not None and perm is None and self.loss in ("bpr", "bce"):
+            self.last_step_form = "lazy"
             self._run_lazy_epoch(lib, users, pos, neg, n_run, bs, steps, getattr(prepared, "own", None))
             if not sync:
                 return None
@@ -918,7 +1000,12 @@
                     "Dimension out of range (expected to be in range of [-1, 0], but got 1)")
             return st
         if self._fused_ok(perm):
-            self._run_fused_epoch(lib, users, pos, neg, n_run, bs, steps)
+            if getattr(prepared, "rows", None) is not None and n_run > 0 and self._mf_step() != "fused":
+                self.last_step_form = "owner"
+                self._run_owner_epoch(lib, prepared, n_run, bs, steps)
+            else:
+                self.last_step_form = "fused"
+                self._run_fused_epoch(lib, users, pos, neg, n_run, bs, steps)
             if not sync:
                 return None
             st = self._sync_stats()
@@ -930,6 +1017,7 @@
             a, b = steps[0] * bs, min(steps[1] * bs, n_run)
             users, pos, neg, n_run = users[a:b], pos[a:b], neg[a:b], b - a
             perm = None if perm is None else perm[a:b]
+        self.last_step_form = "two-kernel"
         return self._run_unfused_epoch(lib, users, pos, neg, perm, bs, n, n_run, sync)
 
     def _run_lazy_epoch(self, lib, users, items_a, third, n_run, bs, steps, own=None):
diff --git a/include/hiprec.h b/include/hiprec.h
--- a/include/hiprec.h
+++ b/include/hiprec.h
@@ -153,6 +153,15 @@
                                     int64_t batch, int64_t step_begin, int64_t step_end, float reg_coef,
                                     double lr, double beta1, double beta2, double eps, hiprec_stats* stats,
                                     int32_t* final_index, void* stream);
+int hiprec_mf_rows_layout(int64_t n_users, int64_t n_items, int64_t n_triples, int64_t batch, int64_t* out9);
+int hiprec_stage_rows(const int64_t* users, const int64_t* pos, const int64_t* neg, int64_t n, int64_t batch,
+                      int64_t n_users, int64_t n_items, int32_t* records, int64_t records_ints, void* stream);
+int hiprec_mf_bpr_epoch_rows_range(int kind, float* const* w_flat, float* m_flat, float* v_flat,
+                                   void* const* scratch2, int64_t n_users, int64_t n_items, int32_t dim,
+                                   const int32_t* records, int64_t records_ints, int64_t records_triples,
+                                   int64_t n_triples, int64_t batch, int64_t step_begin, int64_t step_end,
+                                   float reg_coef, double lr, double beta1, double beta2, double eps,
+                                   hiprec_stats* stats, int32_t* final_index, void* stream);
 int hiprec_mf_bpr_dp_epoch_fused_range(int kind, float* const* w_flat, float* const* bufs, int64_t scratch_floats,
                                        float* const* m_flat, float* const* v_flat, int64_t n_flat, int64_t n_users,
                                        int64_t n_items, int32_t dim, const int64_t* users, const int64_t* pos,
```
